# drprojects/superpoint_transformer

Hardware: AMD Instinct MI355X
Metric: Mpoints/s SPT fwd+bwd on S3DIS-scale NAG (higher is better)
Workload: dtype f32 (the reference's shipped matmul class - configs/train.yaml:60-61 `float32_matmul_precision: high` = TF32 / bf16x3 next to `precision: 32` - as bf16x3: matrix products on the bf16 pipe with split operands, attention and the backward of the fused layers and of the attention blocks' Linears hi*hi +

## Files before the change

include/spt_hip.h:

```cpp
#ifndef SPT_HIP_H
#define SPT_HIP_H

#include <stddef.h>
#include <stdint.h>

#ifdef __cplusplus
extern "C" {
#endif

typedef void* spt_stream_t;

enum spt_reduce_op {
  SPT_SUM = 0,
  SPT_MEAN = 1,
  SPT_MIN = 2,
  SPT_MAX = 3
};

typedef struct spt_gn_fwd_tables {
  const float* weight;
  const float* mean_scale;
  float eps;
  float* mean;
  float* rstd;
// ... 368 lines not shown
                                       const int64_t* edge_a, const int64_t* edge_b, int64_t e,
                                       float* gend, spt_stream_t stream);

int spt_skinny_linear_supported(int K, int N);
int spt_skinny_linear_f32(const float* x, int64_t rows, int K, const float* W, const float* bias,
                          int N, float* y, spt_stream_t stream);
int spt_skinny_linear_wt_f32(const float* x, int64_t rows, int K, const float* Wt, int N, float* y,
                             spt_stream_t stream);
int spt_skinny_pre_supported(int K, int N, int num_graphs);
int spt_skinny_linear_pre_f32(const float* x, int64_t rows, int K, const float* W, const float* bias,
                              int N, float* y, const float* pre_am, const float* pre_scale,
                              const float* pre_bias, const int64_t* batch, int num_graphs,
                              const float* residual, spt_stream_t stream);
int spt_skinny_dw_pre_f32(const float* gy, const float* x, int64_t rows, int N, int K, float* gw,
                          float* gb, const float* pre_am, const float* pre_scale,
                          const float* pre_bias, const int64_t* batch, int num_graphs, void* ws,
                          size_t ws_bytes, spt_stream_t stream);
int spt_skinny_use_split_bf16(int mode);
int spt_skinny_linear_pre_m_f32(const float* x, int64_t rows, int K, const float* W, const float* bias,
                                int N, float* y, const float* pre_am, const float* pre_scale,
                                const float* pre_bias, const int64_t* batch, int num_graphs,
                                const float* residual, int mode, spt_stream_t stream);
int spt_skinny_linear_wt_m_f32(const float* x, int64_t rows, int K, const float* Wt, int N, float* y,
                               int mode, spt_stream_t stream);
int spt_skinny_dw_pre_m_f32(const float* gy, const float* x, int64_t rows, int N, int K, float* gw,
                            float* gb, const float* pre_am, const float* pre_scale,
                            const float* pre_bias, const int64_t* batch, int num_graphs, int mode,
                            void* ws, size_t ws_bytes, spt_stream_t stream);
int spt_skinny_dw_supported(int K, int N);
size_t spt_skinny_dw_workspace_bytes(int K, int N);
int spt_skinny_dw_f32(const float* gy, const float* x, int64_t rows, int N, int K, float* gw,
                      float* gb, void* ws, size_t ws_bytes, spt_stream_t stream);
int spt_narrow_linear_bwd_supported(int K, int N);
size_t spt_narrow_linear_bwd_workspace_bytes(int K, int N);
int spt_narrow_linear_bwd_f32(const float* gy, const float* x, const float* W, int64_t rows, int N,
                              int K, float* gx, float* gw, float* gb, void* ws, size_t ws_bytes,
                              spt_stream_t stream);

int spt_graphnorm_tables_f32(const double* total, int num_graphs, int d, const float* weight,
                             const float* mean_scale, float eps, float* mean, float* rstd,
                             float* am, float* scale, spt_stream_t stream);
int spt_graphnorm_apply_f32(const float* x, const int64_t* batch, int64_t r, int d,
                            int num_graphs, const float* am, const float* scale,
                            const float* bias, float act_slope, float* y, spt_stream_t stream);
int spt_graphnorm_bwd_stats_f32(const float* x, const float* gy, const int64_t* batch, int64_t r,
                                int d, int num_graphs, const float* am, const float* scale,
                                const float* bias, float act_slope, double* total, void* ws,
                                size_t ws_bytes, spt_stream_t stream);
size_t spt_graphnorm_bwd_stats_sparse_workspace_bytes(int64_t num_seg, int d, int num_graphs);
int spt_graphnorm_bwd_stats_sparse_f32(const float* x, const float* gout, const int32_t* arg,
                                       const int64_t* seg_graph, const int64_t* graph_rows,
                                       int64_t num_seg, int64_t n, int d, int num_graphs,
                                       const float* am, const float* scale, const float* bias,
                                       float act_slope, double* total, void* ws,
                                       size_t ws_bytes, spt_stream_t stream);
int spt_graphnorm_bwd_stats_sparse_ex_f32(
    const void* x, int x_is_bf16, const float* gout, const int32_t* arg, const int64_t* seg_graph,
    const int64_t* graph_rows, int64_t num_seg, int64_t n, int d, int num_graphs,
    const float* am, const float* scale, const float* bias, float act_slope, double* total,
    void* ws, size_t ws_bytes, spt_stream_t stream);
int spt_graphnorm_bwd_stats_sparse_raw_f32(
    const float* raw, const float* gout, const int32_t* arg, const int64_t* seg_graph,
    const int64_t* graph_rows, int64_t num_seg, int64_t n, int d, int num_graphs,
    const float* am, const float* scale, const float* bias, float act_slope, double* total,
    void* ws, size_t ws_bytes, spt_stream_t stream);
int spt_graphnorm_bwd_tables_f32(const double* total, int num_graphs, int d, const float* weight,
                                 const float* mean_scale, const float* mean, const float* rstd,
                                 float* c1, float* c2, float* c3, float* gweight, float* gbias,
                                 float* gmean_scale, spt_stream_t stream);

int spt_fused_linear_supported(int K, int N);
int spt_fused_linear_use_split_bf16(int mode);
size_t spt_fused_linear_workspace_bytes(int K, int N);
int spt_fused_linear_fwd_f32(const float* x, int64_t r0, int64_t r1, int K, const float* W,
                             int N, const float* pre_am, const float* pre_scale,
                             const float* pre_bias, float pre_slope, float* h, double* total,
                             void* ws, size_t ws_bytes, spt_stream_t stream);
int spt_fused_linear_bwd_f32(const float* gy, const float* h, int64_t r0, int64_t r1, int N,
                             const float* am, const float* scale, const float* bias,
                             float slope, const float* c1, const float* c2, const float* c3,
                             const float* xprev, int K, const float* pre_am,
                             const float* pre_scale, const float* pre_bias, float pre_slope,
                             const float* W, float* gx, float* gW, int accumulate,
                             double* prev_total, void* ws, size_t ws_bytes, spt_stream_t stream);
int spt_fused_linear_pooled_supported(int K, int N);
int spt_fused_linear_pooled_supported_ex(int K, int N, int mode);
#define SPT_FMLP_BWD_REGISTER_STAGED 4
#define SPT_FMLP_H_BF16 8
#define SPT_FMLP_X_BF16 16
int spt_fused_linear_storage_supported(int K, int N);
int spt_fused_linear_bwd_use_dma(int on);
int spt_fused_linear_fwd_use_x3(int on);
int spt_fused_linear_fwd_ex_f32(const float* x, int64_t r0, int64_t r1, int K, const float* W,
                                int N, const float* pre_am, const float* pre_scale,
                                const float* pre_bias, float pre_slope, float* h, double* total,
                                int mode, void* ws, size_t ws_bytes, spt_stream_t stream);
int spt_fused_linear_bwd_ex_f32(const float* gy, const float* h, int64_t r0, int64_t r1, int N,
                                const float* am, const float* scale, const float* bias,
                                float slope, const float* c1, const float* c2, const float* c3,
                                const float* xprev, int K, const float* pre_am,
                                const float* pre_scale, const float* pre_bias, float pre_slope,
                                const float* W, float* gx, float* gW, int accumulate,
                                double* prev_total, int mode, void* ws, size_t ws_bytes,
                                spt_stream_t stream);
int spt_fused_linear_bwd_pooled_ex_f32(
    const float* gout, const int32_t* arg, const int32_t* perm, const int32_t* pos_seg,
    const float* h, int64_t p0, int64_t p1, int N, const float* am, const float* scale,
    const float* bias, float slope, const float* c1, const float* c2, const float* c3,
    const float* xprev, int K, const float* pre_am, const float* pre_scale, const float* pre_bias,
    float pre_slope, const float* W, float* gx, float* gW, int accumulate, double* prev_total,
    int mode, void* ws, size_t ws_bytes, spt_stream_t stream);
int spt_fused_linear_bwd_pooled_f32(
    const float* gout, const int32_t* arg, const int32_t* perm, const int32_t* pos_seg,
    const float* h, int64_t p0, int64_t p1, int N, const float* am, const float* scale,
    const float* bias, float slope, const float* c1, const float* c2, const float* c3,
    const float* xprev, int K, const float* pre_am, const float* pre_scale, const float* pre_bias,
    float pre_slope, const float* W, float* gx, float* gW, int accumulate, double* prev_total,
    void* ws, size_t ws_bytes, spt_stream_t stream);

int spt_fused_linear_fwd_runs_f32(const float* x, int nruns, const int64_t* run_r0,
                                  const int64_t* run_r1, const int32_t* run_graph, int num_graphs,
                                  int K, const float* W, int N, const float* pre_am,
                                  const float* pre_scale, const float* pre_bias, float pre_slope,
                                  float* h, double* total, int mode, void* ws, size_t ws_bytes,
                                  spt_stream_t stream);
int spt_fused_linear_bwd_runs_f32(
    const float* gy, const float* h, int nruns, const int64_t* run_r0, const int64_t* run_r1,
    const int32_t* run_graph, int num_graphs, int N, const float* am, const float* scale,
    const float* bias, float slope, const float* c1, const float* c2, const float* c3,
    const float* xprev, int K, const float* pre_am, const float* pre_scale, const float* pre_bias,
    float pre_slope, const float* W, float* gx, float* gW, double* prev_total, int mode, void* ws,
    size_t ws_bytes, spt_stream_t stream);
int spt_fused_linear_bwd_pooled_runs_f32(
    const float* gout, const int32_t* arg, const int32_t* perm, const int32_t* pos_seg,
    const float* h, int nruns, const int64_t* run_p0, const int64_t* run_p1,
    const int32_t* run_graph, int num_graphs, int N, const float* am, const float* scale,
    const float* bias, float slope, const float* c1, const float* c2, const float* c3,
    const float* xprev, int K, const float* pre_am, const float* pre_scale, const float* pre_bias,
    float pre_slope, const float* W, float* gx, float* gW, double* prev_total, int mode, void* ws,
    size_t ws_bytes, spt_stream_t stream);
int spt_fused_linear_fwd_runs_gn_f32(const float* x, int nruns, const int64_t* run_r0,
                                     const int64_t* run_r1, const int32_t* run_graph, int num_graphs,
                                     int K, const float* W, int N, const float* pre_am,
                                     const float* pre_scale, const float* pre_bias, float pre_slope,
                                     float* h, double* total, int mode, void* ws, size_t ws_bytes,
                                     const spt_gn_fwd_tables* norm, spt_stream_t stream);
int spt_fused_linear_bwd_runs_gn_f32(
    const float* gy, const float* h, int nruns, const int64_t* run_r0, const int64_t* run_r1,
    const int32_t* run_graph, int num_graphs, int N, const float* am, const float* scale,
    const float* bias, float slope, const float* c1, const float* c2, const float* c3,
    const float* xprev, int K, const float* pre_am, const float* pre_scale, const float* pre_bias,
    float pre_slope, const float* W, float* gx, float* gW, double* prev_total, int mode, void* ws,
    size_t ws_bytes, const spt_gn_bwd_tables* prev_norm, spt_stream_t stream);
int spt_fused_linear_bwd_pooled_runs_gn_f32(
    const float* gout, const int32_t* arg, const int32_t* perm, const int32_t* pos_seg,
    const float* h, int nruns, const int64_t* run_p0, const int64_t* run_p1,
    const int32_t* run_graph, int num_graphs, int N, const float* am, const float* scale,
    const float* bias, float slope, const float* c1, const float* c2, const float* c3,
    const float* xprev, int K, const float* pre_am, const float* pre_scale, const float* pre_bias,
    float pre_slope, const float* W, float* gx, float* gW, double* prev_total, int mode, void* ws,
    size_t ws_bytes, const spt_gn_bwd_tables* prev_norm, spt_stream_t stream);

int spt_csr_check_i64(const int64_t* idx, const int64_t* points, const int64_t* pointers, int64_t n,
                      int64_t num_seg, int check_ascending, int32_t* flag, spt_stream_t stream);
int spt_csr_adopt_i64(const int64_t* idx, const int64_t* points, const int64_t* pointers, int64_t n,
                      int64_t num_seg, int32_t* perm32, int32_t* rowptr32, int32_t* flag,
                      spt_stream_t stream);

int spt_fused_linear_pool_supported(int K, int N, int mode);
size_t spt_fused_linear_pool_gram_len(int K);
size_t spt_fused_linear_pool_workspace_bytes(int K, int N);
int spt_fused_linear_fwd_pool_runs_f32(
    const void* x, const int32_t* perm, const int32_t* pos_seg, const int32_t* rowptr,
    const int64_t* seg_graph, int64_t num_seg, int64_t n_rows, int nruns, const int64_t* run_p0,
    const int64_t* run_p1, const int32_t* run_graph, int num_graphs, int K, const float* W, int N,
    const float* gn_weight, const float* gn_bias, const float* gn_mean_scale, float eps, float slope,
    const float* pre_am, const float* pre_scale, const float* pre_bias, float pre_slope, float* out,
    int32_t* arg, int32_t* argpos, float* raw, double* gram, double* total, float* mean, float* rstd,
    float* am, float* scale, int mode, void* ws, size_t ws_bytes, spt_stream_t stream);
int spt_fused_linear_bwd_pool_runs_f32(
    const float* gout, const float* raw, const int32_t* argpos, const int32_t* perm,
    const int32_t* pos_seg, const int64_t* seg_graph, int64_t num_seg, int nruns,
    const int64_t* run_p0, const int64_t* run_p1, const int32_t* run_graph, int num_graphs, int N,
    const float* am, const float* scale, const float* bias, float slope, const float* c1,
    const float* c2, const float* c3, const void* xprev, int K, const float* pre_am,
    const float* pre_scale, const float* pre_bias, float pre_slope, const float* W,
    const double* gram, float* gm, float* gx, float* gW, double* prev_total, int mode, void* ws,
    size_t ws_bytes, spt_stream_t stream);
int spt_fused_linear_bwd_pool_runs_gn_f32(
    const float* gout, const float* raw, const int32_t* argpos, const int32_t* perm,
    const int32_t* pos_seg, const int64_t* seg_graph, int64_t num_seg, int nruns,
    const int64_t* run_p0, const int64_t* run_p1, const int32_t* run_graph, int num_graphs, int N,
    const float* am, const float* scale, const float* bias, float slope, const float* c1,
    const float* c2, const float* c3, const void* xprev, int K, const float* pre_am,
    const float* pre_scale, const float* pre_bias, float pre_slope, const float* W,
    const double* gram, float* gm, float* gx, float* gW, double* prev_total, int mode, void* ws,
    size_t ws_bytes, const spt_gn_bwd_tables* prev_norm, spt_stream_t stream);

size_t spt_cross_entropy_workspace_bytes(int64_t rows);
int spt_cross_entropy_fwd_f32(const float* logits, const int64_t* target, int64_t rows, int C,
                              int64_t ignore_index, float* lse, float* loss, float* count,
                              void* ws, size_t ws_bytes, spt_stream_t stream);
int spt_cross_entropy_bwd_f32(const float* logits, const int64_t* target, const float* lse,
                              int64_t rows, int C, int64_t ignore_index, const float* gout,
                              const float* count, float* glogits, spt_stream_t stream);

int spt_hist_loss_fwd_f32(const float* logits, const int64_t* target, int64_t rows, int C, int ncols,
                          int mode, int64_t ignore_index, const float* weight, float* loss,
                          double* den, int64_t* confmat, void* ws, size_t ws_bytes,
                          spt_stream_t stream);
int spt_hist_loss_bwd_f32(const float* logits, const int64_t* target, int64_t rows, int C, int ncols,
                          int mode, int64_t ignore_index, const float* weight, const float* gout,
                          const double* den, float* glogits, spt_stream_t stream);
int spt_confusion_matrix_i64(const int64_t* pred, const int64_t* target, int64_t rows, int C,
                             int ncols, int64_t* confmat, spt_stream_t stream);

#ifdef __cplusplus
}
#endif
#endif
```

superpoint_transformer_amd/_lib.py:

```python
import ctypes
import os

import torch

_HERE = os.path.dirname(os.path.abspath(__file__))
LIB_PATH = os.path.join(_HERE, "lib", "libspt_hip.so")

_c = ctypes
_i64 = _c.c_int64
_int = _c.c_int
_p = _c.c_void_p
_sz = _c.c_size_t
_f32 = _c.c_float
_f64 = _c.c_double

SIGNATURES = {
    "spt_version": (_int, []),
    "spt_last_error": (_c.c_char_p, []),
    "spt_csr_build_workspace_bytes": (_sz, [_i64, _i64]),
    "spt_csr_build": (_int, [_p, _i64, _i64, _p, _p, _p, _sz, _p]),
    "spt_csr_pos_seg": (_int, [_p, _i64, _i64, _p, _p]),
    "spt_csr_gather_i64_i32": (_int, [_p, _p, _i64, _p, _p]),
    "spt_segcsr_reduce_f32": (_int, [_int, _p, _p, _p, _i64, _i64, _int, _p, _p, _p]),
    "spt_segcsr_max_affine_f32": (_int, [_p, _p, _p, _i64, _i64, _int, _p, _p, _p, _f32, _p, _p, _p, _p]),
    "spt_segcsr_max_affine_bf16_supported": (_int, [_int, _i64]),
    "spt_segcsr_max_affine_bf16": (_int, [_p, _p, _p, _i64, _i64, _int, _p, _p, _p, _f32, _p, _p, _p, _p]),
    "spt_segcsr_max_affine_raw_supported": (_int, [_int, _i64]),
    "spt_segcsr_max_affine_raw_f32": (_int, [_p, _int, _p, _p, _i64, _i64, _int, _p, _p, _p, _f32, _p, _p, _p,
                                             _p, _p]),
    "spt_graphnorm_bwd_stats_sparse_raw_f32": (_int, [_p, _p, _p, _p, _p, _i64, _i64, _int, _int, _p, _p, _p,
                                                      _f32, _p, _p, _sz, _p]),
    "spt_fused_linear_storage_supported": (_int, [_int, _int]),
    "spt_graphnorm_bwd_stats_sparse_ex_f32": (_int, [_p, _int, _p, _p, _p, _p, _i64, _i64, _int, _int, _p, _p,
                                                     _p, _f32, _p, _p, _sz, _p]),
    "spt_segcsr_reduce_bwd_f32": (_int, [_int, _p, _p, _p, _p, _p, _i64, _i64, _int, _p, _p]),
    "spt_segcsr_sum_i64": (_int, [_p, _p, _p, _i64, _i64, _int, _p, _p]),
    "spt_gather_rows_f32": (_int, [_p, _p, _i64, _i64, _int, _p, _p]),
    "spt_graphnorm_workspace_bytes": (_sz, [_i64, _int, _int]),
    "spt_graphnorm_fwd_f32": (_int, [_p, _p, _i64, _int, _int, _p, _p, _p, _f32, _f32,
                                     _p, _p, _p, _p, _sz, _p]),
    "spt_graphnorm_bwd_f32": (_int, [_p, _p, _p, _i64, _int, _int, _p, _p, _p, _p, _p,
                                     _f32, _p, _p, _p, _p, _p, _sz, _p]),
    "spt_graphnorm_stats_f32": (_int, [_p, _p, _i64, _int, _int, _p, _p, _f32, _p, _p, _p, _p,
                                       _p, _sz, _p]),
    "spt_graphnorm_bwd_acc_f32": (_int, [_p, _p, _p, _i64, _int, _int, _p, _p, _p, _p, _p,
                                         _f32, _p, _p, _p, _p, _p, _p, _sz, _p]),
    "spt_edge_attn_fwd_f32": (_int, [_p, _i64, _int, _int, _int, _p, _p, _p, _i64, _p, _int,
                                     _p, _p, _p, _p, _p, _p, _int, _f32, _p, _p, _p, _p]),
    "spt_edge_attn_bwd_workspace_bytes": (_sz, [_int, _int, _int, _int]),
    "spt_attn_use_mfma": (_int, [_int]),
    "spt_attn_bwd_packed": (_int, [_int]),
    "spt_attn_bwd_el_full_line": (_int, [_int]),
    "spt_attn_bwd_el_target_order": (_int, [_int]),
    "spt_attn_tile_record_ints": (_int, []),
    "spt_attn_pack_tile_ids_ex": (_int, [_p, _p, _p, _p, _i64, _p, _p]),
    "spt_attn_tile_record_ints_m": (_int, [_int]),
    "spt_attn_pack_tile_ids_m": (_int, [_p, _p, _p, _p, _i64, _int, _p, _p]),
    "spt_attn_mirror_prepare": (_int, [_p, _p, _i64, _i64, _p, _p, _p]),
    "spt_attn_pack_tile_ids_mirror": (_int, [_p, _p, _p, _p, _i64, _i64, _p, _p]),
    "spt_attn_split_pack_f32": (_int, [_p, _i64, _int, _int, _p, _p]),
    "spt_attn_split_grad_f32": (_int, [_p, _i64, _int, _int, _p, _p]),
    "spt_edge_attn_bwd_f32": (_int, [_p, _i64, _int, _int, _int, _p, _p, _p, _i64, _p, _int,
                                     _p, _p, _p, _p, _p, _p, _int, _f32, _p, _p, _p, _p,
                                     _p, _p, _p, _p, _p, _p, _p, _p, _p, _sz, _p]),
    "spt_edge_attn_bwd_acc_f32": (_int, [_p, _i64, _int, _int, _int, _p, _p, _p, _i64, _p, _int,
                                         _p, _p, _p, _p, _p, _p, _int, _f32, _p, _p, _p, _p,
                                         _p, _p, _int, _p, _p, _p, _p, _p, _p, _p, _sz, _p]),
    "spt_edge_attn_fwd_ex_f32": (_int, [_p, _i64, _int, _int, _int, _p, _p, _p, _i64, _p, _int,
                                        _p, _p, _p, _p, _p, _p, _int, _f32, _p, _p, _p, _int, _p]),
    "spt_edge_attn_bwd_ex_workspace_bytes": (_sz, [_i64, _i64, _int, _int, _int, _int]),
    "spt_edge_attn_bwd_el_supported": (_int, [_int, _int, _int, _int, _int]),
    "spt_attn_pack_tile_ids": (_int, [_p, _p, _p, _i64, _p, _p]),
    "spt_edge_attn_bwd_ex_f32": (_int, [_p, _i64, _int, _int, _int, _p, _p, _p, _p, _p, _p, _p, _i64, _p, _int,
                                        _p, _p, _p, _p, _p, _p, _int, _f32, _p, _p, _p, _p,
                                        _p, _p, _int, _p, _p, _p, _p, _p, _p, _int, _p, _sz, _p]),
    "spt_grid_knn_workspace_bytes": (_sz, [_i64, _i64]),
    "spt_knn_use_cell_path": (_int, [_int]),
    "spt_segcsr_use_stream": (_int, [_int]),
    "spt_segcsr_reduce_ex_f32": (_int, [_int, _p, _p, _p, _i64, _i64, _int, _p, _p, _int, _p]),
    "spt_segcsr_max_affine_ex_f32": (_int, [_p, _p, _p, _i64, _i64, _int, _p, _p, _p, _f32, _p, _p, _p,
                                            _int, _p]),
    "spt_grid_knn_ex_f32": (_int, [_p, _i64, _p, _i64, _int, _f32, _f32, _p, _p, _int, _int, _int,
                                   _p, _p, _p, _int, _p, _sz, _p]),
    "spt_grid_knn_geof_f32": (_int, [_p, _i64, _int, _f32, _f32, _p, _p, _int, _int, _int, _int,
                                     _p, _p, _p, _p, _int, _p, _sz, _p]),
    "spt_grid_knn_after_f32": (_int, [_p, _i64, _p, _i64, _int, _f32, _f32, _p, _p, _int, _int, _p, _p,
                                      _p, _p, _p, _sz, _p]),
    "spt_grid_knn_f32": (_int, [_p, _i64, _p, _i64, _int, _f32, _f32, _p, _p, _int, _int, _int,
                                _p, _p, _p, _p, _sz, _p]),
    "spt_point_geof_dense_f32": (_int, [_p, _i64, _p, _int, _int, _int, _int, _p, _p, _p]),
    "spt_point_geof_dense_ld_f32": (_int, [_p, _i64, _p, _int, _i64, _int, _int, _int, _p, _p, _p]),
    "spt_bbox_f32": (_int, [_p, _i64, _p, _p]),
    "spt_knn_subsample_f32": (_int, [_p, _i64, _p, _f32, _int, _p, _p, _p]),
    "spt_grid_cell_ids_f32": (_int, [_p, _i64, _f32, _p, _p, _p, _p]),
    "spt_grid_count_cells_workspace_bytes": (_sz, [_i64]),
    "spt_grid_count_cells_f32": (_int, [_p, _i64, _f32, _p, _p, _p, _p, _sz, _p]),
    "spt_spatial_order_workspace_bytes": (_sz, [_i64, _i64]),
    "spt_spatial_order": (_int, [_p, _i64, _f32, _p, _p, _p, _p, _sz, _p]),
    "spt_point_geof_csr_f32": (_int, [_p, _i64, _p, _p, _int, _int, _int, _p, _p]),
    "spt_vertical_edge_features_f32": (_int, [_p, _i64] + [_p] * 13 + [_p]),
    "spt_edge_affinity_features_f32": (_int, [_p, _i64, _int, _p, _p, _i64, _p, _p]),
    "spt_edge_affinity_features_bwd_f32": (_int, [_p, _p, _i64, _int, _p, _p, _i64, _p, _p]),
    "spt_scatter_pca_f32": (_int, [_p, _p, _p, _i64, _p, _p, _p]),
    "spt_neighbors_dense_to_csr_workspace_bytes": (_sz, [_i64]),
    "spt_neighbors_dense_to_csr": (_int, [_p, _i64, _int, _p, _p, _p, _p, _sz, _p]),
    "spt_horizontal_edge_features_f32": (_int, [_p, _i64, _i64, _p, _p, _p, _p, _p, _p, _p, _int,
                                                _p, _p, _p]),
    "spt_graphnorm_tables_f32": (_int, [_p, _int, _int, _p, _p, _f32, _p, _p, _p, _p, _p]),
    "spt_graphnorm_apply_f32": (_int, [_p, _p, _i64, _int, _int, _p, _p, _p, _f32, _p, _p]),
    "spt_graphnorm_bwd_stats_f32": (_int, [_p, _p, _p, _i64, _int, _int, _p, _p, _p, _f32, _p,
                                           _p, _sz, _p]),
    "spt_graphnorm_bwd_stats_sparse_workspace_bytes": (_sz, [_i64, _int, _int]),
    "spt_graphnorm_bwd_stats_sparse_f32": (_int, [_p, _p, _p, _p, _p, _i64, _i64, _int, _int, _p, _p,
                                                   _p, _f32, _p, _p, _sz, _p]),
    "spt_graphnorm_bwd_tables_f32": (_int, [_p, _int, _int, _p, _p, _p, _p, _p, _p, _p, _p, _p,
                                            _p, _p]),
    "spt_fused_linear_supported": (_int, [_int, _int]),
    "spt_fused_linear_use_split_bf16": (_int, [_int]),
    "spt_fused_linear_bwd_use_dma": (_int, [_int]),
    "spt_fused_linear_fwd_use_x3": (_int, [_int]),
    "spt_fused_linear_pooled_supported": (_int, [_int, _int]),
    "spt_fused_linear_bwd_pooled_f32": (_int, [_p, _p, _p, _p, _p, _i64, _i64, _int, _p, _p, _p, _f32,
                                               _p, _p, _p, _p, _int, _p, _p, _p, _f32, _p, _p, _p,
                                               _int, _p, _p, _sz, _p]),
    "spt_fused_linear_pooled_supported_ex": (_int, [_int, _int, _int]),
    "spt_fused_linear_fwd_ex_f32": (_int, [_p, _i64, _i64, _int, _p, _int, _p, _p, _p, _f32, _p, _p,
                                           _int, _p, _sz, _p]),
    "spt_fused_linear_bwd_ex_f32": (_int, [_p, _p, _i64, _i64, _int, _p, _p, _p, _f32, _p, _p, _p,
                                           _p, _int, _p, _p, _p, _f32, _p, _p, _p, _int, _p, _int, _p,
                                           _sz, _p]),
    "spt_fused_linear_bwd_pooled_ex_f32": (_int, [_p, _p, _p, _p, _p, _i64, _i64, _int, _p, _p, _p, _f32,
                                                  _p, _p, _p, _p, _int, _p, _p, _p, _f32, _p, _p, _p,
                                                  _int, _p, _int, _p, _sz, _p]),
    "spt_fused_linear_workspace_bytes": (_sz, [_int, _int]),
    "spt_fused_linear_fwd_runs_f32": (_int, [_p, _int, _p, _p, _p, _int, _int, _p, _int, _p, _p, _p,
                                             _f32, _p, _p, _int, _p, _sz, _p]),
    "spt_fused_linear_bwd_runs_f32": (_int, [_p, _p, _int, _p, _p, _p, _int, _int, _p, _p, _p, _f32,
                                             _p, _p, _p, _p, _int, _p, _p, _p, _f32, _p, _p, _p, _p,
                                             _int, _p, _sz, _p]),
    "spt_fused_linear_bwd_pooled_runs_f32": (_int, [_p, _p, _p, _p, _p, _int, _p, _p, _p, _int, _int,
                                                    _p, _p, _p, _f32, _p, _p, _p, _p, _int, _p, _p,
                                                    _p, _f32, _p, _p, _p, _p, _int, _p, _sz, _p]),
    "spt_fused_linear_fwd_runs_gn_f32": (_int, [_p, _int, _p, _p, _p, _int, _int, _p, _int, _p, _p, _p,
                                                _f32, _p, _p, _int, _p, _sz, _p, _p]),
    "spt_fused_linear_bwd_runs_gn_f32": (_int, [_p, _p, _int, _p, _p, _p, _int, _int, _p, _p, _p, _f32,
                                                _p, _p, _p, _p, _int, _p, _p, _p, _f32, _p, _p, _p, _p,
                                                _int, _p, _sz, _p, _p]),
    "spt_fused_linear_bwd_pooled_runs_gn_f32": (_int, [_p, _p, _p, _p, _p, _int, _p, _p, _p, _int, _int,
                                                       _p, _p, _p, _f32, _p, _p, _p, _p, _int, _p, _p,
                                                       _p, _f32, _p, _p, _p, _p, _int, _p, _sz, _p, _p]),
    "spt_fused_linear_bwd_pool_runs_gn_f32": (_int, [_p, _p, _p, _p, _p, _p, _i64, _int, _p, _p, _p, _int,
                                                     _int, _p, _p, _p, _f32, _p, _p, _p, _p, _int, _p, _p,
                                                     _p, _f32, _p, _p, _p, _p, _p, _p, _int, _p, _sz, _p, _p]),
    "spt_csr_check_i64": (_int, [_p, _p, _p, _i64, _i64, _int, _p, _p]),
    "spt_csr_adopt_i64": (_int, [_p, _p, _p, _i64, _i64, _p, _p, _p, _p]),
    "spt_fused_linear_pool_supported": (_int, [_int, _int, _int]),
    "spt_fused_linear_pool_gram_len": (_sz, [_int]),
    "spt_fused_linear_pool_workspace_bytes": (_sz, [_int, _int]),
    "spt_fused_linear_fwd_pool_runs_f32": (_int, [_p, _p, _p, _p, _p, _i64, _i64, _int, _p, _p, _p, _int,
                                                  _int, _p, _int, _p, _p, _p, _f32, _f32, _p, _p, _p,
                                                  _f32, _p, _p, _p, _p, _p, _p, _p, _p, _p, _p, _int, _p,
                                                  _sz, _p]),
    "spt_fused_linear_bwd_pool_runs_f32": (_int, [_p, _p, _p, _p, _p, _p, _i64, _int, _p, _p, _p, _int,
                                                  _int, _p, _p, _p, _f32, _p, _p, _p, _p, _int, _p, _p,
                                                  _p, _f32, _p, _p, _p, _p, _p, _p, _int, _p, _sz, _p]),
    "spt_fused_linear_fwd_f32": (_int, [_p, _i64, _i64, _int, _p, _int, _p, _p, _p, _f32, _p, _p,
                                        _p, _sz, _p]),
    "spt_fused_linear_bwd_f32": (_int, [_p, _p, _i64, _i64, _int, _p, _p, _p, _f32, _p, _p, _p,
                                        _p, _int, _p, _p, _p, _f32, _p, _p, _p, _int, _p, _p,
                                        _sz, _p]),
    "spt_unit_sphere_norm_f32": (_int, [_p, _p, _p, _p, _p, _p, _i64, _i64, _p, _p, _p, _p]),
    "spt_unit_sphere_assemble_f32": (_int, [_p, _p, _p, _p, _p, _p, _i64, _i64, _p, _int, _p, _p, _p, _p]),
    "spt_unit_sphere_workspace_bytes": (_sz, [_i64, _i64]),
    "spt_unit_sphere_norm_ws_f32": (_int, [_p, _p, _p, _p, _p, _p, _i64, _i64, _p, _p, _p, _p, _sz, _p]),
    "spt_unit_sphere_assemble_ws_f32": (_int, [_p, _p, _p, _p, _p, _p, _i64, _i64, _p, _int, _p, _p, _p,
                                               _p, _sz, _p]),
    "spt_sparse_sample_workspace_bytes": (_sz, [_i64, _i64]),
    "spt_sparse_sample": (_int, [_p, _i64, _i64, _p, _int, _int, _c.c_uint64, _p, _p, _p, _sz, _p]),
    "spt_segment_std_f32": (_int, [_p, _p, _p, _i64, _int, _p, _p]),
    "spt_segment_mean_orientation_f32": (_int, [_p, _p, _p, _i64, _p, _p]),
    "spt_cluster_graph_edges_workspace_bytes": (_sz, [_i64, _int]),
    "spt_cluster_graph_edges": (_int, [_p, _p, _p, _i64, _int, _f32, _int, _p, _p, _p, _p, _sz, _p]),
    "spt_skinny_linear_supported": (_int, [_int, _int]),
    "spt_narrow_linear_bwd_supported": (_int, [_int, _int]),
    "spt_narrow_linear_bwd_workspace_bytes": (_sz, [_int, _int]),
    "spt_narrow_linear_bwd_f32": (_int, [_p, _p, _p, _i64, _int, _int, _p, _p, _p, _p, _sz, _p]),
    "spt_cross_entropy_workspace_bytes": (_sz, [_i64]),
    "spt_cross_entropy_fwd_f32": (_int, [_p, _p, _i64, _int, _i64, _p, _p, _p, _p, _sz, _p]),
    "spt_cross_entropy_bwd_f32": (_int, [_p, _p, _p, _i64, _int, _i64, _p, _p, _p, _p]),
    "spt_hist_loss_fwd_f32": (_int, [_p, _p, _i64, _int, _int, _int, _i64, _p, _p, _p, _p, _p, _sz, _p]),
    "spt_hist_loss_bwd_f32": (_int, [_p, _p, _i64, _int, _int, _int, _i64, _p, _p, _p, _p, _p]),
    "spt_confusion_matrix_i64": (_int, [_p, _p, _i64, _int, _int, _p, _p]),
    "spt_skinny_dw_supported": (_int, [_int, _int]),
    "spt_skinny_dw_workspace_bytes": (_sz, [_int, _int]),
    "spt_skinny_dw_f32": (_int, [_p, _p, _i64, _int, _int, _p, _p, _p, _sz, _p]),
    "spt_skinny_linear_f32": (_int, [_p, _i64, _int, _p, _p, _int, _p, _p]),
    "spt_skinny_linear_wt_f32": (_int, [_p, _i64, _int, _p, _int, _p, _p]),
    "spt_skinny_pre_supported": (_int, [_int, _int, _int]),
    "spt_skinny_linear_pre_f32": (_int, [_p, _i64, _int, _p, _p, _int, _p, _p, _p, _p, _p, _int, _p, _p]),
    "spt_skinny_dw_pre_f32": (_int, [_p, _p, _i64, _int, _int, _p, _p, _p, _p, _p, _p, _int, _p, _sz, _p]),
    "spt_skinny_use_split_bf16": (_int, [_int]),
    "spt_skinny_linear_pre_m_f32": (_int, [_p, _i64, _int, _p, _p, _int, _p, _p, _p, _p, _p, _int, _p, _int, _p]),
    "spt_skinny_linear_wt_m_f32": (_int, [_p, _i64, _int, _p, _int, _p, _int, _p]),
    "spt_skinny_dw_pre_m_f32": (_int, [_p, _p, _i64, _int, _int, _p, _p, _p, _p, _p, _p, _int, _int, _p, _sz, _p]),
    "spt_index_inverse": (_int, [_p, _i64, _i64, _p, _p]),
    "spt_select_edges_workspace_bytes": (_sz, [_i64]),
    "spt_select_edges": (_int, [_p, _i64, _i64, _p, _i64, _p, _i64, _p, _p, _p, _sz, _p]),
    "spt_cluster_select_workspace_bytes": (_sz, [_i64, _i64, _i64]),
    "spt_cluster_select": (_int, [_p, _p, _i64, _p, _i64, _i64, _p, _p, _p, _p, _p, _p, _sz, _p]),
    "spt_relabel_consecutive_workspace_bytes": (_sz, [_i64]),
    "spt_relabel_consecutive": (_int, [_p, _p, _i64, _i64, _p, _p, _p, _p, _sz, _p]),
    "spt_radius_ball_workspace_bytes": (_sz, [_i64]),
    "spt_radius_ball_f32": (_int, [_p, _i64, _p, _f32, _int, _p, _i64, _p, _p, _p, _sz, _p]),
    "spt_cluster_pair_anchors_f32": (_int, [_p, _p, _p, _p, _p, _i64, _i64, _int, _int, _p, _p, _p]),
    "spt_adjacency_stats_workspace_bytes": (_sz, [_i64]),
    "spt_adjacency_stats": (_int, [_p, _p, _i64, _i64, _int, _p, _p, _p, _sz, _p]),
    "spt_adjacency_regression": (_int, [_p, _p, _p, _i64, _i64, _int, _f32, _f32, _p, _p, _sz, _p]),
    "spt_adjacency_count_workspace_bytes": (_sz, [_i64]),
    "spt_adjacency_count": (_int, [_p, _i64, _i64, _int, _p, _p, _p, _i64, _int, _p, _p, _p, _sz, _p]),
    "spt_adjacency_fill_workspace_bytes": (_sz, [_i64, _i64]),
    "spt_adjacency_fill": (_int, [_p, _p, _i64, _i64, _int, _f32, _f32, _p, _p, _p, _p, _i64, _int, _int,
                                  _p, _p, _i64, _p, _p, _p, _p, _sz, _p]),
    "spt_ground_bounds_workspace_bytes": (_sz, [_i64]),
    "spt_ground_bounds_f32": (_int, [_p, _i64, _f32, _p, _p, _sz, _p]),
    "spt_ground_cell_min_f32": (_int, [_p, _i64, _f32, _i64, _i64, _i64, _i64, _p, _p]),
    "spt_ground_trim_workspace_bytes": (_sz, [_i64]),
    "spt_ground_trim_f32": (_int, [_p, _i64, _p, _int, _f32, _p, _f32, _p, _i64, _p, _i64, _p, _p, _sz, _p]),
    "spt_ground_ransac_workspace_bytes": (_sz, [_int]),
    "spt_ground_ransac_f32": (_int, [_p, _i64, _p, _p, _i64, _p, _p, _int, _f64, _p, _p, _p, _sz, _p]),
    "spt_ground_elevation_f32": (_int, [_p, _i64, _p, _f32, _p, _p]),
    "spt_point_color_workspace_bytes": (_sz, [_i64]),
    "spt_point_color_f32": (_int, [_p, _int, _i64, _int, _p, _i64, _p, _i64, _p, _i64, _p, _sz, _p]),
    "spt_point_density_f32": (_int, [_p, _i64, _p, _i64, _i64, _int, _p, _p]),
}


class GnFwdTables(ctypes.Structure):
    _fields_ = [("weight", _p), ("mean_scale", _p), ("eps", _f32), ("mean", _p), ("rstd", _p),
                ("am", _p), ("scale", _p)]


class GnBwdTables(ctypes.Structure):
    _fields_ = [("weight", _p), ("mean_scale", _p), ("mean", _p), ("rstd", _p), ("c1", _p), ("c2", _p),
                ("c3", _p), ("gweight", _p), ("gbias", _p), ("gmean_scale", _p)]


def _load():
    if not os.path.exists(LIB_PATH):
        raise ImportError(
            f"{LIB_PATH} is missing: run `python -c 'import __graft_entry__ as g; "
            f"g.build()'` (hipcc --offload-arch=gfx950). There is no fallback path.")
    lib = ctypes.CDLL(LIB_PATH)
    for name, (res, args) in SIGNATURES.items():
        fn = getattr(lib, name)
        fn.restype = res
        fn.argtypes = args
    return lib


lib = _load()


def last_error():
    return lib.spt_last_error().decode("utf-8", "replace")


def check(status, what):
    if status != 0:
        raise RuntimeError(f"{what} failed ({status}): {last_error()}")


def ptr(t):
    return None if t is None else t.data_ptr()


def stream_ptr(device=None):
    return torch.cuda.current_stream(device).cuda_stream


def require_cuda(*tensors):
    for t in tensors:
        if t is not None and not t.is_cuda:
            raise RuntimeError(
                "superpoint_transformer_amd ops run on the MI355X only: got a "
                f"{t.device} tensor (no CPU fallback is provided)")
```

superpoint_transformer_amd/csrc/fused_mlp.hip:

```cpp
#include <math.h>
#include <stdlib.h>

#include "common.hpp"

namespace spt {
namespace fmlp {

typedef float f32x4 __attribute__((ext_vector_type(4)));
constexpr int WAVES = 4;
constexpr int TR = 16;
constexpr int MAX_BLOCKS = 1024;
constexpr int MAX_BWD_WAVES = 4096;

__device__ __forceinline__ double xg_sum_d(double v) {
  v += __shfl_xor(v, 16, 64);
  v += __shfl_xor(v, 32, 64);
  return v;
}
__device__ __forceinline__ void wave_sync_lds() {
  __builtin_amdgcn_fence(__ATOMIC_RELEASE, "wavefront");
  __builtin_amdgcn_wave_barrier();
  __builtin_amdgcn_fence(__ATOMIC_ACQUIRE, "wavefront");
}

// ... 637 lines not shown
    const __bf16 a = (__bf16)x[i];
    const float r1 = x[i] - (float)a;
    const __bf16 b = (__bf16)r1;
    const float r2 = r1 - (float)b;
    h[i] = a;
    m[i] = b;
    l[i] = (__bf16)r2;
  }
}
template <int K4, int NBK>
__global__ __launch_bounds__(WAVES_X3 * 64, 2) void fwd_kernel_x3(
    const float* __restrict__ x, int64_t r0, int64_t r1, int K, const float* __restrict__ W,
    const float* __restrict__ am, const float* __restrict__ sc, const float* __restrict__ bs,
    float slope, float* __restrict__ h, double* __restrict__ partial, FmlpRuns rt) {
  constexpr int KP = K4 * 4, KS = (KP + 31) / 32, KP32 = KS * 32, LDA = KP32 + 4, N = NBK * 16;
  constexpr int LDW = KP32 + 8;
  SPT_FMLP_RUN_FWD(N)
  __shared__ __attribute__((aligned(16))) float a_lds[WAVES_X3][TR * LDA];
  __shared__ __attribute__((aligned(16))) float tab[3 * KP32];
  __shared__ __attribute__((aligned(16))) __bf16 wpl[3][N * LDW];
  __shared__ double red[WAVES_X3][2 * N];
  const int lane = threadIdx.x & 63;
  const int wid = __builtin_amdgcn_readfirstlane(threadIdx.x >> 6);
  const int g = lane >> 4, c = lane & 15;
  float* al = a_lds[wid];
  const bool pre = am != nullptr;
  load_table(tab, am, K, KP32);
  load_table(tab + KP32, sc, K, KP32);
  load_table(tab + 2 * KP32, bs, K, KP32);
  for (int i = lane; i < TR * LDA; i += 64) al[i] = 0.f;
  for (int i = threadIdx.x; i < N * KP32; i += WAVES_X3 * 64) {
    const int n = i / KP32, k = i - n * KP32;
    const float w1[1] = {(k < K) ? W[(size_t)n * K + k] : 0.f};
    __bf16 a[1], b[1], cc[1];
    split3_bf16<1>(w1, a, b, cc);
    wpl[0][n * LDW + k] = a[0];
    wpl[1][n * LDW + k] = b[0];
    wpl[2][n * LDW + k] = cc[0];
  }
  __syncthreads();

  double s1[NBK], s2[NBK];
#pragma unroll
  for (int nb = 0; nb < NBK; ++nb) s1[nb] = s2[nb] = 0.0;

  const int64_t ntiles = (r1 - r0 + TR - 1) / TR;
  const int64_t wave = (int64_t)blockIdx.x * WAVES_X3 + wid;
  const int64_t nwaves = (int64_t)gridDim.x * WAVES_X3;
  constexpr int CHP = KP / 4, NITP = (TR * CHP + 63) / 64;
  const bool pref = (K & 3) == 0 && K == KP;
  float4 pv[NITP];
  auto prefetch = [&](int64_t t) {
    const int64_t row0 = r0 + t * TR;
    const int cnt = (t < ntiles) ? (int)((r1 - row0) < TR ? (r1 - row0) : TR) : 0;
#pragma unroll
    for (int j = 0; j < NITP; ++j) {
      const int q = lane + 64 * j, rr = q / CHP, k = (q - rr * CHP) << 2;
      const bool ok = q < TR * CHP && rr < cnt;
      const float4 v = *reinterpret_cast<const float4*>(x + (ok ? (row0 + rr) * K + k : r0 * K));
      pv[j] = ok ? v : make_float4(0.f, 0.f, 0.f, 0.f);
    }
  };
  if (pref && wave < ntiles) prefetch(wave);
  for (int64_t t = wave; t < ntiles; t += nwaves) {
    const int64_t row0 = r0 + t * TR;
    const int cnt = (int)((r1 - row0) < TR ? (r1 - row0) : TR);
    wave_sync_lds();
    if (pref) {
#pragma unroll
      for (int j = 0; j < NITP; ++j) {
        const int q = lane + 64 * j, rr = q / CHP, k = (q - rr * CHP) << 2;
        if (q < TR * CHP) {
          float4 w = pv[j];
          if (pre && rr < cnt) {
            const float4 a = *reinterpret_cast<const float4*>(tab + k);
            const float4 s4 = *reinterpret_cast<const float4*>(tab + KP32 + k);
            const float4 b = *reinterpret_cast<const float4*>(tab + 2 * KP32 + k);
            w.x = fmaf(w.x - a.x, s4.x, b.x); w.y = fmaf(w.y - a.y, s4.y, b.y);
            w.z = fmaf(w.z - a.z, s4.z, b.z); w.w = fmaf(w.w - a.w, s4.w, b.w);
            w.x = w.x > 0.f ? w.x : w.x * slope; w.y = w.y > 0.f ? w.y : w.y * slope;
            w.z = w.z > 0.f ? w.z : w.z * slope; w.w = w.w > 0.f ? w.w : w.w * slope;
          }
          *reinterpret_cast<float4*>(al + rr * LDA + k) = w;
        }
      }
    } else {
      stage_tile<KP32, LDA, KP32>(x, row0, cnt, K, pre, tab, slope, al, nullptr, lane);
    }
    wave_sync_lds();
    if (pref) prefetch(t + nwaves);
    f32x4 C[NBK];
#pragma unroll
    for (int nb = 0; nb < NBK; ++nb) C[nb] = (f32x4){0.f, 0.f, 0.f, 0.f};
#pragma unroll
    for (int ks = 0; ks < KS; ++ks) {
      const float4 a0 = *reinterpret_cast<const float4*>(al + c * LDA + 32 * ks + 8 * g);
      const float4 a1 = *reinterpret_cast<const float4*>(al + c * LDA + 32 * ks + 8 * g + 4);
      const float av[8] = {a0.x, a0.y, a0.z, a0.w, a1.x, a1.y, a1.z, a1.w};
      bf16x8 x1, x2, x3;
      split3_bf16<8>(av, x1, x2, x3);
#pragma unroll
      for (int nb = 0; nb < NBK; ++nb) {
        const int wo = (16 * nb + c) * LDW + 32 * ks + 8 * g;
        const bf16x8 w1 = *reinterpret_cast<const bf16x8*>(&wpl[0][wo]);
        const bf16x8 w2 = *reinterpret_cast<const bf16x8*>(&wpl[1][wo]);
        const bf16x8 w3 = *reinterpret_cast<const bf16x8*>(&wpl[2][wo]);
        f32x4 acc = C[nb];
        acc = __builtin_amdgcn_mfma_f32_16x16x32_bf16(x3, w1, acc, 0, 0, 0);
        acc = __builtin_amdgcn_mfma_f32_16x16x32_bf16(x1, w3, acc, 0, 0, 0);
        acc = __builtin_amdgcn_mfma_f32_16x16x32_bf16(x2, w2, acc, 0, 0, 0);
        acc = __builtin_amdgcn_mfma_f32_16x16x32_bf16(x2, w1, acc, 0, 0, 0);
        acc = __builtin_amdgcn_mfma_f32_16x16x32_bf16(x1, w2, acc, 0, 0, 0);
        acc = __builtin_amdgcn_mfma_f32_16x16x32_bf16(x1, w1, acc, 0, 0, 0);
        C[nb] = acc;
      }
    }
#pragma unroll
    for (int r = 0; r < 4; ++r) {
      const int rr = 4 * g + r;
      if (rr < cnt) {
        float* hr = h + (row0 + rr) * N + c;
#pragma unroll
        for (int nb = 0; nb < NBK; ++nb) {
          const float v = C[nb][r];
          hr[16 * nb] = v;
          s1[nb] += (double)v;
          s2[nb] += (double)v * (double)v;
        }
      }
    }
  }
#pragma unroll
  for (int nb = 0; nb < NBK; ++nb) {
    const double a = xg_sum_d(s1[nb]), b = xg_sum_d(s2[nb]);
    if (g == 0) {
      red[wid][nb * 16 + c] = a;
      red[wid][N + nb * 16 + c] = b;
    }
  }
  __syncthreads();
  double* out = partial + (size_t)blockIdx.x * (2 * N + 1);
  for (int i = threadIdx.x; i < 2 * N; i += WAVES_X3 * 64) {
    double t2 = 0.0;
#pragma unroll
    for (int w = 0; w < WAVES_X3; ++w) t2 += red[w][i];
    out[i] = t2;
  }
  if (threadIdx.x == 0) out[2 * N] = (blockIdx.x == 0) ? (double)(r1 - r0) : 0.0;
}

__host__ __device__ constexpr bool fmlp_bf_wg_reduce(int K4, int NBK, int NW) {
  return NBK * 16 <= NW * TR && K4 > 0;
}
template <int K4, int NBK, bool NEED_GX, int NW, bool LO, bool POOLED = false, bool PIPE = false,
          bool H16 = false, bool X16 = false>
__global__ __launch_bounds__(NW * 64, NW / 4) void bwd_kernel_bf(
    const float* __restrict__ gy, const float* __restrict__ h, int64_t r0, int64_t r1,
    const float* __restrict__ am, const float* __restrict__ sc, const float* __restrict__ bs,
    float slope, const float* __restrict__ c1, const float* __restrict__ c2,
    const float* __restrict__ c3, const float* __restrict__ xprev, int K,
    const float* __restrict__ pam, const float* __restrict__ psc, const float* __restrict__ pbs,
    float pslope, const float* __restrict__ W, float* __restrict__ gx,
    float* __restrict__ gw_partial, double* __restrict__ pstat_partial, FmlpRuns rt,
    const int32_t* __restrict__ perm = nullptr, const int32_t* __restrict__ pos_seg = nullptr,
    const float* __restrict__ gout = nullptr, const int32_t* __restrict__ arg = nullptr) {
  constexpr int KP = K4 * 4, KB = (KP + 15) / 16, KPP = KB * 16, N = NBK * 16;
  constexpr int NS = (N + 31) / 32, NP32 = NS * 32;
  constexpr int LDG = NP32 + 4, LDX = KPP + 4, LDT = NP32 + 8;
  constexpr bool WGR = fmlp_bf_wg_reduce(K4, NBK, NW);
  SPT_FMLP_RUN_BWD_T(N, NW, (WGR ? 1 : NW))
  __shared__ __attribute__((aligned(16))) float g_lds[NW][TR * LDG];
  __shared__ __attribute__((aligned(16))) float x_lds[NW][TR * LDX];
  __shared__ __attribute__((aligned(16))) __bf16 wt_hi[NEED_GX ? KPP * LDT : 8];
  __shared__ __attribute__((aligned(16))) __bf16 wt_lo[NEED_GX ? KPP * LDT : 8];
  __shared__ __attribute__((aligned(16))) float gt[6 * N];
  __shared__ __attribute__((aligned(16))) float pt[3 * KPP];
  const int lane = threadIdx.x & 63;
  const int wid = __builtin_amdgcn_readfirstlane(threadIdx.x >> 6);
  const int g = lane >> 4, c = lane & 15;
  float* gl = g_lds[wid];
  float* xl = x_lds[wid];
  const bool pre = pam != nullptr;
  if constexpr (NEED_GX) {
    for (int i = threadIdx.x; i < KPP * NP32; i += NW * 64) {
      const int k = i / NP32, n = i - k * NP32;
      const float w = (k < K && n < N) ? W[(size_t)n * K + k] : 0.f;
      const __bf16 hh = (__bf16)w;
      wt_hi[k * LDT + n] = hh;
      wt_lo[k * LDT + n] = (__bf16)(w - (float)hh);
    }
  }
  load_table(gt, am, N, N);
  load_table(gt + N, sc, N, N);
  load_table(gt + 2 * N, bs, N, N);
  load_table(gt + 3 * N, c1, N, N);
  load_table(gt + 4 * N, c2, N, N);
  load_table(gt + 5 * N, c3, N, N);
  load_table(pt, pam, K, KPP);
  load_table(pt + KPP, psc, K, KPP);
  load_table(pt + 2 * KPP, pbs, K, KPP);
  for (int i = lane; i < TR * LDX; i += 64) xl[i] = 0.f;
  for (int i = lane; i < TR * LDG; i += 64) gl[i] = 0.f;
  __syncthreads();

  f32x4 C3[NBK][KB];
#pragma unroll
  for (int nb = 0; nb < NBK; ++nb)
#pragma unroll
    for (int kb = 0; kb < KB; ++kb) C3[nb][kb] = (f32x4){0.f, 0.f, 0.f, 0.f};
  double p1[KB], p2[KB];
#pragma unroll
  for (int kb = 0; kb < KB; ++kb) p1[kb] = p2[kb] = 0.0;

  const int64_t ntiles = (r1 - r0 + TR - 1) / TR;
  const int64_t wave = (int64_t)blockIdx.x * NW + wid;
  const int64_t nwaves = (int64_t)gridDim.x * NW;
  auto gh_of = [&](const float4& hv, const float4& gv, int n) {
    const float4 a = *reinterpret_cast<const float4*>(gt + n);
    const float4 sc4 = *reinterpret_cast<const float4*>(gt + N + n);
    const float4 b4 = *reinterpret_cast<const float4*>(gt + 2 * N + n);
    const float4 k1 = *reinterpret_cast<const float4*>(gt + 3 * N + n);
    const float4 k2 = *reinterpret_cast<const float4*>(gt + 4 * N + n);
    const float4 k3 = *reinterpret_cast<const float4*>(gt + 5 * N + n);
    const float hh[4] = {hv.x, hv.y, hv.z, hv.w}, gg4[4] = {gv.x, gv.y, gv.z, gv.w};
    const float aa[4] = {a.x, a.y, a.z, a.w}, ss[4] = {sc4.x, sc4.y, sc4.z, sc4.w};
    const float bb[4] = {b4.x, b4.y, b4.z, b4.w}, q1[4] = {k1.x, k1.y, k1.z, k1.w};
    const float q2[4] = {k2.x, k2.y, k2.z, k2.w}, q3[4] = {k3.x, k3.y, k3.z, k3.w};
    float o4[4];
#pragma unroll
    for (int e = 0; e < 4; ++e) {
      const float o = hh[e] - aa[e];
      float gg = gg4[e];
      if (slope != 1.f) {
        const float y = fmaf(o, ss[e], bb[e]);
        gg = (y > 0.f) ? gg : gg * slope;
      }
      o4[e] = fmaf(q1[e], gg, -fmaf(q2[e], o, q3[e]));
    }
    return make_float4(o4[0], o4[1], o4[2], o4[3]);
  };
  static_assert(!(PIPE && (H16 || X16)), "the register-prefetch variant reads f32 rows");
  constexpr int CH = N / 4, CHX = KPP / 4;
  constexpr int HN = PIPE ? TR * CH / 64 : 1, XN = PIPE ? TR * CHX / 64 : 1;
  float4 p_h[HN], p_g[HN], p_x[XN];
  int4 p_a[(PIPE && POOLED) ? HN : 1];
  int rid_n = 0, seg_n = 0;
  auto load_ids = [&](int64_t t) {
    rid_n = seg_n = 0;
    if constexpr (POOLED) {
      const int64_t rowf = r0 + t * TR;
      if (t < ntiles && rowf + lane < r1 && lane < TR) {
        rid_n = perm[rowf + lane];
        seg_n = pos_seg[rowf + lane];
      }
    }
  };
  auto load_raw = [&](int64_t t, int rid_l, int seg_l) {
    const int64_t row0 = r0 + t * TR;
    const int cnt = (t < ntiles) ? (int)((r1 - row0) < TR ? (r1 - row0) : TR) : 0;
#pragma unroll
    for (int i = 0; i < HN; ++i) {
      const int q = lane + 64 * i, rr = q / CH, n = (q - rr * CH) << 2;
      const int rid = POOLED ? __shfl(rid_l, rr, 64) : 0;
      const int64_t sg = POOLED ? (int64_t)__shfl(seg_l, rr, 64) : 0;
      p_h[i] = p_g[i] = make_float4(0.f, 0.f, 0.f, 0.f);
      if (rr < cnt) {
        const int64_t hr = POOLED ? (int64_t)rid : row0 + rr;
        p_h[i] = *reinterpret_cast<const float4*>(h + hr * N + n);
        if constexpr (POOLED) {
          p_a[i] = *reinterpret_cast<const int4*>(arg + sg * N + n);
          p_g[i] = *reinterpret_cast<const float4*>(gout + sg * N + n);
        } else {
          p_g[i] = *reinterpret_cast<const float4*>(gy + (row0 + rr) * N + n);
        }
      }
    }
#pragma unroll
    for (int i = 0; i < XN; ++i) {
      const int q = lane + 64 * i, rr = q / CHX, k = (q - rr * CHX) << 2;
      const int64_t xr = POOLED ? (int64_t)__shfl(rid_l, rr, 64) : row0 + rr;
      p_x[i] = make_float4(0.f, 0.f, 0.f, 0.f);
      if (rr < cnt && k < K) p_x[i] = *reinterpret_cast<const float4*>(xprev + xr * K + k);
    }
  };
  load_ids(wave);
  if constexpr (PIPE) {
    load_raw(wave, rid_n, seg_n);
  }
  int rid_l = rid_n, seg_l = seg_n;
  load_ids(wave + nwaves);
  FM_PROBE_INIT
  for (int64_t t = wave; t < ntiles; t += nwaves) {
    const int64_t row0 = r0 + t * TR;
    const int cnt = (int)((r1 - row0) < TR ? (r1 - row0) : TR);
    wave_sync_lds();
    FM_PROBE(5)
    if constexpr (PIPE) {
#pragma unroll
      for (int i = 0; i < HN; ++i) {
        const int q = lane + 64 * i, rr = q / CH, n = (q - rr * CH) << 2;
        float4 gv = p_g[i];
        if constexpr (POOLED) {
          const int rid = __shfl(rid_l, rr, 64);
          gv = make_float4(p_a[i].x == rid ? gv.x : 0.f, p_a[i].y == rid ? gv.y : 0.f,
                           p_a[i].z == rid ? gv.z : 0.f, p_a[i].w == rid ? gv.w : 0.f);
        }
        float4 v = make_float4(0.f, 0.f, 0.f, 0.f);
        if (rr < cnt) v = gh_of(p_h[i], gv, n);
        *reinterpret_cast<float4*>(gl + rr * LDG + n) = v;
      }
#pragma unroll
      for (int i = 0; i < XN; ++i) {
        const int q = lane + 64 * i, rr = q / CHX, k = (q - rr * CHX) << 2;
        *reinterpret_cast<float4*>(xl + rr * LDX + k) = p_x[i];
      }
    } else {
      constexpr int NITG = TR * CH / 64, GS = NITG < 2 ? 1 : 2;
      static_assert(TR * CH % 64 == 0, "whole waves of chunks");
#pragma unroll 1
      for (int i0 = 0; i0 < NITG; i0 += GS) {
        float4 hv[GS], gv[GS];
        int4 av[POOLED ? GS : 1];
        int ridv[GS];
#pragma unroll
        for (int j = 0; j < GS; ++j) {
          const int q = lane + 64 * (i0 + j), rr = q / CH, n = (q - rr * CH) << 2;
          ridv[j] = POOLED ? __shfl(rid_l, rr, 64) : 0;
          const int64_t sg = POOLED ? (int64_t)__shfl(seg_l, rr, 64) : 0;
          hv[j] = gv[j] = make_float4(0.f, 0.f, 0.f, 0.f);
          if constexpr (POOLED) av[j] = make_int4(-1, -1, -1, -1);
          if (rr < cnt) {
            const int64_t hr = POOLED ? (int64_t)ridv[j] : row0 + rr;
            hv[j] = ld4<H16>(h, hr * N + n);
            if constexpr (POOLED) {
              av[j] = *reinterpret_cast<const int4*>(arg + sg * N + n);
              gv[j] = *reinterpret_cast<const float4*>(gout + sg * N + n);
            } else {
              gv[j] = *reinterpret_cast<const float4*>(gy + (row0 + rr) * N + n);
            }
          }
        }
#pragma unroll
        for (int j = 0; j < GS; ++j) {
          const int q = lane + 64 * (i0 + j), rr = q / CH, n = (q - rr * CH) << 2;
          float4 v = make_float4(0.f, 0.f, 0.f, 0.f);
          if (rr < cnt) {
            float4 g4 = gv[j];
            if constexpr (POOLED) {
              const int rid = ridv[j];
              g4 = make_float4(av[j].x == rid ? g4.x : 0.f, av[j].y == rid ? g4.y : 0.f,
                               av[j].z == rid ? g4.z : 0.f, av[j].w == rid ? g4.w : 0.f);
            }
            v = gh_of(hv[j], g4, n);
          }
          *reinterpret_cast<float4*>(gl + rr * LDG + n) = v;
        }
      }
      FM_PROBE(0)
      stage_tile<KPP, LDX, KPP, POOLED, (POOLED && NBK >= 8) ? 2 : 4, X16>(xprev, row0, cnt, K, false, pt,
                                                                             pslope, xl, nullptr, lane, rid_l);
      FM_PROBE(1)
    }
    const int rid_cur = rid_l;
    if constexpr (PIPE) load_raw(t + nwaves, rid_n, seg_n);
    rid_l = rid_n;
    seg_l = seg_n;
    load_ids(t + 2 * nwaves);
    wave_sync_lds();
    FM_PROBE(2)
    {
      bf16x4 Xh[KB], Xl[KB];
#pragma unroll
      for (int kb = 0; kb < KB; ++kb) {
        const int k = 16 * kb + c;
        float xv[4];
#pragma unroll
        for (int r = 0; r < 4; ++r) {
          float v = xl[(4 * g + r) * LDX + k];
          if (pre) {
            v = fmaf(v - pt[k], pt[KPP + k], pt[2 * KPP + k]);
            v = (v > 0.f) ? v : v * pslope;
            v = (4 * g + r < cnt && k < K) ? v : 0.f;
          }
          xv[r] = v;
        }
        split_bf16<4>(xv, Xh[kb], Xl[kb]);
      }
#pragma unroll
      for (int nb = 0; nb < NBK; ++nb) {
        float gv[4];
#pragma unroll
        for (int r = 0; r < 4; ++r) gv[r] = gl[(4 * g + r) * LDG + 16 * nb + c];
        bf16x4 gh4, gl4;
        split_bf16<4>(gv, gh4, gl4);
#pragma unroll
        for (int kb = 0; kb < KB; ++kb) C3[nb][kb] = mfma3_16<LO>(gh4, gl4, Xh[kb], Xl[kb], C3[nb][kb]);
      }
    }
    FM_PROBE(3)
    if constexpr (NEED_GX) {
      f32x4 CX[KB];
#pragma unroll
      for (int kb = 0; kb < KB; ++kb) CX[kb] = (f32x4){0.f, 0.f, 0.f, 0.f};
      constexpr int LAB = (NW == 4 && K4 > 16) ? 2 : 0, NSTG = NS * KB;
      bf16x8 bfh[LAB + 1], bfl[LAB + 1];
      auto ldb = [&](int step, bf16x8& bh, bf16x8& bl) {
        const int sg = step / KB, kb = step - sg * KB;
        bh = *reinterpret_cast<const bf16x8*>(wt_hi + (16 * kb + c) * LDT + 32 * sg + 8 * g);
        if constexpr (LO) bl = *reinterpret_cast<const bf16x8*>(wt_lo + (16 * kb + c) * LDT + 32 * sg + 8 * g);
        else bl = bh;
      };
#pragma unroll
      for (int i = 0; i < LAB && i < NSTG; ++i) ldb(i, bfh[i], bfl[i]);
      bf16x8 ah, alo;
#pragma unroll
      for (int step = 0; step < NSTG; ++step) {
        const int sg = step / KB, kb = step - sg * KB;
        if (kb == 0) {
          const float4 a0 = *reinterpret_cast<const float4*>(gl + c * LDG + 32 * sg + 8 * g);
          const float4 a1 = *reinterpret_cast<const float4*>(gl + c * LDG + 32 * sg + 8 * g + 4);
          const float av[8] = {a0.x, a0.y, a0.z, a0.w, a1.x, a1.y, a1.z, a1.w};
          split_bf16<8>(av, ah, alo);
        }
        if (step + LAB < NSTG) ldb(step + LAB, bfh[(step + LAB) % (LAB + 1)], bfl[(step + LAB) % (LAB + 1)]);
        if constexpr (LAB > 0) __builtin_amdgcn_sched_barrier(0);
        CX[kb] = mfma3_32<LO>(ah, alo, bfh[step % (LAB + 1)], bfl[step % (LAB + 1)], CX[kb]);
        if constexpr (LAB > 0) __builtin_amdgcn_sched_barrier(0);
      }
#pragma unroll
      for (int r = 0; r < 4; ++r) {
        const int rr = 4 * g + r;
        const int64_t orow = POOLED ? (int64_t)__shfl(rid_cur, rr, 64) : row0 + rr;
        if (rr < cnt) {
#pragma unroll
          for (int kb = 0; kb < KB; ++kb) {
            const int k = 16 * kb + c;
            if (k < K) {
              const float v = CX[kb][r];
              gx[orow * K + k] = v;
              if (pre) {
                const float o = xl[rr * LDX + k] - pt[k];
                float gg = v;
                if (pslope != 1.f) {
                  const float y = fmaf(o, pt[KPP + k], pt[2 * KPP + k]);
                  gg = (y > 0.f) ? gg : gg * pslope;
                }
                p1[kb] += (double)gg;
                p2[kb] += (double)gg * (double)o;
              }
            }
          }
        }
      }
    }
    FM_PROBE(4)
  }
#ifdef SPT_FMLP_PROFILE
  if (K4 == 16 && NBK == 8 && lane == 0 && wave == 5)
    printf("fmlp bwd<16,8,pooled=%d> wave 5 cycles: stage_gh %lu stage_x %lu ids+sync %lu dW %lu "
           "dX+store+stats %lu looptop %lu\n", (int)POOLED, (unsigned long)prof[0],
           (unsigned long)prof[1], (unsigned long)prof[2], (unsigned long)prof[3],
           (unsigned long)prof[4], (unsigned long)prof[5]);
#endif
  if constexpr (WGR) {
    __syncthreads();
    float* red = &x_lds[0][0];
    for (int w = 1; w < NW; ++w) {
      if (wid == w) {
#pragma unroll
        for (int nb = 0; nb < NBK; ++nb)
#pragma unroll
          for (int kb = 0; kb < KB; ++kb)
#pragma unroll
            for (int r = 0; r < 4; ++r) red[(16 * nb + 4 * g + r) * LDX + 16 * kb + c] = C3[nb][kb][r];
      }
      __syncthreads();
      if (wid == 0) {
#pragma unroll
        for (int nb = 0; nb < NBK; ++nb)
#pragma unroll
          for (int kb = 0; kb < KB; ++kb)
#pragma unroll
            for (int r = 0; r < 4; ++r) C3[nb][kb][r] += red[(16 * nb + 4 * g + r) * LDX + 16 * kb + c];
      }
      __syncthreads();
    }
  }
  if (!WGR || wid == 0) {
    float* gwp = gw_partial + (size_t)(WGR ? (int64_t)blockIdx.x : wave) * N * K;
#pragma unroll
    for (int nb = 0; nb < NBK; ++nb)
#pragma unroll
      for (int kb = 0; kb < KB; ++kb)
#pragma unroll
        for (int r = 0; r < 4; ++r) {
          const int k = 16 * kb + c;
          if (k < K) gwp[(size_t)(16 * nb + 4 * g + r) * K + k] = C3[nb][kb][r];
        }
  }
  if (pstat_partial) {
    double* pp = pstat_partial + (size_t)wave * (2 * K + 1);
#pragma unroll
    for (int kb = 0; kb < KB; ++kb) {
      const double a = xg_sum_d(p1[kb]), b = xg_sum_d(p2[kb]);
      const int k = 16 * kb + c;
      if (g == 0 && k < K) {
        pp[k] = a;
        pp[K + k] = b;
      }
    }
    if (lane == 0) pp[2 * K] = (wave == 0) ? (double)(r1 - r0) : 0.0;
  }
}

template <typename T>
__device__ __forceinline__ void reduce_tables_body(const T* __restrict__ partial, int ntab, int len,
                                                   T* __restrict__ total, int accumulate,
                                                   int bx = -1) {
  __shared__ T sl[64][17];
  const int cl = threadIdx.x & 15;
  const int col = (bx < 0 ? (int)blockIdx.x : bx) * 16 + cl;
  const int slice = threadIdx.x >> 4;
  T acc = 0;
  if (col < len) {
    const int per = (ntab + 63) / 64;
    const int lo = slice * per, hi = (lo + per < ntab) ? lo + per : ntab;
    int k = lo;
    constexpr int UNR = sizeof(T) == 4 ? 8 : 4;
    for (; k + UNR <= hi; k += UNR) {
      T a[UNR];
#pragma unroll
      for (int j = 0; j < UNR; ++j) a[j] = partial[(size_t)(k + j) * len + col];
#pragma unroll
      for (int j = 0; j < UNR; ++j) acc += a[j];
    }
    for (; k + 4 <= hi; k += 4) {
      const T a0 = partial[(size_t)k * len + col], a1 = partial[(size_t)(k + 1) * len + col];
      const T a2 = partial[(size_t)(k + 2) * len + col], a3 = partial[(size_t)(k + 3) * len + col];
      acc += a0; acc += a1; acc += a2; acc += a3;
    }
    for (; k < hi; ++k) acc += partial[(size_t)k * len + col];
  }
  sl[slice][cl] = acc;
  __syncthreads();
  if (slice == 0 && col < len) {
    T t = 0;
#pragma unroll
    for (int k = 0; k < 64; ++k) t += sl[k][cl];
    total[col] = accumulate ? total[col] + t : t;
  }
}
template <typename T>
__global__ __launch_bounds__(1024) void reduce_tables_kernel(const T* __restrict__ partial,
                                                             int ntab, int len,
                                                             T* __restrict__ total, int accumulate) {
  reduce_tables_body<T>(partial, ntab, len, total, accumulate);
}
template <typename T>
__global__ __launch_bounds__(1024) void reduce_tables_groups_kernel(const T* __restrict__ partial,
                                                                    FmlpGroups grp, int len,
                                                                    T* __restrict__ total) {
  const int b = blockIdx.y;
  reduce_tables_body<T>(partial + (size_t)grp.start[b] * len, grp.count[b], len,
                        total + (size_t)b * len, 0);
}

template <int NV>
__device__ __forceinline__ void sliced_col_sums(const double* const (&base)[NV], const int (&ntab)[NV],
                                                int len, const int (&col)[NV], double (*sl)[17],
                                                double (&out)[NV]) {
  const int cl = threadIdx.x & 15, slice = threadIdx.x >> 4;
  double acc[NV];
  int lo[NV], hi[NV], kmax = 0;
#pragma unroll
  for (int v = 0; v < NV; ++v) {
    acc[v] = 0;
    const int per = (ntab[v] + 63) / 64;
    lo[v] = slice * per;
    hi[v] = (lo[v] + per < ntab[v]) ? lo[v] + per : ntab[v];
    if (col[v] < 0) hi[v] = lo[v];
    const int n = hi[v] - lo[v];
    kmax = n > kmax ? n : kmax;
  }
  constexpr int UNR = NV <= 3 ? 4 : 1;
  int k = 0;
  if constexpr (UNR > 1)
  for (; k + UNR <= kmax; k += UNR) {
    double t[NV][UNR];
#pragma unroll
    for (int j = 0; j < UNR; ++j)
#pragma unroll
      for (int v = 0; v < NV; ++v)
        t[v][j] = (lo[v] + k + j < hi[v]) ? base[v][(size_t)(lo[v] + k + j) * len + col[v]] : 0.0;
#pragma unroll
    for (int j = 0; j < UNR; ++j)
#pragma unroll
      for (int v = 0; v < NV; ++v)
        if (lo[v] + k + j < hi[v]) acc[v] += t[v][j];
  }
  for (; k < kmax; ++k) {
    double t[NV];
#pragma unroll
    for (int v = 0; v < NV; ++v)
      t[v] = (lo[v] + k < hi[v]) ? base[v][(size_t)(lo[v] + k) * len + col[v]] : 0.0;
#pragma unroll
    for (int v = 0; v < NV; ++v)
      if (lo[v] + k < hi[v]) acc[v] += t[v];
  }
#pragma unroll
  for (int v = 0; v < NV; ++v) {
    sl[slice][cl] = acc[v];
    __syncthreads();
    double t = 0;
    if (slice == 0) {
#pragma unroll 8
      for (int k = 0; k < 64; ++k) t += sl[k][cl];
    }
    out[v] = t;
    __syncthreads();
  }
}

__global__ __launch_bounds__(1024) void fwd_post_kernel(const double* __restrict__ partial,
                                                        FmlpGroups grp, int N,
                                                        double* __restrict__ total,
                                                        spt_gn_fwd_tables t) {
  __shared__ double sl[64][17];
  const int b = blockIdx.y, cl = threadIdx.x & 15, slice = threadIdx.x >> 4;
  const int c = blockIdx.x * 16 + cl, len = 2 * N + 1;
  const bool cv = c < N;
  const double* pb = partial + (size_t)grp.start[b] * len;
  const double* const base[3] = {pb, pb, pb};
  const int ntab[3] = {grp.count[b], grp.count[b], grp.count[b]};
  const int col[3] = {cv ? c : -1, cv ? N + c : -1, 2 * N};
  double s3[3];
  sliced_col_sums<3>(base, ntab, len, col, sl, s3);
  const double s1 = s3[0], s2 = s3[1], cnt = s3[2];
  if (slice != 0) return;
  if (total) {
    double* tr = total + (size_t)b * len;
    if (cv) {
      tr[c] = s1;
      tr[N + c] = s2;
    }
    if (blockIdx.x == 0 && cl == 0) tr[2 * N] = cnt;
  }
  if (!cv) return;
  double n = cnt;
  if (n < 1.0) n = 1.0;
  const double mu = s1 / n;
  const double a = (double)t.mean_scale[c];
  double var = s2 / n - (2.0 * a - a * a) * mu * mu;
  if (var < 0.0) var = 0.0;
  const double rs = 1.0 / sqrt(var + (double)t.eps);
  const float mu32 = (float)mu, rs32 = (float)rs;
  const int o = b * N + c;
  t.mean[o] = mu32;
  t.rstd[o] = rs32;
  t.am[o] = (float)(a * (double)mu32);
  t.scale[o] = (float)((double)t.weight[c] * (double)rs32);
}

constexpr int POST_GB = 2;
__global__ __launch_bounds__(1024, 8) void bwd_post_kernel(const float* __restrict__ gwp, int ntab_w,
                                                        int NK, float* __restrict__ gW, int accumulate,
                                                        int nA, const double* __restrict__ pst,
                                                        FmlpGroups grp, int K, int B,
                                                        double* __restrict__ prev_total,
                                                        spt_gn_bwd_tables pn) {
  if ((int)blockIdx.x < nA) {
    reduce_tables_body<float>(gwp, ntab_w, NK, gW, accumulate, (int)blockIdx.x);
    return;
  }
  const int bx = (int)blockIdx.x - nA, len = 2 * K + 1;
  if (!pn.c1) {
    const int per_graph = (len + 15) / 16;
    const int b = bx / per_graph;
    reduce_tables_body<double>(pst + (size_t)grp.start[b] * len, grp.count[b], len,
                               prev_total + (size_t)b * len, 0, bx - b * per_graph);
    return;
  }
  __shared__ double sl[64][17];
  const int cl = threadIdx.x & 15, slice = threadIdx.x >> 4;
  const int c = bx * 16 + cl;
  const bool cv = c < K;
  const double w = cv ? (double)pn.weight[c] : 0.0, a = cv ? (double)pn.mean_scale[c] : 0.0;
  double gw = 0.0, gb = 0.0, ga = 0.0;
  for (int b0 = 0; b0 < B; b0 += POST_GB) {
    const int nb = (B - b0 < POST_GB) ? B - b0 : POST_GB;
    const double* base[3 * POST_GB];
    int ntab[3 * POST_GB], col[3 * POST_GB];
#pragma unroll
    for (int j = 0; j < POST_GB; ++j) {
      const int b = b0 + (j < nb ? j : 0);
      const double* pb = pst + (size_t)grp.start[b] * len;
      base[3 * j] = base[3 * j + 1] = base[3 * j + 2] = pb;
      ntab[3 * j] = ntab[3 * j + 1] = ntab[3 * j + 2] = grp.count[b];
      col[3 * j] = (j < nb && cv) ? c : -1;
      col[3 * j + 1] = (j < nb && cv) ? K + c : -1;
      col[3 * j + 2] = j < nb ? 2 * K : -1;
    }
    double s[3 * POST_GB];
    sliced_col_sums<3 * POST_GB>(base, ntab, len, col, sl, s);
    if (slice != 0) continue;
#pragma unroll
    for (int j = 0; j < POST_GB; ++j) {
      if (j >= nb) break;
      const int b = b0 + j;
      const double A = s[3 * j], GO = s[3 * j + 1], cnt = s[3 * j + 2];
      if (prev_total) {
        double* tr = prev_total + (size_t)b * len;
        if (cv) {
          tr[c] = A;
          tr[K + c] = GO;
        }
        if (bx == 0 && cl == 0) tr[2 * K] = cnt;
      }
      if (!cv) continue;
      double n = cnt;
      if (n < 1.0) n = 1.0;
      const double sd = (double)pn.rstd[b * K + c], mu = (double)pn.mean[b * K + c];
      const double k2 = w * sd * sd * sd * GO / n;
      const double sumdo = w * sd * A - k2 * n * mu * (1.0 - a);
      pn.c1[b * K + c] = (float)(w * sd);
      pn.c2[b * K + c] = (float)k2;
      pn.c3[b * K + c] = (float)(a * sumdo / n);
      gw += sd * GO;
      gb += A;
      ga += -mu * sumdo;
    }
  }
  if (slice == 0 && cv) {
    pn.gweight[c] = (float)gw;
    pn.gbias[c] = (float)gb;
    pn.gmean_scale[c] = (float)ga;
  }
}

static void bwd_post_launch(const float* gwp, int ntab_w, int NK, float* gW, int accumulate,
                            const double* pst, const FmlpGroups& grp, int K, int B,
                            double* prev_total, const spt_gn_bwd_tables* pn, hipStream_t stream) {
  const int nA = (NK + 15) / 16;
  spt_gn_bwd_tables none = {};
  int nB = 0;
  if (pn && pn->c1) nB = (K + 15) / 16;
  else if (prev_total) nB = ((2 * K + 1 + 15) / 16) * B;
  bwd_post_kernel<<<nA + nB, 1024, 0, stream>>>(gwp, ntab_w, NK, gW, accumulate, nA, pst, grp, K, B,
                                                prev_total, (pn && pn->c1) ? *pn : none);
}

static int grid_for_nw(int64_t rows, int per_cu, int nwv) {
  const int64_t tiles = (rows + TR - 1) / TR;
  int64_t blocks = (tiles + nwv - 1) / nwv;
  const int64_t cap = 256 * per_cu;
  if (blocks > cap) blocks = cap;
  if (blocks < 1) blocks = 1;
  return (int)blocks;
}

static int grid_for(int64_t rows, int per_cu) {
  const int64_t tiles = (rows + TR - 1) / TR;
  int64_t blocks = (tiles + WAVES - 1) / WAVES;
  const int64_t cap = 256 * per_cu;
  if (blocks > cap) blocks = cap;
  if (blocks < 1) blocks = 1;
  return (int)blocks;
}

}

bool fmlp_dma_supported(int K, int N);
int fmlp_dma_bwd_launch(bool pooled, bool lo, const float* gy, const float* h, FmlpRuns rt,
                        int64_t max_rows, int N, const float* am, const float* sc, const float* bs,
                        float slope, const float* c1, const float* c2, const float* c3,
                        const float* xprev, int K, const float* pam, const float* psc,
                        const float* pbs, float pslope, const float* W, float* gx,
                        float* gw_partial, double* pstat_partial, const int32_t* perm,
                        const int32_t* pos_seg, const float* gout, const int32_t* arg,
                        hipStream_t stream, bool s16 = false, int* gw_tabs = nullptr);
}

using namespace spt;
using namespace spt::fmlp;

#define SPT_FMLP_SHAPES(X) X(3, 2) X(5, 2) X(8, 2) X(8, 4) X(16, 4) X(16, 8) X(17, 4) X(33, 4)

static std::atomic<int> g_fmlp_mode{1};
static inline int fmlp_mode_of(int mode) { return mode < 0 ? (int)g_fmlp_mode : (mode & 3); }
static std::atomic<int> g_fmlp_x3{[] { const char* e = getenv("SPT_FMLP_X3"); return e ? (atoi(e) != 0) : 1; }()};
extern "C" int spt_fused_linear_fwd_use_x3(int on) {
  const int prev = g_fmlp_x3;
  if (on >= 0) g_fmlp_x3 = on != 0;
  return prev;
}
static std::atomic<int> g_fmlp_dma{1};
static inline bool fmlp_dma_of(int mode) { return g_fmlp_dma != 0 && !(mode >= 0 && (mode & 4)); }
extern "C" int spt_fused_linear_bwd_use_dma(int on) {
  const int prev = g_fmlp_dma;
  if (on >= 0) g_fmlp_dma = on != 0;
  return prev;
}
extern "C" int spt_fused_linear_use_split_bf16(int mode) {
  const int prev = g_fmlp_mode;
  g_fmlp_mode = mode < 0 ? 0 : (mode > 3 ? 3 : mode);
  return prev;
}

#define SPT_FMLP_POOLED_SHAPES(X) X(16, 8) X(16, 4) X(8, 4)
extern "C" int spt_fused_linear_pooled_supported(int K, int N) {
  return spt_fused_linear_pooled_supported_ex(K, N, -1);
}
extern "C" int spt_fused_linear_pooled_supported_ex(int K, int N, int mode) {
  const int k4 = (K + 3) / 4, nbk = N / 16;
  if (N % 16 || fmlp_mode_of(mode) < 1) return 0;
#define X(a, b) if (k4 == a && nbk == b) return 1;
  SPT_FMLP_POOLED_SHAPES(X)
#undef X
  return 0;
}

#define SPT_FMLP_ST_SHAPES(X) X(3, 2) X(8, 4) X(16, 8) X(16, 4)
#define SPT_FMLP_ST_POOLED_SHAPES(X) X(16, 8) X(16, 4) X(8, 4)
extern "C" int spt_fused_linear_storage_supported(int K, int N) {
  const int k4 = (K + 3) / 4, nbk = N / 16;
  if (N % 16) return 0;
#define X(a, b) if (k4 == a && nbk == b) return 1;
  SPT_FMLP_ST_SHAPES(X)
#undef X
  return 0;
}

extern "C" int spt_fused_linear_supported(int K, int N) {
  const int k4 = (K + 3) / 4, nbk = N / 16;
  if (N % 16) return 0;
#define X(a, b) if (k4 == a && nbk == b) return 1;
  SPT_FMLP_SHAPES(X)
#undef X
  return 0;
}

extern "C" size_t spt_fused_linear_workspace_bytes(int K, int N) {
  const size_t fwd = (size_t)MAX_BLOCKS * (2 * N + 1) * 8;
  const size_t bwd = (size_t)MAX_BWD_WAVES * ((size_t)N * K * 4 + (2 * K + 1) * 8);
  return align_up(fwd > bwd ? fwd : bwd, 256) + 4096;
}

static const char* fmlp_make_runs(int nruns, const int64_t* r0, const int64_t* r1, const int32_t* g,
                                  int num_graphs, FmlpRuns* rt, int64_t* max_rows) {
  if (nruns < 1 || nruns > FMLP_MAX_RUNS) return "1 <= nruns <= 16";
  if (num_graphs < 1 || num_graphs > FMLP_MAX_RUNS) return "1 <= num_graphs <= 16";
  if (!r0 || !r1 || !g) return "null run table";
  rt->n = nruns;
  *max_rows = 0;
  for (int r = 0; r < nruns; ++r) {
    if (r1[r] < r0[r] || g[r] < 0 || g[r] >= num_graphs) return "bad run";
    if (r && g[r] < g[r - 1]) return "runs must be sorted by graph";
    rt->r0[r] = r0[r];
    rt->r1[r] = r1[r];
    rt->g[r] = g[r];
    if (r1[r] - r0[r] > *max_rows) *max_rows = r1[r] - r0[r];
  }
  return nullptr;
}
static FmlpGroups fmlp_groups(const FmlpRuns& rt, int num_graphs, int per_run) {
  FmlpGroups grp;
  for (int b = 0; b < FMLP_MAX_RUNS; ++b) grp.start[b] = grp.count[b] = 0;
  for (int r = 0; r < rt.n; ++r) {
    const int b = rt.g[r];
    if (grp.count[b] == 0) grp.start[b] = r * per_run;
    grp.count[b] += per_run;
  }
  (void)num_graphs;
  return grp;
}

static int fmlp_fwd_impl(const char* fn, const float* x, const FmlpRuns& rt, int64_t max_rows,
                         int num_graphs, int K, const float* W, int N, const float* pre_am,
                         const float* pre_scale, const float* pre_bias, float pre_slope, float* h,
                         double* total, int mode, void* ws, size_t ws_bytes, hipStream_t stream,
                         const spt_gn_fwd_tables* norm = nullptr) {
  const int g_fmlp_mode = fmlp_mode_of(mode);
  (void)fn;
  SPT_CHECK_ARG(K >= 1 && N >= 16, "bad shape");
  SPT_CHECK_ARG(spt_fused_linear_supported(K, N), "(K, N) not built");
  SPT_CHECK_ARG(x && W && h && (total || norm) && ws, "null pointer");
  SPT_CHECK_ARG(!norm || (norm->weight && norm->mean_scale && norm->mean && norm->rstd && norm->am &&
                          norm->scale), "incomplete norm tables");
  auto post = [&](const double* partial_, int gx__) {
    if (norm)
      fwd_post_kernel<<<dim3((N + 15) / 16, num_graphs), 1024, 0, stream>>>(
          partial_, fmlp_groups(rt, num_graphs, gx__), N, total, *norm);
    else
      reduce_tables_groups_kernel<double><<<dim3((2 * N + 1 + 15) / 16, num_graphs), 1024, 0, stream>>>(
          partial_, fmlp_groups(rt, num_graphs, gx__), 2 * N + 1, total);
  };
  SPT_CHECK_ARG(ws_bytes >= spt_fused_linear_workspace_bytes(K, N), "workspace too small");
  SPT_CHECK_ARG(!pre_am || (pre_scale && pre_bias), "incomplete pre-normalisation tables");
  const int k4 = (K + 3) / 4, nbk = N / 16;
  const int per_cu = (k4 * nbk <= 32) ? 4 : 2;
  int gx_ = grid_for(max_rows, per_cu);
  const int cap = MAX_BLOCKS / rt.n;
  if (gx_ > cap) gx_ = cap;
  const bool x3 = g_fmlp_mode == 1 && g_fmlp_x3 && !(mode >= 0 && (mode & (SPT_FMLP_H_BF16 | SPT_FMLP_X_BF16)));
  if (x3) {
    const int64_t tiles = (max_rows + TR - 1) / TR;
    int64_t blocks = (tiles + WAVES_X3 - 1) / WAVES_X3;
    const int64_t cap8 = 256 * ((k4 * nbk <= 32) ? 2 : 1);
    if (blocks > cap8) blocks = cap8;
    if (blocks > cap) blocks = cap;
    gx_ = (int)(blocks < 1 ? 1 : blocks);
  }
  const dim3 grid((unsigned)gx_, (unsigned)rt.n);
  const dim3 grid8 = grid;
  double* partial = (double*)ws;
  const bool h16 = mode >= 0 && (mode & SPT_FMLP_H_BF16), x16 = mode >= 0 && (mode & SPT_FMLP_X_BF16);
  if (h16 || x16) {
    SPT_CHECK_ARG(g_fmlp_mode == 3 && h16 && spt_fused_linear_storage_supported(K, N) &&
                  (!x16 || K % 32 == 0),
                  "bf16 activation storage: bf16 matrix mode, a built shape, h stored as bf16");
#define XS(a, b)                                                                                   \
  if (k4 == a && nbk == b) {                                                                       \
    if (x16)                                                                                       \
      fwd_kernel_bf<a, b, false, true, true><<<grid, WAVES * 64, 0, stream>>>(                     \
          x, 0, 0, K, W, pre_am, pre_scale, pre_bias, pre_slope, h, partial, rt);                  \
    else                                                                                           \
      fwd_kernel_bf<a, b, false, false, true><<<grid, WAVES * 64, 0, stream>>>(                    \
          x, 0, 0, K, W, pre_am, pre_scale, pre_bias, pre_slope, h, partial, rt);                  \
  }
    SPT_FMLP_ST_SHAPES(XS)
#undef XS
    post(partial, gx_);
    SPT_CHECK_LAUNCH();
    return 0;
  }
#define X(a, b)                                                                        \
  if (k4 == a && nbk == b) {                                                           \
    if (g_fmlp_mode == 3)                                                              \
      fwd_kernel_bf<a, b, false><<<grid, WAVES * 64, 0, stream>>>(x, 0, 0, K, W, pre_am, pre_scale, \
                                                                  pre_bias, pre_slope, h, partial, rt); \
    else if (g_fmlp_mode == 2)                                                         \
      fwd_kernel_bf<a, b, true><<<grid, WAVES * 64, 0, stream>>>(x, 0, 0, K, W, pre_am, pre_scale, \
                                                                 pre_bias, pre_slope, h, partial, rt);  \
    else if (g_fmlp_mode == 1 && g_fmlp_x3)                                            \
      fwd_kernel_x3<a, b><<<grid8, WAVES_X3 * 64, 0, stream>>>(x, 0, 0, K, W, pre_am, pre_scale, \
                                                               pre_bias, pre_slope, h, partial, rt); \
    else                                                                               \
      fwd_kernel<a, b><<<grid, WAVES * 64, 0, stream>>>(x, 0, 0, K, W, pre_am, pre_scale, \
                                                        pre_bias, pre_slope, h, partial, rt);  \
  }
  SPT_FMLP_SHAPES(X)
#undef X
  post(partial, gx_);
  SPT_CHECK_LAUNCH();
  return 0;
}

extern "C" int spt_fused_linear_fwd_f32(const float* x, int64_t r0, int64_t r1, int K,
                                        const float* W, int N, const float* pre_am,
                                        const float* pre_scale, const float* pre_bias,
                                        float pre_slope, float* h, double* total, void* ws,
                                        size_t ws_bytes, spt_stream_t stream_) {
  return spt_fused_linear_fwd_ex_f32(x, r0, r1, K, W, N, pre_am, pre_scale, pre_bias, pre_slope, h,
                                     total, -1, ws, ws_bytes, stream_);
}
extern "C" int spt_fused_linear_fwd_ex_f32(const float* x, int64_t r0, int64_t r1, int K,
                                           const float* W, int N, const float* pre_am,
                                           const float* pre_scale, const float* pre_bias,
                                           float pre_slope, float* h, double* total, int mode,
                                           void* ws, size_t ws_bytes, spt_stream_t stream_) {
  SPT_CHECK_ARG(r1 >= r0, "bad shape");
  FmlpRuns rt;
  rt.n = 1; rt.g[0] = 0; rt.r0[0] = r0; rt.r1[0] = r1;
  return fmlp_fwd_impl(__func__, x, rt, r1 - r0, 1, K, W, N, pre_am, pre_scale, pre_bias, pre_slope,
                       h, total, mode, ws, ws_bytes, (hipStream_t)stream_);
}
extern "C" int spt_fused_linear_fwd_runs_f32(const float* x, int nruns, const int64_t* run_r0,
                                             const int64_t* run_r1, const int32_t* run_graph,
                                             int num_graphs, int K, const float* W, int N,
                                             const float* pre_am, const float* pre_scale,
                                             const float* pre_bias, float pre_slope, float* h,
                                             double* total, int mode, void* ws, size_t ws_bytes,
                                             spt_stream_t stream_) {
  FmlpRuns rt;
  int64_t max_rows;
  const char* err = fmlp_make_runs(nruns, run_r0, run_r1, run_graph, num_graphs, &rt, &max_rows);
  SPT_CHECK_ARG(!err, err ? err : "");
  return fmlp_fwd_impl(__func__, x, rt, max_rows, num_graphs, K, W, N, pre_am, pre_scale, pre_bias,
                       pre_slope, h, total, mode, ws, ws_bytes, (hipStream_t)stream_);
}
extern "C" int spt_fused_linear_fwd_runs_gn_f32(const float* x, int nruns, const int64_t* run_r0,
                                                const int64_t* run_r1, const int32_t* run_graph,
                                                int num_graphs, int K, const float* W, int N,
                                                const float* pre_am, const float* pre_scale,
                                                const float* pre_bias, float pre_slope, float* h,
                                                double* total, int mode, void* ws, size_t ws_bytes,
                                                const spt_gn_fwd_tables* norm, spt_stream_t stream_) {
  FmlpRuns rt;
  int64_t max_rows;
  const char* err = fmlp_make_runs(nruns, run_r0, run_r1, run_graph, num_graphs, &rt, &max_rows);
  SPT_CHECK_ARG(!err, err ? err : "");
  SPT_CHECK_ARG(norm, "null norm descriptor");
  return fmlp_fwd_impl(__func__, x, rt, max_rows, num_graphs, K, W, N, pre_am, pre_scale, pre_bias,
                       pre_slope, h, total, mode, ws, ws_bytes, (hipStream_t)stream_, norm);
}

static int fmlp_bwd_impl(bool pooled, const float* gy, const float* gout, const int32_t* arg,
                         const int32_t* perm, const int32_t* pos_seg, const float* h,
                         const FmlpRuns& rt, int64_t max_rows, int num_graphs, int N,
                         const float* am, const float* scale, const float* bias, float slope,
                         const float* c1, const float* c2, const float* c3, const float* xprev,
                         int K, const float* pre_am, const float* pre_scale, const float* pre_bias,
                         float pre_slope, const float* W, float* gx, float* gW, int accumulate,
                         double* prev_total, int mode, void* ws, size_t ws_bytes,
                         hipStream_t stream, const spt_gn_bwd_tables* prev_norm = nullptr) {
  const int g_fmlp_mode = fmlp_mode_of(mode);
  const bool g_fmlp_split_bf16 = g_fmlp_mode >= 1;
  const bool want_prev = prev_total || prev_norm;
  SPT_CHECK_ARG(!prev_norm || (prev_norm->weight && prev_norm->mean_scale && prev_norm->mean &&
                               prev_norm->rstd && prev_norm->c1 && prev_norm->c2 && prev_norm->c3 &&
                               prev_norm->gweight && prev_norm->gbias && prev_norm->gmean_scale),
                "incomplete norm tables");
  SPT_CHECK_ARG(K >= 1 && N >= 16, "bad shape");
  SPT_CHECK_ARG(h && am && scale && bias && c1 && c2 && c3 && xprev && W && gW && ws, "null pointer");
  SPT_CHECK_ARG(ws_bytes >= spt_fused_linear_workspace_bytes(K, N), "workspace too small");
  if (pooled) {
    SPT_CHECK_ARG(spt_fused_linear_pooled_supported_ex(K, N, g_fmlp_mode),
                  "(K, N) has no pooled kernel in this matrix mode");
    SPT_CHECK_ARG(gout && arg && perm && pos_seg && gx, "null pointer");
    SPT_CHECK_ARG(!want_prev || pre_am, "previous-layer statistics need its tables");
  } else {
    SPT_CHECK_ARG(spt_fused_linear_supported(K, N), "(K, N) not built");
    SPT_CHECK_ARG(gy, "null pointer");
    SPT_CHECK_ARG(!want_prev || (gx && pre_am), "previous-layer statistics need gx and its tables");
  }
  const int k4 = (K + 3) / 4, nbk = N / 16;
  int gx_ = 1, nwv = 1;
  float* gwp = (float*)ws;
  double* pst = (double*)((char*)ws + align_up((size_t)MAX_BWD_WAVES * N * K * 4, 256));
  double* pstp = want_prev ? pst : nullptr;
  const int nr = rt.n;
  auto cap_grid = [&](int g_, int nw_) {
    const int cap = MAX_BWD_WAVES / (nw_ * nr);
    return g_ > cap ? (cap < 1 ? 1 : cap) : g_;
  };
#define XP(a, b)                                                                                 \
  if (k4 == a && nbk == b) {                                                                     \
     \
     \
    constexpr bool big = (a * b >= 32);                                                          \
    constexpr int NWB = (a * b > 128) ? 4 : (big ? 8 : 4);                                       \
    gx_ = cap_grid(grid_for_nw(max_rows, (a * b > 128) ? 1 : (big ? ((a * b <= 32) ? 2 : 1) : 4), NWB), NWB); \
    nwv = NWB;                                                                                   \
    gw_tabs = gx_ * (fmlp_bf_wg_reduce(a, b, NWB) ? 1 : NWB);                                    \
    const dim3 grid((unsigned)gx_, (unsigned)nr);                                                \
    if (g_fmlp_mode == 3)                                                                        \
      bwd_kernel_bf<a, b, true, NWB, false, true><<<grid, NWB * 64, 0, stream>>>(                \
          nullptr, h, 0, 0, am, scale, bias, slope, c1, c2, c3, xprev, K, pre_am, pre_scale,     \
          pre_bias, pre_slope, W, gx, gwp, pstp, rt, perm, pos_seg, gout, arg);                  \
    else                                                                                         \
      bwd_kernel_bf<a, b, true, NWB, true, true><<<grid, NWB * 64, 0, stream>>>(                 \
          nullptr, h, 0, 0, am, scale, bias, slope, c1, c2, c3, xprev, K, pre_am, pre_scale,     \
          pre_bias, pre_slope, W, gx, gwp, pstp, rt, perm, pos_seg, gout, arg);                  \
  }
#define X(a, b)                                                                                  \
  if (k4 == a && nbk == b) {                                                                     \
    constexpr bool big = (a * b >= 32);                 \
    constexpr int NWV = big ? 8 : 4;                                                             \
             \
                                \
     \
     \
    constexpr int NWB = (a * b > 128) ? 4 : NWV;                                                 \
    if (g_fmlp_split_bf16) {                                                                     \
      gx_ = cap_grid(grid_for_nw(max_rows, (a * b > 128) ? 1 : (big ? ((a * b <= 32) ? 2 : 1) : 4), NWB), NWB); \
      nwv = NWB;                                                                                 \
      gw_tabs = gx_ * (fmlp_bf_wg_reduce(a, b, NWB) ? 1 : NWB);                                  \
    } else {                                                                                     \
      gx_ = cap_grid(grid_for_nw(max_rows, big ? ((a * b <= 32) ? 2 : 1) : 4, NWV), NWV);        \
      nwv = NWV;                                                                                 \
      gw_tabs = gx_ * NWV;                                                                       \
    }                                                                                            \
    const dim3 grid((unsigned)gx_, (unsigned)nr);                                                \
     \
     \
    constexpr bool PIPE_ = (a * b > 128);             \
    if (PIPE_ && K % 4 == 0 && g_fmlp_mode == 3 && gx)                                           \
      bwd_kernel_bf<a, b, true, NWB, false, false, PIPE_><<<grid, NWB * 64, 0, stream>>>(        \
          gy, h, 0, 0, am, scale, bias, slope, c1, c2, c3, xprev, K, pre_am, pre_scale,          \
          pre_bias, pre_slope, W, gx, gwp, pstp, rt);                                            \
    else if (PIPE_ && K % 4 == 0 && g_fmlp_split_bf16 && gx)                                     \
      bwd_kernel_bf<a, b, true, NWB, true, false, PIPE_><<<grid, NWB * 64, 0, stream>>>(         \
          gy, h, 0, 0, am, scale, bias, slope, c1, c2, c3, xprev, K, pre_am, pre_scale,          \
          pre_bias, pre_slope, W, gx, gwp, pstp, rt);                                            \
    else if (g_fmlp_mode == 3 && gx)                                                             \
      bwd_kernel_bf<a, b, true, NWB, false><<<grid, NWB * 64, 0, stream>>>(                      \
          gy, h, 0, 0, am, scale, bias, slope, c1, c2, c3, xprev, K, pre_am, pre_scale,          \
          pre_bias, pre_slope, W, gx, gwp, pstp, rt);                                            \
    else if (g_fmlp_mode == 3)                                                                   \
      bwd_kernel_bf<a, b, false, NWB, false><<<grid, NWB * 64, 0, stream>>>(                     \
          gy, h, 0, 0, am, scale, bias, slope, c1, c2, c3, xprev, K, pre_am, pre_scale,          \
          pre_bias, pre_slope, W, nullptr, gwp, nullptr, rt);                                    \
    else if (g_fmlp_split_bf16 && gx)                                                            \
      bwd_kernel_bf<a, b, true, NWB, true><<<grid, NWB * 64, 0, stream>>>(                       \
          gy, h, 0, 0, am, scale, bias, slope, c1, c2, c3, xprev, K, pre_am, pre_scale,          \
          pre_bias, pre_slope, W, gx, gwp, pstp, rt);                                            \
    else if (g_fmlp_split_bf16)                                                                  \
      bwd_kernel_bf<a, b, false, NWB, true><<<grid, NWB * 64, 0, stream>>>(                      \
          gy, h, 0, 0, am, scale, bias, slope, c1, c2, c3, xprev, K, pre_am, pre_scale,          \
          pre_bias, pre_slope, W, nullptr, gwp, nullptr, rt);                                    \
    else if (gx)                                                                                 \
      bwd_kernel<a, b, true, NWV, big><<<grid, NWV * 64, 0, stream>>>(                           \
          gy, h, 0, 0, am, scale, bias, slope, c1, c2, c3, xprev, K, pre_am, pre_scale,          \
          pre_bias, pre_slope, W, gx, gwp, pstp, rt);                                            \
    else                                                                                         \
      bwd_kernel<a, b, false, NWV, big><<<grid, NWV * 64, 0, stream>>>(                          \
          gy, h, 0, 0, am, scale, bias, slope, c1, c2, c3, xprev, K, pre_am, pre_scale,          \
          pre_bias, pre_slope, W, nullptr, gwp, nullptr, rt);                                    \
  }
  int per_run = 0;
  int gw_tabs = 0;
  const bool h16 = mode >= 0 && (mode & SPT_FMLP_H_BF16), x16 = mode >= 0 && (mode & SPT_FMLP_X_BF16);
  if (h16 || x16) {
    SPT_CHECK_ARG(g_fmlp_mode == 3 && h16 && spt_fused_linear_storage_supported(K, N) &&
                  (!x16 || K % 16 == 0),
                  "bf16 activation storage: bf16 matrix mode, a built shape, h stored as bf16");
#define XSP(a, b)                                                                                \
  if (pooled && k4 == a && nbk == b) {                                                           \
    constexpr bool big = (a * b >= 32);                                                          \
    constexpr int NWB = (a * b > 128) ? 4 : (big ? 8 : 4);                                       \
    gx_ = cap_grid(grid_for_nw(max_rows, (a * b > 128) ? 1 : (big ? ((a * b <= 32) ? 2 : 1) : 4), NWB), NWB); \
    nwv = NWB;                                                                                   \
    gw_tabs = gx_ * (fmlp_bf_wg_reduce(a, b, NWB) ? 1 : NWB);                                    \
    const dim3 grid((unsigned)gx_, (unsigned)nr);                                                \
    if (x16)                                                                                     \
      bwd_kernel_bf<a, b, true, NWB, false, true, false, true, true><<<grid, NWB * 64, 0, stream>>>( \
          nullptr, h, 0, 0, am, scale, bias, slope, c1, c2, c3, xprev, K, pre_am, pre_scale,     \
          pre_bias, pre_slope, W, gx, gwp, pstp, rt, perm, pos_seg, gout, arg);                  \
    else                                                                                         \
      bwd_kernel_bf<a, b, true, NWB, false, true, false, true, false><<<grid, NWB * 64, 0, stream>>>( \
          nullptr, h, 0, 0, am, scale, bias, slope, c1, c2, c3, xprev, K, pre_am, pre_scale,     \
          pre_bias, pre_slope, W, gx, gwp, pstp, rt, perm, pos_seg, gout, arg);                  \
  }
#define XSD(a, b)                                                                                \
  if (!pooled && k4 == a && nbk == b) {                                                          \
    constexpr bool big = (a * b >= 32);                                                          \
    constexpr int NWV = big ? 8 : 4;                                                             \
    constexpr int NWB = (a * b > 128) ? 4 : NWV;                                                 \
    gx_ = cap_grid(grid_for_nw(max_rows, (a * b > 128) ? 1 : (big ? ((a * b <= 32) ? 2 : 1) : 4), NWB), NWB); \
    nwv = NWB;                                                                                   \
    gw_tabs = gx_ * (fmlp_bf_wg_reduce(a, b, NWB) ? 1 : NWB);                                    \
    const dim3 grid((unsigned)gx_, (unsigned)nr);                                                \
    if (gx && x16)                                                                               \
      bwd_kernel_bf<a, b, true, NWB, false, false, false, true, true><<<grid, NWB * 64, 0, stream>>>( \
          gy, h, 0, 0, am, scale, bias, slope, c1, c2, c3, xprev, K, pre_am, pre_scale,          \
          pre_bias, pre_slope, W, gx, gwp, pstp, rt);                                            \
    else if (gx)                                                                                 \
      bwd_kernel_bf<a, b, true, NWB, false, false, false, true, false><<<grid, NWB * 64, 0, stream>>>( \
          gy, h, 0, 0, am, scale, bias, slope, c1, c2, c3, xprev, K, pre_am, pre_scale,          \
          pre_bias, pre_slope, W, gx, gwp, pstp, rt);                                            \
    else if (x16)                                                                                \
      bwd_kernel_bf<a, b, false, NWB, false, false, false, true, true><<<grid, NWB * 64, 0, stream>>>( \
          gy, h, 0, 0, am, scale, bias, slope, c1, c2, c3, xprev, K, pre_am, pre_scale,          \
          pre_bias, pre_slope, W, nullptr, gwp, nullptr, rt);                                    \
    else                                                                                         \
      bwd_kernel_bf<a, b, false, NWB, false, false, false, true, false><<<grid, NWB * 64, 0, stream>>>( \
          gy, h, 0, 0, am, scale, bias, slope, c1, c2, c3, xprev, K, pre_am, pre_scale,          \
          pre_bias, pre_slope, W, nullptr, gwp, nullptr, rt);                                    \
  }
    if (x16 && gx && fmlp_dma_of(mode) && fmlp_dma_supported(K, N)) {
      per_run = fmlp_dma_bwd_launch(pooled, false, gy, h, rt, max_rows, N, am, scale, bias, slope, c1,
                                    c2, c3, xprev, K, pre_am, pre_scale, pre_bias, pre_slope, W, gx,
                                    gwp, pstp, perm, pos_seg, gout, arg, stream, true, &gw_tabs);
    } else {
      SPT_FMLP_ST_POOLED_SHAPES(XSP)
      SPT_FMLP_ST_SHAPES(XSD)
      per_run = gx_ * nwv;
    }
#undef XSP
#undef XSD
  } else if (g_fmlp_split_bf16 && gx && fmlp_dma_of(mode) && fmlp_dma_supported(K, N)) {
    per_run = fmlp_dma_bwd_launch(pooled, g_fmlp_mode != 3, gy, h, rt, max_rows, N, am, scale, bias,
                                  slope, c1, c2, c3, xprev, K, pre_am, pre_scale, pre_bias, pre_slope,
                                  W, gx, gwp, pstp, perm, pos_seg, gout, arg, stream, false, &gw_tabs);
  } else if (pooled) {
    SPT_FMLP_POOLED_SHAPES(XP)
    per_run = gx_ * nwv;
  } else {
    SPT_FMLP_SHAPES(X)
    per_run = gx_ * nwv;
  }
#undef X
#undef XP
  SPT_CHECK_ARG(per_run > 0, "no kernel for this shape");
  bwd_post_launch(gwp, gw_tabs * nr, N * K, gW, accumulate, pst, fmlp_groups(rt, num_graphs, per_run), K,
                  num_graphs, prev_total, prev_norm, stream);
  SPT_CHECK_LAUNCH();
  return 0;
}

extern "C" int spt_fused_linear_bwd_pooled_f32(
    const float* gout, const int32_t* arg, const int32_t* perm, const int32_t* pos_seg,
    const float* h, int64_t p0, int64_t p1, int N, const float* am, const float* scale,
    const float* bias, float slope, const float* c1, const float* c2, const float* c3,
    const float* xprev, int K, const float* pre_am, const float* pre_scale, const float* pre_bias,
    float pre_slope, const float* W, float* gx, float* gW, int accumulate, double* prev_total,
    void* ws, size_t ws_bytes, spt_stream_t stream_) {
  return spt_fused_linear_bwd_pooled_ex_f32(gout, arg, perm, pos_seg, h, p0, p1, N, am, scale, bias,
                                            slope, c1, c2, c3, xprev, K, pre_am, pre_scale, pre_bias,
                                            pre_slope, W, gx, gW, accumulate, prev_total, -1, ws,
                                            ws_bytes, stream_);
}
extern "C" int spt_fused_linear_bwd_pooled_ex_f32(
    const float* gout, const int32_t* arg, const int32_t* perm, const int32_t* pos_seg,
    const float* h, int64_t p0, int64_t p1, int N, const float* am, const float* scale,
    const float* bias, float slope, const float* c1, const float* c2, const float* c3,
    const float* xprev, int K, const float* pre_am, const float* pre_scale, const float* pre_bias,
    float pre_slope, const float* W, float* gx, float* gW, int accumulate, double* prev_total,
    int mode, void* ws, size_t ws_bytes, spt_stream_t stream_) {
  SPT_CHECK_ARG(p1 >= p0, "bad shape");
  FmlpRuns rt;
  rt.n = 1; rt.g[0] = 0; rt.r0[0] = p0; rt.r1[0] = p1;
  return fmlp_bwd_impl(true, nullptr, gout, arg, perm, pos_seg, h, rt, p1 - p0, 1, N, am, scale, bias,
                       slope, c1, c2, c3, xprev, K, pre_am, pre_scale, pre_bias, pre_slope, W, gx, gW,
                       accumulate, prev_total, mode, ws, ws_bytes, (hipStream_t)stream_);
}
extern "C" int spt_fused_linear_bwd_pooled_runs_f32(
    const float* gout, const int32_t* arg, const int32_t* perm, const int32_t* pos_seg,
    const float* h, int nruns, const int64_t* run_p0, const int64_t* run_p1,
    const int32_t* run_graph, int num_graphs, int N, const float* am, const float* scale,
    const float* bias, float slope, const float* c1, const float* c2, const float* c3,
    const float* xprev, int K, const float* pre_am, const float* pre_scale, const float* pre_bias,
    float pre_slope, const float* W, float* gx, float* gW, double* prev_total, int mode, void* ws,
    size_t ws_bytes, spt_stream_t stream_) {
  FmlpRuns rt;
  int64_t max_rows;
  const char* err = fmlp_make_runs(nruns, run_p0, run_p1, run_graph, num_graphs, &rt, &max_rows);
  SPT_CHECK_ARG(!err, err ? err : "");
  return fmlp_bwd_impl(true, nullptr, gout, arg, perm, pos_seg, h, rt, max_rows, num_graphs, N, am,
                       scale, bias, slope, c1, c2, c3, xprev, K, pre_am, pre_scale, pre_bias,
                       pre_slope, W, gx, gW, 0, prev_total, mode, ws, ws_bytes, (hipStream_t)stream_);
}
extern "C" int spt_fused_linear_bwd_pooled_runs_gn_f32(
    const float* gout, const int32_t* arg, const int32_t* perm, const int32_t* pos_seg,
    const float* h, int nruns, const int64_t* run_p0, const int64_t* run_p1,
    const int32_t* run_graph, int num_graphs, int N, const float* am, const float* scale,
    const float* bias, float slope, const float* c1, const float* c2, const float* c3,
    const float* xprev, int K, const float* pre_am, const float* pre_scale, const float* pre_bias,
    float pre_slope, const float* W, float* gx, float* gW, double* prev_total, int mode, void* ws,
    size_t ws_bytes, const spt_gn_bwd_tables* prev_norm, spt_stream_t stream_) {
  FmlpRuns rt;
  int64_t max_rows;
  const char* err = fmlp_make_runs(nruns, run_p0, run_p1, run_graph, num_graphs, &rt, &max_rows);
  SPT_CHECK_ARG(!err, err ? err : "");
  SPT_CHECK_ARG(prev_norm, "null norm descriptor");
  return fmlp_bwd_impl(true, nullptr, gout, arg, perm, pos_seg, h, rt, max_rows, num_graphs, N, am,
                       scale, bias, slope, c1, c2, c3, xprev, K, pre_am, pre_scale, pre_bias,
                       pre_slope, W, gx, gW, 0, prev_total, mode, ws, ws_bytes, (hipStream_t)stream_,
                       prev_norm);
}

extern "C" int spt_fused_linear_bwd_f32(const float* gy, const float* h, int64_t r0, int64_t r1,
                                        int N, const float* am, const float* scale,
                                        const float* bias, float slope, const float* c1,
                                        const float* c2, const float* c3, const float* xprev,
                                        int K, const float* pre_am, const float* pre_scale,
                                        const float* pre_bias, float pre_slope, const float* W,
                                        float* gx, float* gW, int accumulate,
                                        double* prev_total, void* ws, size_t ws_bytes,
                                        spt_stream_t stream_) {
  return spt_fused_linear_bwd_ex_f32(gy, h, r0, r1, N, am, scale, bias, slope, c1, c2, c3, xprev, K,
                                     pre_am, pre_scale, pre_bias, pre_slope, W, gx, gW, accumulate,
                                     prev_total, -1, ws, ws_bytes, stream_);
}
extern "C" int spt_fused_linear_bwd_ex_f32(const float* gy, const float* h, int64_t r0, int64_t r1,
                                           int N, const float* am, const float* scale,
                                           const float* bias, float slope, const float* c1,
                                           const float* c2, const float* c3, const float* xprev,
                                           int K, const float* pre_am, const float* pre_scale,
                                           const float* pre_bias, float pre_slope, const float* W,
                                           float* gx, float* gW, int accumulate,
                                           double* prev_total, int mode, void* ws, size_t ws_bytes,
                                           spt_stream_t stream_) {
  SPT_CHECK_ARG(r1 >= r0, "bad shape");
  FmlpRuns rt;
  rt.n = 1; rt.g[0] = 0; rt.r0[0] = r0; rt.r1[0] = r1;
  return fmlp_bwd_impl(false, gy, nullptr, nullptr, nullptr, nullptr, h, rt, r1 - r0, 1, N, am, scale,
                       bias, slope, c1, c2, c3, xprev, K, pre_am, pre_scale, pre_bias, pre_slope, W,
                       gx, gW, accumulate, prev_total, mode, ws, ws_bytes, (hipStream_t)stream_);
}
extern "C" int spt_fused_linear_bwd_runs_f32(
    const float* gy, const float* h, int nruns, const int64_t* run_r0, const int64_t* run_r1,
    const int32_t* run_graph, int num_graphs, int N, const float* am, const float* scale,
    const float* bias, float slope, const float* c1, const float* c2, const float* c3,
    const float* xprev, int K, const float* pre_am, const float* pre_scale, const float* pre_bias,
    float pre_slope, const float* W, float* gx, float* gW, double* prev_total, int mode, void* ws,
    size_t ws_bytes, spt_stream_t stream_) {
  FmlpRuns rt;
  int64_t max_rows;
  const char* err = fmlp_make_runs(nruns, run_r0, run_r1, run_graph, num_graphs, &rt, &max_rows);
  SPT_CHECK_ARG(!err, err ? err : "");
  return fmlp_bwd_impl(false, gy, nullptr, nullptr, nullptr, nullptr, h, rt, max_rows, num_graphs, N,
                       am, scale, bias, slope, c1, c2, c3, xprev, K, pre_am, pre_scale, pre_bias,
                       pre_slope, W, gx, gW, 0, prev_total, mode, ws, ws_bytes, (hipStream_t)stream_);
}
extern "C" int spt_fused_linear_bwd_runs_gn_f32(
    const float* gy, const float* h, int nruns, const int64_t* run_r0, const int64_t* run_r1,
    const int32_t* run_graph, int num_graphs, int N, const float* am, const float* scale,
    const float* bias, float slope, const float* c1, const float* c2, const float* c3,
    const float* xprev, int K, const float* pre_am, const float* pre_scale, const float* pre_bias,
    float pre_slope, const float* W, float* gx, float* gW, double* prev_total, int mode, void* ws,
    size_t ws_bytes, const spt_gn_bwd_tables* prev_norm, spt_stream_t stream_) {
  FmlpRuns rt;
  int64_t max_rows;
  const char* err = fmlp_make_runs(nruns, run_r0, run_r1, run_graph, num_graphs, &rt, &max_rows);
  SPT_CHECK_ARG(!err, err ? err : "");
  SPT_CHECK_ARG(prev_norm, "null norm descriptor");
  return fmlp_bwd_impl(false, gy, nullptr, nullptr, nullptr, nullptr, h, rt, max_rows, num_graphs, N,
                       am, scale, bias, slope, c1, c2, c3, xprev, K, pre_am, pre_scale, pre_bias,
                       pre_slope, W, gx, gW, 0, prev_total, mode, ws, ws_bytes, (hipStream_t)stream_,
                       prev_norm);
}

namespace spt {
bool fpool_supported(int K, int N);
int fpool_gram_len(int K);
int fpool_fwd_launch(int prec, bool in16, const float* x, const int32_t* perm, const int32_t* pos_seg,
                     const int32_t* rowptr, const FmlpRuns& rt, int64_t max_rows, int K, int N,
                     const float* W, const float* gnw, const float* pam, const float* psc,
                     const float* pbs, float pslope, float* raw, int32_t* argpos, double* partial,
                     hipStream_t stream);
void fpool_tables_launch(int K, const double* gram, int B, const float* W, int N, int bfw,
                         const float* weight, const float* mean_scale, float eps, double* total,
                         float* mean, float* rstd, float* am, float* scale, hipStream_t stream);
void fpool_apply_launch(int K, bool in16, const int32_t* rowptr, const int32_t* perm,
                        const int64_t* seg_graph, int64_t num_seg, int N, int64_t n_rows,
                        const float* am, const float* sc, const float* bs, float slope,
                        const float* gnw, const float* x, const float* W, const float* pam,
                        const float* psc, const float* pbs, float pslope, int bfw, float* raw,
                        int32_t* argpos, int32_t* arg, float* out, hipStream_t stream);
int fpool_bwd_launch(bool lo, bool x16, const float* gout, const float* raw, const int32_t* argpos,
                     const int32_t* perm, const int32_t* pos_seg, const int64_t* seg_graph,
                     int64_t num_seg, const FmlpRuns& rt, int64_t max_rows, int num_graphs, int K,
                     int N, const float* am, const float* sc, const float* bs, float slope,
                     const float* c1, const float* c2, const float* c3, const float* xprev,
                     const float* pam, const float* psc, const float* pbs, float pslope,
                     const float* W, float* gm, float* Mbuf, float* c0buf, float* gx,
                     float* gw_partial, double* pstat_partial, int max_waves, hipStream_t stream,
                     int* gw_tabs);
void fpool_gw_dense_launch(int K, const double* gram, int B, const float* W, int N, int bfw,
                           const float* am, const float* c2, const float* c3, float* gW,
                           hipStream_t stream);
}

static int fpool_prec_of(int mode) {
  const int m = fmlp_mode_of(mode);
  if (m == 1) return g_fmlp_x3 ? 3 : 0;
  return m == 2 ? 2 : (m == 3 ? 1 : 0);
}
extern "C" int spt_fused_linear_pool_supported(int K, int N, int mode) {
  return fpool_supported(K, N) && fpool_prec_of(mode) != 0;
}
extern "C" size_t spt_fused_linear_pool_gram_len(int K) { return (size_t)fpool_gram_len(K); }
extern "C" size_t spt_fused_linear_pool_workspace_bytes(int K, int N) {
  return align_up(spt_fused_linear_workspace_bytes(K, N), 256) +
         align_up((size_t)FMLP_MAX_RUNS * (K * K + K) * 4, 256) + 256;
}

extern "C" int spt_fused_linear_fwd_pool_runs_f32(
    const void* x, const int32_t* perm, const int32_t* pos_seg, const int32_t* rowptr,
    const int64_t* seg_graph, int64_t num_seg, int64_t n_rows, int nruns, const int64_t* run_p0,
    const int64_t* run_p1, const int32_t* run_graph, int num_graphs, int K, const float* W, int N,
    const float* gn_weight, const float* gn_bias, const float* gn_mean_scale, float eps, float slope,
    const float* pre_am, const float* pre_scale, const float* pre_bias, float pre_slope, float* out,
    int32_t* arg, int32_t* argpos, float* raw, double* gram, double* total, float* mean, float* rstd,
    float* am, float* scale, int mode, void* ws, size_t ws_bytes, spt_stream_t stream_) {
  hipStream_t stream = (hipStream_t)stream_;
  FmlpRuns rt;
  int64_t max_rows;
  const char* err = fmlp_make_runs(nruns, run_p0, run_p1, run_graph, num_graphs, &rt, &max_rows);
  SPT_CHECK_ARG(!err, err ? err : "");
  const int prec = fpool_prec_of(mode);
  const bool in16 = mode >= 0 && (mode & SPT_FMLP_X_BF16);
  SPT_CHECK_ARG(fpool_supported(K, N) && prec != 0 && (!in16 || prec == 1),
                "(K, N) has no pool-fused kernel in this matrix mode");
  SPT_CHECK_ARG(x && pos_seg && rowptr && W && gn_weight && gn_bias && gn_mean_scale && pre_am &&
                pre_scale && pre_bias && out && argpos && raw && gram && mean && rstd && am && scale && ws,
                "null pointer");
  SPT_CHECK_ARG(num_seg >= 0 && n_rows >= 0 && (num_graphs == 1 || seg_graph), "bad shape");
  SPT_CHECK_ARG(ws_bytes >= spt_fused_linear_pool_workspace_bytes(K, N), "workspace too small");
  for (int r = 0; r < rt.n; ++r)
    SPT_CHECK_ARG(rt.r0[r] == (r ? rt.r1[r - 1] : 0), "runs must tile the CSR positions");
  SPT_CHECK_ARG(rt.r1[rt.n - 1] == n_rows, "runs must tile the CSR positions");
  double* partial = (double*)ws;
  const int glen = fpool_gram_len(K);
  const int gx_ = fpool_fwd_launch(prec, in16, (const float*)x, perm, pos_seg, rowptr, rt, max_rows, K, N,
                                   W, gn_weight, pre_am, pre_scale, pre_bias, pre_slope, raw, argpos,
                                   partial, stream);
  SPT_CHECK_ARG(gx_ > 0, "no kernel for this variant");
  reduce_tables_groups_kernel<double><<<dim3((glen + 15) / 16, num_graphs), 1024, 0, stream>>>(
      partial, fmlp_groups(rt, num_graphs, gx_), glen, gram);
  fpool_tables_launch(K, gram, num_graphs, W, N, prec == 1, gn_weight, gn_mean_scale, eps, total, mean,
                      rstd, am, scale, stream);
  fpool_apply_launch(K, in16, rowptr, perm, seg_graph, num_seg, N, n_rows, am, scale, gn_bias, slope,
                     gn_weight, (const float*)x, W, pre_am, pre_scale, pre_bias, pre_slope, prec == 1,
                     raw, argpos, arg, out, stream);
  SPT_CHECK_LAUNCH();
  return 0;
}

static int fpool_bwd_entry(
    const float* gout, const float* raw, const int32_t* argpos, const int32_t* perm,
    const int32_t* pos_seg, const int64_t* seg_graph, int64_t num_seg, int nruns,
    const int64_t* run_p0, const int64_t* run_p1, const int32_t* run_graph, int num_graphs, int N,
    const float* am, const float* scale, const float* bias, float slope, const float* c1,
    const float* c2, const float* c3, const void* xprev, int K, const float* pre_am,
    const float* pre_scale, const float* pre_bias, float pre_slope, const float* W,
    const double* gram, float* gm, float* gx, float* gW, double* prev_total, int mode, void* ws,
    size_t ws_bytes, spt_stream_t stream_, const spt_gn_bwd_tables* prev_norm) {
  hipStream_t stream = (hipStream_t)stream_;
  FmlpRuns rt;
  int64_t max_rows;
  const char* err = fmlp_make_runs(nruns, run_p0, run_p1, run_graph, num_graphs, &rt, &max_rows);
  SPT_CHECK_ARG(!err, err ? err : "");
  const int prec = fpool_prec_of(mode);
  const bool x16 = mode >= 0 && (mode & SPT_FMLP_X_BF16);
  SPT_CHECK_ARG(fpool_supported(K, N) && prec != 0 && (!x16 || prec == 1),
                "(K, N) has no pool-fused kernel in this matrix mode");
  SPT_CHECK_ARG(gout && raw && argpos && pos_seg && am && scale && bias && c1 && c2 && c3 && xprev &&
                pre_am && pre_scale && pre_bias && W && gram && gm && gx && gW && (prev_total || prev_norm) && ws,
                "null pointer");
  SPT_CHECK_ARG(num_seg >= 0 && (num_graphs == 1 || seg_graph), "bad shape");
  SPT_CHECK_ARG(ws_bytes >= spt_fused_linear_pool_workspace_bytes(K, N), "workspace too small");
  float* gwp = (float*)ws;
  double* pst = (double*)((char*)ws + align_up((size_t)MAX_BWD_WAVES * N * K * 4, 256));
  float* Mbuf = (float*)((char*)ws + align_up(spt_fused_linear_workspace_bytes(K, N), 256));
  float* c0buf = Mbuf + (size_t)FMLP_MAX_RUNS * K * K;
  int gw_tabs = 0;
  const int per_run = fpool_bwd_launch(prec != 1, x16, gout, raw, argpos, perm, pos_seg, seg_graph, num_seg,
                                       rt, max_rows, num_graphs, K, N, am, scale, bias, slope, c1, c2, c3,
                                       (const float*)xprev, pre_am, pre_scale, pre_bias, pre_slope, W, gm,
                                       Mbuf, c0buf, gx, gwp, pst, MAX_BWD_WAVES, stream, &gw_tabs);
  SPT_CHECK_ARG(per_run > 0, "no kernel for this variant");
  bwd_post_launch(gwp, gw_tabs * rt.n, N * K, gW, 0, pst, fmlp_groups(rt, num_graphs, per_run), K,
                  num_graphs, prev_total, prev_norm, stream);
  fpool_gw_dense_launch(K, gram, num_graphs, W, N, prec == 1, am, c2, c3, gW, stream);
  SPT_CHECK_LAUNCH();
  return 0;
}
extern "C" int spt_fused_linear_bwd_pool_runs_f32(
    const float* gout, const float* raw, const int32_t* argpos, const int32_t* perm,
    const int32_t* pos_seg, const int64_t* seg_graph, int64_t num_seg, int nruns,
    const int64_t* run_p0, const int64_t* run_p1, const int32_t* run_graph, int num_graphs, int N,
    const float* am, const float* scale, const float* bias, float slope, const float* c1,
    const float* c2, const float* c3, const void* xprev, int K, const float* pre_am,
    const float* pre_scale, const float* pre_bias, float pre_slope, const float* W,
    const double* gram, float* gm, float* gx, float* gW, double* prev_total, int mode, void* ws,
    size_t ws_bytes, spt_stream_t stream_) {
  return fpool_bwd_entry(gout, raw, argpos, perm, pos_seg, seg_graph, num_seg, nruns, run_p0, run_p1, run_graph,
                         num_graphs, N, am, scale, bias, slope, c1, c2, c3, xprev, K, pre_am, pre_scale,
                         pre_bias, pre_slope, W, gram, gm, gx, gW, prev_total, mode, ws, ws_bytes, stream_, nullptr);
}
extern "C" int spt_fused_linear_bwd_pool_runs_gn_f32(
    const float* gout, const float* raw, const int32_t* argpos, const int32_t* perm,
    const int32_t* pos_seg, const int64_t* seg_graph, int64_t num_seg, int nruns,
    const int64_t* run_p0, const int64_t* run_p1, const int32_t* run_graph, int num_graphs, int N,
    const float* am, const float* scale, const float* bias, float slope, const float* c1,
    const float* c2, const float* c3, const void* xprev, int K, const float* pre_am,
    const float* pre_scale, const float* pre_bias, float pre_slope, const float* W,
    const double* gram, float* gm, float* gx, float* gW, double* prev_total, int mode, void* ws,
    size_t ws_bytes, const spt_gn_bwd_tables* prev_norm, spt_stream_t stream_) {
  SPT_CHECK_ARG(prev_norm, "null norm descriptor");
  return fpool_bwd_entry(gout, raw, argpos, perm, pos_seg, seg_graph, num_seg, nruns, run_p0, run_p1, run_graph,
                         num_graphs, N, am, scale, bias, slope, c1, c2, c3, xprev, K, pre_am, pre_scale,
// ... 3 lines not shown
```

superpoint_transformer_amd/csrc/fused_mlp_dma.hip:

```cpp
#include <math.h>

#include "common.hpp"

#ifndef SPT_FDMA_SKIP
#define SPT_FDMA_SKIP 0
#endif

namespace spt {
namespace fdma {

typedef float f32x4 __attribute__((ext_vector_type(4)));
typedef __bf16 bf16x8 __attribute__((ext_vector_type(8)));
typedef __bf16 bf16x4 __attribute__((ext_vector_type(4)));
typedef short s16x4 __attribute__((ext_vector_type(4)));
constexpr int TR = 16;

__device__ __forceinline__ double xg_sum_d(double v) {
  v += __shfl_xor(v, 16, 64);
  v += __shfl_xor(v, 32, 64);
  return v;
}
__device__ __forceinline__ void lds_order() {
  __builtin_amdgcn_fence(__ATOMIC_RELEASE, "wavefront");
  __builtin_amdgcn_wave_barrier();
  __builtin_amdgcn_fence(__ATOMIC_ACQUIRE, "wavefront");
}
__device__ __forceinline__ void lds_dma16(const void* g, float* lds) {
#if SPT_FDMA_SKIP & 32
  return;
#endif
  const unsigned a = __builtin_amdgcn_readfirstlane(
      (unsigned)(size_t)((__attribute__((address_space(3))) void*)lds));
  asm volatile("s_mov_b32 m0, %0\n\ts_nop 0\n\tglobal_load_lds_dwordx4 %1, off"
               :: "s"(a), "v"(g) : "memory");
}
__device__ __forceinline__ void wait_vm0() {
  asm volatile("s_waitcnt vmcnt(0)" ::: "memory");
  __builtin_amdgcn_fence(__ATOMIC_ACQUIRE, "wavefront");
}
__device__ __forceinline__ void wait_lds() {
  asm volatile("s_waitcnt lgkmcnt(0)" ::: "memory");
}
__device__ __forceinline__ int opaque(int v) {
  asm volatile("" : "+v"(v));
  return v;
}
template <int NV, typename V>
__device__ __forceinline__ void split_bf16(const float (&x)[NV], V& hi, V& lo) {
#pragma unroll
  for (int i = 0; i < NV; ++i) {
    const __bf16 h = (__bf16)x[i];
    hi[i] = h;
    lo[i] = (__bf16)(x[i] - (float)h);
  }
}
template <bool LO>
__device__ __forceinline__ f32x4 mfma3_32(const bf16x8& ah, const bf16x8& al, const bf16x8& bh,
                                          const bf16x8& bl, f32x4 c) {
  if constexpr (LO) {
    c = __builtin_amdgcn_mfma_f32_16x16x32_bf16(al, bh, c, 0, 0, 0);
    c = __builtin_amdgcn_mfma_f32_16x16x32_bf16(ah, bl, c, 0, 0, 0);
  }
  return __builtin_amdgcn_mfma_f32_16x16x32_bf16(ah, bh, c, 0, 0, 0);
}
template <bool LO>
__device__ __forceinline__ f32x4 mfma3_16(const bf16x4& ah, const bf16x4& al, const bf16x4& bh,
                                          const bf16x4& bl, f32x4 c) {
  const s16x4 AH = __builtin_bit_cast(s16x4, ah), AL = __builtin_bit_cast(s16x4, al);
  const s16x4 BH = __builtin_bit_cast(s16x4, bh), BL = __builtin_bit_cast(s16x4, bl);
  if constexpr (LO) {
    c = __builtin_amdgcn_mfma_f32_16x16x16bf16_1k(AL, BH, c, 0, 0, 0);
    c = __builtin_amdgcn_mfma_f32_16x16x16bf16_1k(AH, BL, c, 0, 0, 0);
  }
  return __builtin_amdgcn_mfma_f32_16x16x16bf16_1k(AH, BH, c, 0, 0, 0);
}

template <int R>
__device__ __forceinline__ int pick_lane(int v, int base, int sel) {
  int r = __builtin_amdgcn_readlane(v, base);
#pragma unroll
  for (int j = 1; j < R; ++j) r = (sel == j) ? __builtin_amdgcn_readlane(v, base + j) : r;
  return r;
}

template <int K, int N, int NW, int OCC, bool LO, bool POOLED, bool S16 = false>
__global__ __launch_bounds__(NW * 64, OCC) void bwd_dma_kernel(
    const float* __restrict__ gy, const float* __restrict__ h, int64_t r0, int64_t r1,
    const float* __restrict__ am, const float* __restrict__ sc, const float* __restrict__ bs,
    float slope, const float* __restrict__ c1, const float* __restrict__ c2,
    const float* __restrict__ c3, const float* __restrict__ xprev,
    const float* __restrict__ pam, const float* __restrict__ psc, const float* __restrict__ pbs,
    float pslope, const float* __restrict__ W, float* __restrict__ gx,
    float* __restrict__ gw_partial, double* __restrict__ pstat_partial,
    const int32_t* __restrict__ perm, const int32_t* __restrict__ pos_seg,
    const float* __restrict__ gout, const int32_t* __restrict__ arg, FmlpRuns rt) {
  constexpr int NC = N / 4, KC = K / 4, NBK = N / 16, KB = K / 16, NS = N / 32;
  if (rt.n > 0) {
    const int run_ = blockIdx.y, gph_ = rt.g[run_];
    r0 = rt.r0[run_];
    r1 = rt.r1[run_];
    am += (size_t)gph_ * N; sc += (size_t)gph_ * N;
    c1 += (size_t)gph_ * N; c2 += (size_t)gph_ * N; c3 += (size_t)gph_ * N;
    if (pam) { pam += (size_t)gph_ * K; psc += (size_t)gph_ * K; }
    gw_partial += (size_t)run_ * gridDim.x * N * K;
    if (pstat_partial) pstat_partial += (size_t)run_ * gridDim.x * NW * (2 * K + 1);
  }
  constexpr int HI = TR * NC / 64, XI = TR * KC / 64;
  constexpr int RH = 64 / NC;
  constexpr int NSEG = RH;
  constexpr int LDT = N + 8;
  constexpr int W_H = TR * N, W_X = TR * K, W_G = POOLED ? NSEG * N : 0;
  static_assert(K % 16 == 0 && N % 32 == 0 && (TR * NC) % 64 == 0 && (TR * KC) % 64 == 0, "shape");
  __shared__ __attribute__((aligned(16))) float lw[NW][W_H + W_X + 2 * W_G];
  __shared__ __attribute__((aligned(16))) __bf16 wt_hi[K * LDT];
  __shared__ __attribute__((aligned(16))) __bf16 wt_lo[LO ? K * LDT : 8];
  __shared__ __attribute__((aligned(16))) float pt[3 * K];
  const int lane = threadIdx.x & 63;
  const int wid = __builtin_amdgcn_readfirstlane(threadIdx.x >> 6);
  const int g = lane >> 4, c = lane & 15;
  float* HB = lw[wid];
  float* XB = HB + W_H;
  float* GO = XB + W_X;
  int* AR = reinterpret_cast<int*>(GO + W_G);
  const bool pre = pam != nullptr;
  for (int i = threadIdx.x; i < K * N; i += NW * 64) {
    const int k = i / N, n = i - k * N;
    const float w = W[(size_t)n * K + k];
    const __bf16 hh = (__bf16)w;
    wt_hi[k * LDT + n] = hh;
    if constexpr (LO) wt_lo[k * LDT + n] = (__bf16)(w - (float)hh);
  }
  for (int i = threadIdx.x; i < K; i += NW * 64) {
    pt[i] = pre ? pam[i] : 0.f;
    pt[K + i] = pre ? psc[i] : 1.f;
    pt[2 * K + i] = pre ? pbs[i] : 0.f;
  }
  __syncthreads();

  f32x4 C3[NBK][KB];
#pragma unroll
  for (int nb = 0; nb < NBK; ++nb)
#pragma unroll
    for (int kb = 0; kb < KB; ++kb) C3[nb][kb] = (f32x4){0.f, 0.f, 0.f, 0.f};
  double p1[KB], p2[KB];
#pragma unroll
  for (int kb = 0; kb < KB; ++kb) p1[kb] = p2[kb] = 0.0;

  const int64_t ntiles = (r1 - r0 + TR - 1) / TR;
  const int64_t wave = (int64_t)blockIdx.x * NW + wid;
  const int64_t nwaves = (int64_t)gridDim.x * NW;

  const float4 t_am = *reinterpret_cast<const float4*>(am + 4 * (lane % NC));
  const float4 t_sc = *reinterpret_cast<const float4*>(sc + 4 * (lane % NC));
  const float4 t_bs = *reinterpret_cast<const float4*>(bs + 4 * (lane % NC));
  const float4 t_c1 = *reinterpret_cast<const float4*>(c1 + 4 * (lane % NC));
  const float4 t_c2 = *reinterpret_cast<const float4*>(c2 + 4 * (lane % NC));
  const float4 t_c3 = *reinterpret_cast<const float4*>(c3 + 4 * (lane % NC));
  int ln = opaque(lane);
  auto gh1 = [&](float hh, float gg, float aa, float ss, float bb, float q1, float q2, float q3) {
    const float o = hh - aa;
    if (slope != 1.f) {
      const float y = fmaf(o, ss, bb);
      gg = (y > 0.f) ? gg : gg * slope;
    }
    return fmaf(q1, gg, -fmaf(q2, o, q3));
  };
  auto gh_of = [&](const float4& hv, const float4& gv) {
    return make_float4(gh1(hv.x, gv.x, t_am.x, t_sc.x, t_bs.x, t_c1.x, t_c2.x, t_c3.x),
                       gh1(hv.y, gv.y, t_am.y, t_sc.y, t_bs.y, t_c1.y, t_c2.y, t_c3.y),
                       gh1(hv.z, gv.z, t_am.z, t_sc.z, t_bs.z, t_c1.z, t_c2.z, t_c3.z),
                       gh1(hv.w, gv.w, t_am.w, t_sc.w, t_bs.w, t_c1.w, t_c2.w, t_c3.w));
  };
  auto pick = [&](int v, int base) {
    const int hi = ln / NC;
    int r = __builtin_amdgcn_readlane(v, base);
#pragma unroll
    for (int j = 1; j < RH; ++j) r = (hi == j) ? __builtin_amdgcn_readlane(v, base + j) : r;
    return r;
  };
  constexpr int RX = 64 / KC;
  auto pickx = [&](int v, int base) {
    const int hx = ln / KC;
    int r = __builtin_amdgcn_readlane(v, base);
#pragma unroll
    for (int j = 1; j < RX; ++j) r = (hx == j) ? __builtin_amdgcn_readlane(v, base + j) : r;
    return r;
  };

  int rid_n = 0, seg_n = 0;
  auto load_ids = [&](int64_t t) {
    rid_n = seg_n = 0;
    const int64_t rowf = r0 + t * TR;
    if constexpr (POOLED) {
      if (t < ntiles && rowf + lane < r1 && lane < TR) {
        rid_n = perm[rowf + lane];
        seg_n = pos_seg[rowf + lane];
      }
    } else {
      if (t < ntiles && lane < TR) rid_n = (rowf + lane < r1) ? lane : 0;
    }
  };
  constexpr int NC16 = N / 8, RH16 = 64 / NC16, HI16 = TR / RH16;
  constexpr int KC16 = K / 8, RX16 = 64 / KC16, XI16 = (TR + RX16 - 1) / RX16;
  static_assert(!S16 || (TR % RH16 == 0 && RX16 <= TR), "bf16 rows: whole DMA instructions per tile");
  auto issue_h = [&](int64_t t, int rid_l, int seg_l) {
    if (t >= ntiles) return;
    const int64_t row0 = r0 + t * TR;
    const int hi = ln / NC, n4 = ln % NC;
    if constexpr (S16) {
      const uint16_t* hb = reinterpret_cast<const uint16_t*>(h) + (POOLED ? 0 : row0 * N);
      const int h16 = ln / NC16, p16 = ln % NC16;
#pragma unroll
      for (int i = 0; i < HI16; ++i)
        lds_dma16(hb + (int64_t)pick_lane<RH16>(rid_l, RH16 * i, h16) * N + 8 * p16,
                  HB + W_H / 2 + 256 * i);
    } else {
      const float* hb = POOLED ? h : h + row0 * N;
#pragma unroll
      for (int i = 0; i < HI; ++i) {
        const int rr7 = (hi + RH * i) & 7;
        lds_dma16(hb + (int64_t)pick(rid_l, RH * i) * N + 4 * (n4 ^ rr7), HB + 256 * i);
      }
    }
    if constexpr (POOLED) {
      const int cnt = (int)((r1 - row0) < TR ? (r1 - row0) : TR);
      const int s0 = __builtin_amdgcn_readlane(seg_l, 0);
      const int s1 = __builtin_amdgcn_readfirstlane(__shfl(seg_l, cnt - 1, 64));
      const int64_t sgm = (s0 + hi < s1) ? s0 + hi : s1;
      lds_dma16(gout + sgm * N + 4 * n4, GO);
      lds_dma16(arg + sgm * N + 4 * n4, reinterpret_cast<float*>(AR));
    }
  };
  auto issue_x = [&](int64_t t, int rid_l) {
    if (t >= ntiles) return;
    const int64_t row0 = r0 + t * TR;
    if constexpr (S16) {
      const uint16_t* xb = reinterpret_cast<const uint16_t*>(xprev) + (POOLED ? 0 : row0 * K);
      const int x16 = ln / KC16, q16 = ln % KC16;
#pragma unroll
      for (int i = 0; i < XI16; ++i)
        lds_dma16(xb + (int64_t)pick_lane<RX16>(rid_l, RX16 * i, x16) * K + 8 * q16,
                  XB + W_X / 2 + 256 * i);
    } else {
      const float* xb = POOLED ? xprev : xprev + row0 * K;
      const int hx = ln / KC, px = ln % KC;
#pragma unroll
      for (int i = 0; i < XI; ++i) {
        const int rr = hx + RX * i;
        lds_dma16(xb + (int64_t)pickx(rid_l, RX * i) * K + 4 * (px ^ (4 * ((rr >> 2) & 1))), XB + 256 * i);
      }
    }
  };

  load_ids(wave);
  int rid_l = rid_n, seg_l = seg_n;
  issue_h(wave, rid_l, seg_l);
  issue_x(wave, rid_l);
  load_ids(wave + nwaves);
  for (int64_t t = wave; t < ntiles; t += nwaves) {
    const int64_t row0 = r0 + t * TR;
    const int cnt = (int)((r1 - row0) < TR ? (r1 - row0) : TR);
    ln = opaque(ln);
    const int hi = ln / NC, n4 = ln % NC, hx = ln / KC, px = ln % KC, g = ln >> 4, c = ln & 15;
    float4 gyv[POOLED ? 1 : HI];
    if constexpr (!POOLED) {
#pragma unroll
      for (int i = 0; i < HI; ++i) {
        const int rr = hi + RH * i;
        gyv[i] = (rr < cnt) ? *reinterpret_cast<const float4*>(gy + (row0 + rr) * N + 4 * n4)
                            : make_float4(0.f, 0.f, 0.f, 0.f);
      }
    }
    wait_vm0();
    lds_order();
    if constexpr (S16) {
#pragma unroll
      for (int i = 0; i < XI; ++i) {
        const int rr = hx + RX * i;
        const int cx = px ^ (4 * ((rr >> 2) & 1));
        const uint2 u = *reinterpret_cast<const uint2*>(
            reinterpret_cast<const uint16_t*>(XB + W_X / 2) + rr * K + 4 * cx);
        *reinterpret_cast<float4*>(XB + rr * K + 4 * px) =
            make_float4(__uint_as_float(u.x << 16), __uint_as_float(u.x & 0xffff0000u),
                        __uint_as_float(u.y << 16), __uint_as_float(u.y & 0xffff0000u));
      }
    }
    if constexpr (!(SPT_FDMA_SKIP & 1)) {
      const int s0 = POOLED ? __builtin_amdgcn_readlane(seg_l, 0) : 0;
      const int s1 = POOLED ? __builtin_amdgcn_readfirstlane(__shfl(seg_l, cnt - 1, 64)) : 0;
      const bool in_lds = s1 - s0 < NSEG;
#pragma unroll
      for (int i = 0; i < HI; ++i) {
        const int rr = hi + RH * i;
        float* slot = HB + rr * N + 4 * (n4 ^ (rr & 7));
        float4 hv;
        if constexpr (S16) {
          const uint2 u = *reinterpret_cast<const uint2*>(
              reinterpret_cast<const uint16_t*>(HB + W_H / 2) + rr * N + 4 * n4);
          hv = make_float4(__uint_as_float(u.x << 16), __uint_as_float(u.x & 0xffff0000u),
                           __uint_as_float(u.y << 16), __uint_as_float(u.y & 0xffff0000u));
        } else {
          hv = *reinterpret_cast<const float4*>(slot);
        }
        float4 gv;
        if constexpr (POOLED) {
          const int rid = pick(rid_l, RH * i);
          const int sg = pick(seg_l, RH * i);
          int4 av;
          if (in_lds) {
            gv = *reinterpret_cast<const float4*>(GO + (sg - s0) * N + 4 * n4);
            av = *reinterpret_cast<const int4*>(AR + (sg - s0) * N + 4 * n4);
          } else {
            gv = *reinterpret_cast<const float4*>(gout + (int64_t)sg * N + 4 * n4);
            av = *reinterpret_cast<const int4*>(arg + (int64_t)sg * N + 4 * n4);
          }
          gv = make_float4(av.x == rid ? gv.x : 0.f, av.y == rid ? gv.y : 0.f,
                           av.z == rid ? gv.z : 0.f, av.w == rid ? gv.w : 0.f);
        } else {
          gv = gyv[i];
        }
        *reinterpret_cast<float4*>(slot) = gh_of(hv, gv);
      }
      if (cnt < TR) {
#pragma unroll
        for (int i = 0; i < HI; ++i) {
          const int rr = hi + RH * i;
          if (rr >= cnt)
            *reinterpret_cast<float4*>(HB + rr * N + 4 * (n4 ^ (rr & 7))) = make_float4(0.f, 0.f, 0.f, 0.f);
        }
      }
    }
    lds_order();
    if constexpr (!(SPT_FDMA_SKIP & 2)) {
      bf16x4 Xh[KB], Xl[KB];
#pragma unroll
      for (int kb = 0; kb < KB; ++kb) {
        const int k = 16 * kb + c;
        float xv[4];
#pragma unroll
        for (int r = 0; r < 4; ++r) {
          float v = XB[(4 * g + r) * K + 4 * ((4 * kb + (c >> 2)) ^ (4 * (g & 1))) + (c & 3)];
          if (pre) {
            v = fmaf(v - pt[k], pt[K + k], pt[2 * K + k]);
            v = (v > 0.f) ? v : v * pslope;
          }
          xv[r] = v;
        }
        split_bf16<4>(xv, Xh[kb], Xl[kb]);
      }
#pragma unroll
      for (int nb = 0; nb < NBK; ++nb) {
        float gv[4];
#pragma unroll
        for (int r = 0; r < 4; ++r)
          gv[r] = HB[(4 * g + r) * N + 4 * ((4 * nb + (c >> 2)) ^ (4 * (g & 1) + r)) + (c & 3)];
        bf16x4 gh4, gl4;
        split_bf16<4>(gv, gh4, gl4);
#pragma unroll
        for (int kb = 0; kb < KB; ++kb) C3[nb][kb] = mfma3_16<LO>(gh4, gl4, Xh[kb], Xl[kb], C3[nb][kb]);
      }
    }
    f32x4 CX[KB];
#pragma unroll
    for (int kb = 0; kb < KB; ++kb) CX[kb] = (f32x4){0.f, 0.f, 0.f, 0.f};
    if constexpr (!(SPT_FDMA_SKIP & 4)) {
#pragma unroll
      for (int sg = 0; sg < NS; ++sg) {
        const float4 a0 = *reinterpret_cast<const float4*>(HB + c * N + 4 * ((8 * sg + 2 * g) ^ (c & 7)));
        const float4 a1 = *reinterpret_cast<const float4*>(HB + c * N + 4 * ((8 * sg + 2 * g + 1) ^ (c & 7)));
        const float av[8] = {a0.x, a0.y, a0.z, a0.w, a1.x, a1.y, a1.z, a1.w};
        bf16x8 ah, alo;
        split_bf16<8>(av, ah, alo);
#pragma unroll
        for (int kb = 0; kb < KB; ++kb) {
          const bf16x8 bh = *reinterpret_cast<const bf16x8*>(wt_hi + (16 * kb + c) * LDT + 32 * sg + 8 * g);
          bf16x8 bl = bh;
          if constexpr (LO) bl = *reinterpret_cast<const bf16x8*>(wt_lo + (16 * kb + c) * LDT + 32 * sg + 8 * g);
          CX[kb] = mfma3_32<LO>(ah, alo, bh, bl, CX[kb]);
        }
      }
    }
    const int rid_cur = rid_l;
    wait_lds();
    issue_h(t + nwaves, rid_n, seg_n);
#pragma unroll
    for (int kb = 0; kb < KB; ++kb) {
      const int k = 16 * kb + c;
#pragma unroll
      for (int r = 0; r < 4; ++r) {
        float* xs = XB + (4 * g + r) * K + 4 * ((4 * kb + (c >> 2)) ^ (4 * (g & 1))) + (c & 3);
        const float v = CX[kb][r];
        if (!(SPT_FDMA_SKIP & 8) && pre) {
          const float o = *xs - pt[k];
          float gg = v;
          if (pslope != 1.f) {
            const float y = fmaf(o, pt[K + k], pt[2 * K + k]);
            gg = (y > 0.f) ? gg : gg * pslope;
          }
          p1[kb] += (double)gg;
          p2[kb] += (double)gg * (double)o;
        }
        *xs = v;
      }
    }
    lds_order();
#pragma unroll
    for (int i = 0; i < XI; ++i) {
      const int rr = hx + RX * i;
      const float4 v = *reinterpret_cast<const float4*>(XB + rr * K + 4 * px);
      const int64_t orow = POOLED ? (int64_t)pickx(rid_cur, RX * i) : row0 + rr;
      if (!(SPT_FDMA_SKIP & 16) && rr < cnt)
        *reinterpret_cast<float4*>(gx + orow * K + 4 * (px ^ (4 * ((rr >> 2) & 1)))) = v;
    }
    wait_lds();
    issue_x(t + nwaves, rid_n);
    rid_l = rid_n;
    seg_l = seg_n;
    load_ids(t + 2 * nwaves);
  }
  wait_vm0();
  {
    constexpr int LDR = K + 4;
    static_assert(N * LDR <= NW * (W_H + W_X + 2 * W_G), "the table fits the tile buffers");
    __syncthreads();
    float* red = &lw[0][0];
    for (int w = 1; w < NW; ++w) {
      if (wid == w) {
#pragma unroll
        for (int nb = 0; nb < NBK; ++nb)
#pragma unroll
          for (int kb = 0; kb < KB; ++kb)
#pragma unroll
            for (int r = 0; r < 4; ++r) red[(16 * nb + 4 * g + r) * LDR + 16 * kb + c] = C3[nb][kb][r];
      }
      __syncthreads();
      if (wid == 0) {
#pragma unroll
        for (int nb = 0; nb < NBK; ++nb)
#pragma unroll
          for (int kb = 0; kb < KB; ++kb)
#pragma unroll
            for (int r = 0; r < 4; ++r) C3[nb][kb][r] += red[(16 * nb + 4 * g + r) * LDR + 16 * kb + c];
      }
      __syncthreads();
    }
  }
  if (wid == 0) {
    float* gwp = gw_partial + (size_t)blockIdx.x * N * K;
#pragma unroll
    for (int nb = 0; nb < NBK; ++nb)
#pragma unroll
      for (int kb = 0; kb < KB; ++kb)
#pragma unroll
        for (int r = 0; r < 4; ++r)
          gwp[(size_t)(16 * nb + 4 * g + r) * K + 16 * kb + c] = C3[nb][kb][r];
  }
  if (pstat_partial) {
    double* pp = pstat_partial + (size_t)wave * (2 * K + 1);
#pragma unroll
    for (int kb = 0; kb < KB; ++kb) {
      const double a = xg_sum_d(p1[kb]), b = xg_sum_d(p2[kb]);
      if (g == 0) {
        pp[16 * kb + c] = a;
        pp[K + 16 * kb + c] = b;
      }
    }
    if (lane == 0) pp[2 * K] = (wave == 0) ? (double)(r1 - r0) : 0.0;
  }
}

}

bool fmlp_dma_supported(int K, int N) {
  return (K == 64 && N == 128) || (K == 32 && N == 64) || (K == 64 && N == 64);
}

int fmlp_dma_bwd_launch(bool pooled, bool lo, const float* gy, const float* h, FmlpRuns rt,
                        int64_t max_rows, int N, const float* am, const float* sc, const float* bs,
                        float slope, const float* c1, const float* c2, const float* c3,
                        const float* xprev, int K, const float* pam, const float* psc,
                        const float* pbs, float pslope, const float* W, float* gx,
                        float* gw_partial, double* pstat_partial, const int32_t* perm,
                        const int32_t* pos_seg, const float* gout, const int32_t* arg,
                        hipStream_t stream, bool s16, int* gw_tabs) {
  using namespace fdma;
  const int64_t tiles = (max_rows + TR - 1) / TR;
  const int nr = rt.n < 1 ? 1 : rt.n;
#define SPT_DMA_CASE(KK, NN, NWV, PER_CU, OCC)                                                        \
  if (K == KK && N == NN) {                                                                        \
    int64_t blocks = (tiles + NWV - 1) / NWV;                                                      \
                                      \
    const int64_t cap = (256 * PER_CU) / nr > 1 ? (256 * PER_CU) / nr : 1;                         \
    if (blocks > cap) blocks = cap;                                                                \
    if (blocks < 1) blocks = 1;                                                                    \
    const dim3 grid((unsigned)blocks, (unsigned)nr);                                               \
    if (s16 && pooled)                                                                             \
      bwd_dma_kernel<KK, NN, NWV, OCC, false, true, true><<<grid, NWV * 64, 0, stream>>>(          \
          gy, h, 0, 0, am, sc, bs, slope, c1, c2, c3, xprev, pam, psc, pbs, pslope, W, gx,         \
          gw_partial, pstat_partial, perm, pos_seg, gout, arg, rt);                                \
    else if (s16)                                                                                  \
      bwd_dma_kernel<KK, NN, NWV, OCC, false, false, true><<<grid, NWV * 64, 0, stream>>>(         \
          gy, h, 0, 0, am, sc, bs, slope, c1, c2, c3, xprev, pam, psc, pbs, pslope, W, gx,         \
          gw_partial, pstat_partial, perm, pos_seg, gout, arg, rt);                                \
    else if (pooled && lo)                                                                              \
      bwd_dma_kernel<KK, NN, NWV, OCC, true, true><<<grid, NWV * 64, 0, stream>>>(                      \
          gy, h, 0, 0, am, sc, bs, slope, c1, c2, c3, xprev, pam, psc, pbs, pslope, W, gx,         \
          gw_partial, pstat_partial, perm, pos_seg, gout, arg, rt);                                \
    else if (pooled)                                                                               \
      bwd_dma_kernel<KK, NN, NWV, OCC, false, true><<<grid, NWV * 64, 0, stream>>>(                     \
          gy, h, 0, 0, am, sc, bs, slope, c1, c2, c3, xprev, pam, psc, pbs, pslope, W, gx,         \
          gw_partial, pstat_partial, perm, pos_seg, gout, arg, rt);                                \
    else if (lo)                                                                                   \
      bwd_dma_kernel<KK, NN, NWV, OCC, true, false><<<grid, NWV * 64, 0, stream>>>(                     \
          gy, h, 0, 0, am, sc, bs, slope, c1, c2, c3, xprev, pam, psc, pbs, pslope, W, gx,         \
          gw_partial, pstat_partial, perm, pos_seg, gout, arg, rt);                                \
    else                                                                                           \
      bwd_dma_kernel<KK, NN, NWV, OCC, false, false><<<grid, NWV * 64, 0, stream>>>(                    \
          gy, h, 0, 0, am, sc, bs, slope, c1, c2, c3, xprev, pam, psc, pbs, pslope, W, gx,         \
          gw_partial, pstat_partial, perm, pos_seg, gout, arg, rt);                                \
    if (gw_tabs) *gw_tabs = (int)blocks;                                                           \
    return (int)blocks * NWV;                                                                      \
  }
  SPT_DMA_CASE(64, 128, 8, 1, 2)
  SPT_DMA_CASE(64, 64, 8, 1, 2)
  SPT_DMA_CASE(32, 64, 8, 2, 4)
#undef SPT_DMA_CASE
  return 0;
}

}
```

superpoint_transformer_amd/ops.py:

```python
import contextlib
import ctypes
import os

import torch

from . import _lib
from . import precision as _precision
from .csr import EdgeCSR, SegmentCSR, csr_of, edge_csr_of

_OPS = {"sum": 0, "add": 0, "mean": 1, "min": 2, "max": 3}

_TIMERS = {}
_TIMER_PREFIXES = []
_TIMER_CAP = 8192


def enable_timer(name, prefix=False):
    _TIMERS[name] = []
    if prefix and name not in _TIMER_PREFIXES:
        _TIMER_PREFIXES.append(name)


def timer_count(name):
    return len(_TIMERS.get(name) or [])
# ... 1326 lines not shown
    def rows_per_graph(self):
        out = [0] * self.B
        for a, b, g in zip(self.r0, self.r1, self.g):
            out[g] += b - a
        return out


def graph_runs(batch, num_graphs, rows):
    if batch is None or (num_graphs is not None and int(num_graphs) == 1):
        return GraphRuns([(0, rows, 0)], 1, rows)
    B = int(num_graphs)
    if B > MAX_FUSED_RUNS:
        return None
    memo = getattr(batch, _GRUN_ATTR, None)
    key = (batch._version, B, batch.data_ptr(), batch.numel())
    if memo is not None and memo[0] == key:
        return memo[1]
    runs = None
    hp = _host_ptr(batch, B)
    if batch.numel() == 0:
        runs = GraphRuns([], B, 0)
    elif hp is not None:
        runs = GraphRuns([(hp[g], hp[g + 1], g) for g in range(B) if hp[g + 1] > hp[g]], B,
                         batch.numel())
    else:
        change = (batch[1:] != batch[:-1])
        n_change = int(change.sum())
        if n_change + 1 <= MAX_FUSED_RUNS:
            starts = [0] + (torch.nonzero(change).flatten() + 1).tolist()
            ends = starts[1:] + [int(batch.numel())]
            ids = batch[torch.tensor(starts, device=batch.device)].tolist()
            if all(0 <= g < B for g in ids):
                runs = GraphRuns(list(zip(starts, ends, ids)), B, batch.numel())
    try:
        setattr(batch, _GRUN_ATTR, (key, runs))
    except Exception:
        pass
    return runs


_GRUN_ATTR = "_spt_graph_runs"


def graph_runs_via(batch, num_graphs, holder, *deps):
    key = tuple((d._version, d.data_ptr(), d.numel()) for d in deps) + (int(num_graphs),)
    memo = getattr(holder, _GRUN_ATTR + "_via", None)
    host = getattr(holder, "_spt_host_runs", None)
    if memo is not None and memo[0] == key:
        runs = memo[1]
    elif (host is not None and holder._version == 0 and host[0] == (int(num_graphs), batch.numel())
          and len(host[1]) <= MAX_FUSED_RUNS):
        runs = GraphRuns(list(host[1]), int(num_graphs), batch.numel())
    else:
        runs = graph_runs(batch, num_graphs, batch.numel())
        try:
            setattr(holder, _GRUN_ATTR + "_via", (key, runs))
        except Exception:
            pass
    try:
        setattr(batch, _GRUN_ATTR, ((batch._version, int(num_graphs), batch.data_ptr(), batch.numel()), runs))
    except Exception:
        pass
    return runs


def fused_mlp_supported(dims):
    return all(_lib.lib.spt_fused_linear_supported(int(k), int(n))
               for k, n in zip(dims[:-1], dims[1:]))


_ST_H, _ST_X = 8, 16


def _fmlp_forward(x, batch, runs, eps_list, slope_list, params, apply_last=True, fmode=-1,
                  store16=False):
    L = len(eps_list)
    Ws = [params[4 * i].detach().float().contiguous() for i in range(L)]
    gnw = [params[4 * i + 1].detach().float().contiguous() for i in range(L)]
    gnb = [params[4 * i + 2].detach().float().contiguous() for i in range(L)]
    gms = [params[4 * i + 3].detach().float().contiguous() for i in range(L)]
    x2 = x.detach().contiguous()
    if x2.dtype != torch.float32:
        x2 = x2.float()
    R = x2.shape[0]
    dev = x2.device
    B = runs.B
    nr, c_r0, c_r1, c_g = runs.c_arrays()
    sp = _lib.stream_ptr(dev)
    hs, tabs = [], []
    cur, pre = x2, None
    y = None
    with torch.cuda.device(dev):
        for l in range(L):
            N, K = Ws[l].shape
            h = torch.empty((R, N), dtype=torch.bfloat16 if store16 else torch.float32, device=dev)
            lmode = (3 | _ST_H | (_ST_X if l else 0)) if store16 else fmode
            total = torch.empty((B, 2 * N + 1), dtype=torch.float64, device=dev)
            nb = _lib.lib.spt_fused_linear_workspace_bytes(K, N)
            ws = _workspace(nb, dev)
            pa = ps = pb = None
            if pre is not None:
                pa, ps, pb = pre
            mean = torch.empty((B, N), dtype=torch.float32, device=dev)
            rstd, am, sc = (torch.empty_like(mean) for _ in range(3))
            if FUSE_POST:
                norm = _lib.GnFwdTables(_lib.ptr(gnw[l]), _lib.ptr(gms[l]), float(eps_list[l]),
                                        _lib.ptr(mean), _lib.ptr(rstd), _lib.ptr(am), _lib.ptr(sc))
                with _timed(f"fused_linear_fwd:{K}x{N}:{R}"):
                    st = _lib.lib.spt_fused_linear_fwd_runs_gn_f32(
                        _lib.ptr(cur), nr, c_r0, c_r1, c_g, B, K, _lib.ptr(Ws[l]), N,
                        _lib.ptr(pa), _lib.ptr(ps), _lib.ptr(pb),
                        float(slope_list[l - 1]) if l else 1.0, _lib.ptr(h),
                        _lib.ptr(total), lmode, _lib.ptr(ws), ws.numel(), ctypes.addressof(norm), sp)
                _lib.check(st, "spt_fused_linear_fwd_runs_gn_f32")
            else:
                with _timed(f"fused_linear_fwd:{K}x{N}:{R}"):
                    st = _lib.lib.spt_fused_linear_fwd_runs_f32(
                        _lib.ptr(cur), nr, c_r0, c_r1, c_g, B, K, _lib.ptr(Ws[l]), N,
                        _lib.ptr(pa), _lib.ptr(ps), _lib.ptr(pb),
                        float(slope_list[l - 1]) if l else 1.0, _lib.ptr(h),
                        _lib.ptr(total), lmode, _lib.ptr(ws), ws.numel(), sp)
                _lib.check(st, "spt_fused_linear_fwd_runs_f32")
                st = _lib.lib.spt_graphnorm_tables_f32(
                    _lib.ptr(total), B, N, _lib.ptr(gnw[l]), _lib.ptr(gms[l]), float(eps_list[l]),
                    _lib.ptr(mean), _lib.ptr(rstd), _lib.ptr(am), _lib.ptr(sc), sp)
                _lib.check(st, "spt_graphnorm_tables_f32")
            hs.append(h)
            tabs.append((mean, rstd, am, sc))
            cur, pre = h, (am, sc, gnb[l])
        if apply_last:
            assert not store16, "bf16 storage: the last norm is applied by the consumer (the pool)"
            N = Ws[-1].shape[0]
            y = torch.empty((R, N), dtype=torch.float32, device=dev)
            st = _lib.lib.spt_graphnorm_apply_f32(
                _lib.ptr(hs[-1]), _lib.ptr(batch) if B > 1 else None, R, N, B,
                _lib.ptr(tabs[-1][2]), _lib.ptr(tabs[-1][3]), _lib.ptr(gnb[-1]),
                float(slope_list[-1]), _lib.ptr(y), sp)
            _lib.check(st, "spt_graphnorm_apply_f32")
    saved = (x2, batch, *hs, *[t for tab in tabs for t in tab], *Ws, *gnw, *gnb, *gms)
    return y, saved, hs[-1], (tabs[-1][2], tabs[-1][3], gnb[-1])


FUSE_POST = os.environ.get("SPT_FUSE_POST", "1") != "0"


def fuse_post(on=None):
    global FUSE_POST
    old = FUSE_POST
    if on is not None:
        FUSE_POST = bool(on)
    return old


def _fmlp_backward(saved, meta, gy, top_total=None, pooled=None, top_tabs=None):
    L, runs, slopes, in_dtype, need_gx0 = meta[:5]
    fmode = meta[5] if len(meta) > 5 else -1
    store16 = bool(meta[6]) if len(meta) > 6 else False
    sv = list(saved)
    x2, batch = sv[0], sv[1]
    hs = sv[2:2 + L]
    tabs = [tuple(sv[2 + L + 4 * i: 2 + L + 4 * i + 4]) for i in range(L)]
    o = 2 + 5 * L
    Ws, gnw, gnb, gms = sv[o:o + L], sv[o + L:o + 2 * L], sv[o + 2 * L:o + 3 * L], sv[o + 3 * L:o + 4 * L]
    R = x2.shape[0]
    dev = x2.device
    B = runs.B
    nr, c_r0, c_r1, c_g = runs.c_arrays()
    sp = _lib.stream_ptr(dev)
    g_cur = gy.contiguous().float() if gy is not None else None
    grads = [None] * (4 * L)
    gx0 = None
    with torch.cuda.device(dev):
        N = Ws[-1].shape[0]
        mean, rstd, am, sc = tabs[-1]
        if top_tabs is not None:
            total = None
        elif top_total is not None:
            total = top_total
        else:
            assert not store16, "bf16 storage: the top statistics come from the sparse route"
            total = torch.empty((B, 2 * N + 1), dtype=torch.float64, device=dev)
            ws = _workspace(_lib.lib.spt_graphnorm_workspace_bytes(R, N, B), dev)
            st = _lib.lib.spt_graphnorm_bwd_stats_f32(
                _lib.ptr(hs[-1]), _lib.ptr(g_cur), _lib.ptr(batch) if B > 1 else None, R, N, B,
                _lib.ptr(am), _lib.ptr(sc), _lib.ptr(gnb[-1]), float(slopes[-1]), _lib.ptr(total),
                _lib.ptr(ws), ws.numel(), sp)
            _lib.check(st, "spt_graphnorm_bwd_stats_f32")
        cur_tabs = top_tabs
        for l in range(L - 1, -1, -1):
            N, K = Ws[l].shape
            mean, rstd, am, sc = tabs[l]
            if cur_tabs is not None:
                c1, c2, c3, gw_n, gb_n, ga_n = cur_tabs
            else:
                c1, c2, c3 = (torch.empty((B, N), dtype=torch.float32, device=dev) for _ in range(3))
                gw_n, gb_n, ga_n = (torch.empty(N, dtype=torch.float32, device=dev) for _ in range(3))
                st = _lib.lib.spt_graphnorm_bwd_tables_f32(
                    _lib.ptr(total), B, N, _lib.ptr(gnw[l]), _lib.ptr(gms[l]), _lib.ptr(mean),
                    _lib.ptr(rstd), _lib.ptr(c1), _lib.ptr(c2), _lib.ptr(c3), _lib.ptr(gw_n),
                    _lib.ptr(gb_n), _lib.ptr(ga_n), sp)
                _lib.check(st, "spt_graphnorm_bwd_tables_f32")
            xprev = hs[l - 1] if l else x2
            pre = tabs[l - 1] if l else None
            want_gx = l > 0 or need_gx0
            gx = torch.empty((R, K), dtype=torch.float32, device=dev) if want_gx else None
            gW = torch.empty((N, K), dtype=torch.float32, device=dev)
            nxt_tabs, pn = None, None
            if l and FUSE_POST:
                nxt_tabs = (*(torch.empty((B, K), dtype=torch.float32, device=dev) for _ in range(3)),
                            *(torch.empty(K, dtype=torch.float32, device=dev) for _ in range(3)))
                pn = _lib.GnBwdTables(_lib.ptr(gnw[l - 1]), _lib.ptr(gms[l - 1]), _lib.ptr(tabs[l - 1][0]),
                                      _lib.ptr(tabs[l - 1][1]), *[_lib.ptr(t) for t in nxt_tabs])
            ptot = (torch.empty((B, 2 * K + 1), dtype=torch.float64, device=dev)
                    if (l and pn is None) else None)
            ws = _workspace(_lib.lib.spt_fused_linear_workspace_bytes(K, N), dev)
            pa = ps = pb = None
            if pre is not None:
                pa, ps, pb = pre[2], pre[3], gnb[l - 1]
            lmode = (3 | _ST_H | (_ST_X if l else 0)) if store16 else fmode
            if pooled is not None and l == L - 1:
                p_gout, p_arg, p_csr = pooled
                args = (_lib.ptr(p_gout), _lib.ptr(p_arg), _lib.ptr(p_csr.perm),
                        _lib.ptr(p_csr.pos_seg()), _lib.ptr(hs[l]), nr, c_r0, c_r1, c_g, B, N,
                        _lib.ptr(am), _lib.ptr(sc), _lib.ptr(gnb[l]), float(slopes[l]),
                        _lib.ptr(c1), _lib.ptr(c2), _lib.ptr(c3), _lib.ptr(xprev), K,
                        _lib.ptr(pa), _lib.ptr(ps), _lib.ptr(pb),
                        float(slopes[l - 1]) if l else 1.0, _lib.ptr(Ws[l]), _lib.ptr(gx),
                        _lib.ptr(gW), _lib.ptr(ptot), lmode, _lib.ptr(ws), ws.numel())
                with _timed(f"fused_linear_bwd_pooled:{K}x{N}:{R}"):
                    if pn is not None:
                        st = _lib.lib.spt_fused_linear_bwd_pooled_runs_gn_f32(*args, ctypes.addressof(pn), sp)
                    else:
                        st = _lib.lib.spt_fused_linear_bwd_pooled_runs_f32(*args, sp)
                _lib.check(st, "spt_fused_linear_bwd_pooled_runs_f32")
            else:
                args = (_lib.ptr(g_cur), _lib.ptr(hs[l]), nr, c_r0, c_r1, c_g, B, N,
                        _lib.ptr(am), _lib.ptr(sc), _lib.ptr(gnb[l]), float(slopes[l]),
                        _lib.ptr(c1), _lib.ptr(c2), _lib.ptr(c3), _lib.ptr(xprev), K,
                        _lib.ptr(pa), _lib.ptr(ps), _lib.ptr(pb),
                        float(slopes[l - 1]) if l else 1.0, _lib.ptr(Ws[l]), _lib.ptr(gx),
                        _lib.ptr(gW), _lib.ptr(ptot), lmode, _lib.ptr(ws), ws.numel())
                if pn is not None:
                    st = _lib.lib.spt_fused_linear_bwd_runs_gn_f32(*args, ctypes.addressof(pn), sp)
                else:
                    st = _lib.lib.spt_fused_linear_bwd_runs_f32(*args, sp)
                _lib.check(st, "spt_fused_linear_bwd_runs_f32")
            grads[4 * l], grads[4 * l + 1], grads[4 * l + 2], grads[4 * l + 3] = gW, gw_n, gb_n, ga_n
            if l:
                g_cur, total, cur_tabs = gx, ptot, nxt_tabs
            else:
                gx0 = gx
    return (None if gx0 is None else gx0.to(in_dtype)), grads


class _FusedMLP(torch.autograd.Function):

    @staticmethod
    def forward(ctx, x, batch, runs, eps_list, slope_list, *params):
        fmode = _precision.fused_mode()
        y, saved, _, _ = _fmlp_forward(x, batch, runs, eps_list, slope_list, params, fmode=fmode)
        ctx.save_for_backward(*saved)
        ctx.meta = (len(eps_list), runs, list(slope_list), x.dtype, x.requires_grad, fmode)
        return y.to(x.dtype)

    @staticmethod
    def backward(ctx, gy):
        gx0, grads = _fmlp_backward(ctx.saved_tensors, ctx.meta, gy)
        return (gx0, None, None, None, None, *grads)


POOL_RAW_OUTPUT = True

POOL_IN_FORWARD = os.environ.get("SPT_POOL_IN_FORWARD", "1") != "0"


def pool_in_forward(on=None):
    global POOL_IN_FORWARD
    prev = POOL_IN_FORWARD
    if on is not None:
        POOL_IN_FORWARD = bool(on)
    return prev


class _FusedMLPMaxPool(torch.autograd.Function):

    @staticmethod
    def forward(ctx, x, batch, runs, eps_list, slope_list, csr, seg_graph, *params):
        fmode = _precision.fused_mode()
        L = len(eps_list)
        dims = [params[0].shape[1]] + [params[4 * i].shape[0] for i in range(L)]
        store16 = bool(
            _precision.bf16_activation_storage()
            and all(_lib.lib.spt_fused_linear_storage_supported(int(k), int(n))
                    for k, n in zip(dims[:-1], dims[1:]))
            and all(int(k) % 32 == 0 for k in dims[1:-1])
            and 256 % int(dims[-1]) == 0
            and _lib.lib.spt_segcsr_max_affine_bf16_supported(int(dims[-1]), x.shape[0]))
        ctx.pool_fused = False
        mode_top = (3 | _ST_X) if store16 else fmode
        if (POOL_IN_FORWARD and L > 1 and runs.sorted_batch
                and _lib.lib.spt_fused_linear_pool_supported(int(dims[-2]), int(dims[-1]), mode_top)
                and (runs.B == 1 or graph_ranges(seg_graph, runs.B, csr.num_seg) is not None)):
            return _FusedMLPMaxPool._forward_pooled(ctx, x, batch, runs, eps_list, slope_list, csr,
                                                    seg_graph, params, fmode, store16, mode_top)
        _, saved, h_last, (am, sc, bs) = _fmlp_forward(x, batch, runs, eps_list, slope_list,
                                                        params, apply_last=False, fmode=fmode,
                                                        store16=store16)
        R, N = h_last.shape
        dev = h_last.device
        out = torch.empty((csr.num_seg, N), dtype=torch.float32, device=dev)
        arg = torch.empty((csr.num_seg, N), dtype=torch.int32, device=dev)
        raw = None
        if (POOL_RAW_OUTPUT and any(ctx.needs_input_grad) and N <= 256 and 256 % N == 0
                and _lib.lib.spt_segcsr_max_affine_raw_supported(int(N), R)):
            raw = torch.empty((csr.num_seg, N), dtype=torch.float32, device=dev)
        with torch.cuda.device(dev), _timed(f"segcsr_reduce_fwd:3:{R}x{N}"):
            if raw is not None:
                st = _lib.lib.spt_segcsr_max_affine_raw_f32(
                    _lib.ptr(h_last), 1 if store16 else 0, _lib.ptr(csr.perm), _lib.ptr(csr.rowptr),
                    R, csr.num_seg, N, _lib.ptr(am), _lib.ptr(sc), _lib.ptr(bs),
                    float(slope_list[-1]), _lib.ptr(seg_graph), _lib.ptr(out), _lib.ptr(arg),
                    _lib.ptr(raw), _lib.stream_ptr(dev))
            else:
                seg_max = (_lib.lib.spt_segcsr_max_affine_bf16 if store16
                           else _lib.lib.spt_segcsr_max_affine_f32)
                st = seg_max(
                    _lib.ptr(h_last), _lib.ptr(csr.perm), _lib.ptr(csr.rowptr), R, csr.num_seg, N,
                    _lib.ptr(am), _lib.ptr(sc), _lib.ptr(bs), float(slope_list[-1]),
                    _lib.ptr(seg_graph), _lib.ptr(out), _lib.ptr(arg), _lib.stream_ptr(dev))
        _lib.check(st, "spt_segcsr_max_affine")
        ctx.has_raw = raw is not None
        if raw is not None:
            ctx.save_for_backward(arg, *saved, raw)
        else:
            ctx.save_for_backward(arg, *saved)
        ctx.csr = csr
        ctx.seg_graph = seg_graph
        ctx.meta = (len(eps_list), runs, list(slope_list), x.dtype, x.requires_grad,
                    3 if store16 else fmode, store16)
        return out.to(x.dtype)

    @staticmethod
    def _forward_pooled(ctx, x, batch, runs, eps_list, slope_list, csr, seg_graph, params, fmode,
                        store16, mode_top):
        L = len(eps_list)
        _, saved_sub, h_prev, (pam, psc, pbs) = _fmlp_forward(
            x, batch, runs, eps_list[:L - 1], slope_list[:L - 1], params[:4 * (L - 1)],
            apply_last=False, fmode=fmode, store16=store16)
        W = params[4 * (L - 1)].detach().float().contiguous()
        gnw, gnb, gms = (params[4 * (L - 1) + i].detach().float().contiguous() for i in (1, 2, 3))
        N, K = W.shape
        R = h_prev.shape[0]
        dev = h_prev.device
        B = runs.B
        S = csr.num_seg
        nr, c_r0, c_r1, c_g = runs.c_arrays()
        out = torch.empty((S, N), dtype=torch.float32, device=dev)
        arg = None
        argpos = torch.empty((S, N), dtype=torch.int32, device=dev)
        raw = torch.empty((S, N), dtype=torch.float32, device=dev)
        glen = int(_lib.lib.spt_fused_linear_pool_gram_len(K))
        gram = torch.empty((B, glen), dtype=torch.float64, device=dev)
        mean, rstd, am, sc = (torch.empty((B, N), dtype=torch.float32, device=dev) for _ in range(4))
        nb = _lib.lib.spt_fused_linear_pool_workspace_bytes(K, N)
        ws = _workspace(nb, dev)
        with torch.cuda.device(dev), _timed(f"fused_linear_fwd_pool:{K}x{N}:{R}"):
            st = _lib.lib.spt_fused_linear_fwd_pool_runs_f32(
                _lib.ptr(h_prev), _lib.ptr(csr.perm), _lib.ptr(csr.pos_seg()), _lib.ptr(csr.rowptr),
                _lib.ptr(seg_graph), S, R, nr, c_r0, c_r1, c_g, B, K, _lib.ptr(W), N,
                _lib.ptr(gnw), _lib.ptr(gnb), _lib.ptr(gms), float(eps_list[-1]),
                float(slope_list[-1]), _lib.ptr(pam), _lib.ptr(psc), _lib.ptr(pbs),
                float(slope_list[-2]), _lib.ptr(out), _lib.ptr(arg), _lib.ptr(argpos), _lib.ptr(raw),
# ... 159 lines not shown
```

Measured before the change: 348.2.

## Fold bottom MLP layer's weight gradient into layer-1 backward via per-graph moment tables

When backpropagating through layer 1 of a fused MLP whose input x0 is narrow (K0=12), the change skips writing gx for layer 1 and the separate layer-0 backward pass. Instead the kernel accumulates per-workgroup moment tables (gg·[x0-shift,1] and the Gram of [x0-shift,1]) with split-bf16 MFMAs. A post kernel then reconstructs gW0 and the GroupNorm parameter grads algebraically from those tables, using a per-graph shift computed from up to 4096 rows to limit cancellation. This removes a full R×K gradient write/read and one bwd kernel, at the cost of extra MFMA work per tile, more LDS, and numerical risk from the algebraic reconstruction.

```diff
diff --git a/include/spt_hip.h b/include/spt_hip.h
--- a/include/spt_hip.h
+++ b/include/spt_hip.h
@@ -544,6 +544,15 @@
     const float* xprev, int K, const float* pre_am, const float* pre_scale, const float* pre_bias,
     float pre_slope, const float* W, float* gx, float* gW, double* prev_total, int mode, void* ws,
     size_t ws_bytes, const spt_gn_bwd_tables* prev_norm, spt_stream_t stream);
+int spt_fused_linear_bwd_fold_supported(int K0, int K, int N, int mode);
+int spt_fused_linear_bwd_runs_gn_fold_f32(
+    const float* gy, const float* h, int nruns, const int64_t* run_r0, const int64_t* run_r1,
+    const int32_t* run_graph, int num_graphs, int N, const float* am, const float* scale,
+    const float* bias, float slope, const float* c1, const float* c2, const float* c3,
+    const float* xprev, int K, const float* pre_am, const float* pre_scale, const float* pre_bias,
+    float pre_slope, const float* W, float* gW, int mode, void* ws, size_t ws_bytes,
+    const spt_gn_bwd_tables* prev_norm, const float* x0, int K0, const float* W0, float* gW0,
+    spt_stream_t stream);
 int spt_fused_linear_bwd_pooled_runs_gn_f32(
     const float* gout, const int32_t* arg, const int32_t* perm, const int32_t* pos_seg,
     const float* h, int nruns, const int64_t* run_p0, const int64_t* run_p1,
diff --git a/superpoint_transformer_amd/_lib.py b/superpoint_transformer_amd/_lib.py
--- a/superpoint_transformer_amd/_lib.py
+++ b/superpoint_transformer_amd/_lib.py
@@ -146,6 +146,10 @@
     "spt_fused_linear_bwd_runs_gn_f32": (_int, [_p, _p, _int, _p, _p, _p, _int, _int, _p, _p, _p, _f32,
                                                 _p, _p, _p, _p, _int, _p, _p, _p, _f32, _p, _p, _p, _p,
                                                 _int, _p, _sz, _p, _p]),
+    "spt_fused_linear_bwd_fold_supported": (_int, [_int, _int, _int, _int]),
+    "spt_fused_linear_bwd_runs_gn_fold_f32": (_int, [_p, _p, _int, _p, _p, _p, _int, _int, _p, _p, _p, _f32,
+                                                     _p, _p, _p, _p, _int, _p, _p, _p, _f32, _p, _p,
+                                                     _int, _p, _sz, _p, _p, _int, _p, _p, _p]),
     "spt_fused_linear_bwd_pooled_runs_gn_f32": (_int, [_p, _p, _p, _p, _p, _int, _p, _p, _p, _int, _int,
                                                        _p, _p, _p, _f32, _p, _p, _p, _p, _int, _p, _p,
                                                        _p, _f32, _p, _p, _p, _p, _int, _p, _sz, _p, _p]),
diff --git a/superpoint_transformer_amd/csrc/fused_mlp.hip b/superpoint_transformer_amd/csrc/fused_mlp.hip
--- a/superpoint_transformer_amd/csrc/fused_mlp.hip
+++ b/superpoint_transformer_amd/csrc/fused_mlp.hip
@@ -813,8 +813,10 @@
 __host__ __device__ constexpr bool fmlp_bf_wg_reduce(int K4, int NBK, int NW) {
   return NBK * 16 <= NW * TR && K4 > 0;
 }
+constexpr int fold_zp(int K0) { return (K0 + 16) / 16 * 16; }
+constexpr int FOLD_SHIFT_LD = 32;
 template <int K4, int NBK, bool NEED_GX, int NW, bool LO, bool POOLED = false, bool PIPE = false,
-          bool H16 = false, bool X16 = false>
+          bool H16 = false, bool X16 = false, int FK0 = 0>
 __global__ __launch_bounds__(NW * 64, NW / 4) void bwd_kernel_bf(
     const float* __restrict__ gy, const float* __restrict__ h, int64_t r0, int64_t r1,
     const float* __restrict__ am, const float* __restrict__ sc, const float* __restrict__ bs,
@@ -824,12 +826,27 @@
     float pslope, const float* __restrict__ W, float* __restrict__ gx,
     float* __restrict__ gw_partial, double* __restrict__ pstat_partial, FmlpRuns rt,
     const int32_t* __restrict__ perm = nullptr, const int32_t* __restrict__ pos_seg = nullptr,
-    const float* __restrict__ gout = nullptr, const int32_t* __restrict__ arg = nullptr) {
+    const float* __restrict__ gout = nullptr, const int32_t* __restrict__ arg = nullptr,
+    const float* __restrict__ x0 = nullptr, const float* __restrict__ fshift = nullptr,
+    float* __restrict__ fold_partial = nullptr) {
   constexpr int KP = K4 * 4, KB = (KP + 15) / 16, KPP = KB * 16, N = NBK * 16;
   constexpr int NS = (N + 31) / 32, NP32 = NS * 32;
   constexpr int LDG = NP32 + 4, LDX = KPP + 4, LDT = NP32 + 8;
   constexpr bool WGR = fmlp_bf_wg_reduce(K4, NBK, NW);
+  constexpr bool FOLD = FK0 > 0;
+  constexpr int ZP = fold_zp(FOLD ? FK0 : 1), ZB = ZP / 16, LDZ = ZP + 4, FLN = (KPP + ZP) * ZP;
+  static_assert(!FOLD || (WGR && NEED_GX && !POOLED && !PIPE && !H16 && !X16 && KP == KPP && ZP <= 32),
+                "the fold: dense f32 rows, one table per workgroup");
+  static_assert(!FOLD || FLN <= NW * TR * LDX, "the fold table fits the x tile buffers");
   SPT_FMLP_RUN_BWD_T(N, NW, (WGR ? 1 : NW))
+  if constexpr (FOLD) {
+    if (rt.n > 0) {
+      fshift += (size_t)rt.g[blockIdx.y] * FOLD_SHIFT_LD;
+      fold_partial += (size_t)blockIdx.y * gridDim.x * FLN;
+    }
+  }
+  __shared__ __attribute__((aligned(16))) float z_lds[FOLD ? NW : 1][FOLD ? TR * LDZ : 4];
+  __shared__ float fsh[32];
   __shared__ __attribute__((aligned(16))) float g_lds[NW][TR * LDG];
   __shared__ __attribute__((aligned(16))) float x_lds[NW][TR * LDX];
   __shared__ __attribute__((aligned(16))) __bf16 wt_hi[NEED_GX ? KPP * LDT : 8];
@@ -862,8 +879,20 @@
   load_table(pt + 2 * KPP, pbs, K, KPP);
   for (int i = lane; i < TR * LDX; i += 64) xl[i] = 0.f;
   for (int i = lane; i < TR * LDG; i += 64) gl[i] = 0.f;
+  if constexpr (FOLD) {
+    if (threadIdx.x < 32) fsh[threadIdx.x] = (int)threadIdx.x < FK0 ? fshift[threadIdx.x] : 0.f;
+  }
+  float* zl = z_lds[FOLD ? wid : 0];
   __syncthreads();
 
+  f32x4 FA[FOLD ? KB : 1][ZB], FG[FOLD ? ZB : 1][ZB];
+#pragma unroll
+  for (int zb = 0; zb < ZB; ++zb) {
+#pragma unroll
+    for (int kb = 0; kb < (FOLD ? KB : 1); ++kb) FA[kb][zb] = (f32x4){0.f, 0.f, 0.f, 0.f};
+#pragma unroll
+    for (int za = 0; za < (FOLD ? ZB : 1); ++za) FG[za][zb] = (f32x4){0.f, 0.f, 0.f, 0.f};
+  }
   f32x4 C3[NBK][KB];
 #pragma unroll
   for (int nb = 0; nb < NBK; ++nb)
@@ -1020,6 +1049,8 @@
       FM_PROBE(0)
       stage_tile<KPP, LDX, KPP, POOLED, (POOLED && NBK >= 8) ? 2 : 4, X16>(xprev, row0, cnt, K, false, pt,
                                                                              pslope, xl, nullptr, lane, rid_l);
+      if constexpr (FOLD)
+        stage_tile<ZP, LDZ, ZP>(x0, row0, cnt, FK0, false, pt, pslope, zl, nullptr, lane);
       FM_PROBE(1)
     }
     const int rid_cur = rid_l;
@@ -1088,6 +1119,13 @@
         CX[kb] = mfma3_32<LO>(ah, alo, bfh[step % (LAB + 1)], bfl[step % (LAB + 1)], CX[kb]);
         if constexpr (LAB > 0) __builtin_amdgcn_sched_barrier(0);
       }
+      float ggv[FOLD ? KB : 1][4];
+      if constexpr (FOLD) {
+#pragma unroll
+        for (int kb = 0; kb < KB; ++kb)
+#pragma unroll
+          for (int r = 0; r < 4; ++r) ggv[kb][r] = 0.f;
+      }
 #pragma unroll
       for (int r = 0; r < 4; ++r) {
         const int rr = 4 * g + r;
@@ -1098,7 +1136,7 @@
             const int k = 16 * kb + c;
             if (k < K) {
               const float v = CX[kb][r];
-              gx[orow * K + k] = v;
+              if constexpr (!FOLD) gx[orow * K + k] = v;
               if (pre) {
                 const float o = xl[rr * LDX + k] - pt[k];
                 float gg = v;
@@ -1108,10 +1146,38 @@
                 }
                 p1[kb] += (double)gg;
                 p2[kb] += (double)gg * (double)o;
+                if constexpr (FOLD) ggv[kb][r] = gg;
               }
             }
           }
         }
+      }
+      if constexpr (FOLD) {
+        bf16x4 Zh[ZB], Zl[ZB];
+#pragma unroll
+        for (int zb = 0; zb < ZB; ++zb) {
+          const int col = 16 * zb + c;
+          float zv[4];
+#pragma unroll
+          for (int r = 0; r < 4; ++r) {
+            const float raw = zl[(4 * g + r) * LDZ + col];
+            const float in = (col < FK0) ? raw - fsh[col] : ((col == FK0) ? 1.f : 0.f);
+            zv[r] = (4 * g + r < cnt) ? in : 0.f;
+          }
+          split_bf16<4>(zv, Zh[zb], Zl[zb]);
+        }
+#pragma unroll
+        for (int kb = 0; kb < KB; ++kb) {
+          bf16x4 ah, al;
+          split_bf16<4>(ggv[kb], ah, al);
+#pragma unroll
+          for (int zb = 0; zb < ZB; ++zb) FA[kb][zb] = mfma3_16<LO>(ah, al, Zh[zb], Zl[zb], FA[kb][zb]);
+        }
+#pragma unroll
+        for (int za = 0; za < ZB; ++za)
+#pragma unroll
+          for (int zb = 0; zb < ZB; ++zb)
+            FG[za][zb] = mfma3_16<LO>(Zh[za], Zl[za], Zh[zb], Zl[zb], FG[za][zb]);
       }
     }
     FM_PROBE(4)
@@ -1145,6 +1211,47 @@
             for (int r = 0; r < 4; ++r) C3[nb][kb][r] += red[(16 * nb + 4 * g + r) * LDX + 16 * kb + c];
       }
       __syncthreads();
+    }
+  }
+  if constexpr (FOLD) {
+    float* red = &x_lds[0][0];
+    for (int w = 1; w < NW; ++w) {
+      if (wid == w) {
+#pragma unroll
+        for (int zb = 0; zb < ZB; ++zb)
+#pragma unroll
+          for (int r = 0; r < 4; ++r) {
+#pragma unroll
+            for (int kb = 0; kb < KB; ++kb) red[(16 * kb + 4 * g + r) * ZP + 16 * zb + c] = FA[kb][zb][r];
+#pragma unroll
+            for (int za = 0; za < ZB; ++za) red[(KPP + 16 * za + 4 * g + r) * ZP + 16 * zb + c] = FG[za][zb][r];
+          }
+      }
+      __syncthreads();
+      if (wid == 0) {
+#pragma unroll
+        for (int zb = 0; zb < ZB; ++zb)
+#pragma unroll
+          for (int r = 0; r < 4; ++r) {
+#pragma unroll
+            for (int kb = 0; kb < KB; ++kb) FA[kb][zb][r] += red[(16 * kb + 4 * g + r) * ZP + 16 * zb + c];
+#pragma unroll
+            for (int za = 0; za < ZB; ++za) FG[za][zb][r] += red[(KPP + 16 * za + 4 * g + r) * ZP + 16 * zb + c];
+          }
+      }
+      __syncthreads();
+    }
+    if (wid == 0) {
+      float* fp = fold_partial + (size_t)blockIdx.x * FLN;
+#pragma unroll
+      for (int zb = 0; zb < ZB; ++zb)
+#pragma unroll
+        for (int r = 0; r < 4; ++r) {
+#pragma unroll
+          for (int kb = 0; kb < KB; ++kb) fp[(16 * kb + 4 * g + r) * ZP + 16 * zb + c] = FA[kb][zb][r];
+#pragma unroll
+          for (int za = 0; za < ZB; ++za) fp[(KPP + 16 * za + 4 * g + r) * ZP + 16 * zb + c] = FG[za][zb][r];
+        }
     }
   }
   if (!WGR || wid == 0) {
@@ -1226,8 +1333,8 @@
                         total + (size_t)b * len, 0);
 }
 
-template <int NV>
-__device__ __forceinline__ void sliced_col_sums(const double* const (&base)[NV], const int (&ntab)[NV],
+template <int NV, typename T = double, int UNRF = 0>
+__device__ __forceinline__ void sliced_col_sums(const T* const (&base)[NV], const int (&ntab)[NV],
                                                 int len, const int (&col)[NV], double (*sl)[17],
                                                 double (&out)[NV]) {
   const int cl = threadIdx.x & 15, slice = threadIdx.x >> 4;
@@ -1243,30 +1350,30 @@
     const int n = hi[v] - lo[v];
     kmax = n > kmax ? n : kmax;
   }
-  constexpr int UNR = NV <= 3 ? 4 : 1;
+  constexpr int UNR = UNRF > 0 ? UNRF : (NV <= 3 ? 4 : 1);
   int k = 0;
   if constexpr (UNR > 1)
   for (; k + UNR <= kmax; k += UNR) {
-    double t[NV][UNR];
+    T t[NV][UNR];
 #pragma unroll
     for (int j = 0; j < UNR; ++j)
 #pragma unroll
       for (int v = 0; v < NV; ++v)
-        t[v][j] = (lo[v] + k + j < hi[v]) ? base[v][(size_t)(lo[v] + k + j) * len + col[v]] : 0.0;
+        t[v][j] = (lo[v] + k + j < hi[v]) ? base[v][(size_t)(lo[v] + k + j) * len + col[v]] : (T)0;
 #pragma unroll
     for (int j = 0; j < UNR; ++j)
 #pragma unroll
       for (int v = 0; v < NV; ++v)
-        if (lo[v] + k + j < hi[v]) acc[v] += t[v][j];
+        if (lo[v] + k + j < hi[v]) acc[v] += (double)t[v][j];
   }
   for (; k < kmax; ++k) {
-    double t[NV];
+    T t[NV];
 #pragma unroll
     for (int v = 0; v < NV; ++v)
-      t[v] = (lo[v] + k < hi[v]) ? base[v][(size_t)(lo[v] + k) * len + col[v]] : 0.0;
+      t[v] = (lo[v] + k < hi[v]) ? base[v][(size_t)(lo[v] + k) * len + col[v]] : (T)0;
 #pragma unroll
     for (int v = 0; v < NV; ++v)
-      if (lo[v] + k < hi[v]) acc[v] += t[v];
+      if (lo[v] + k < hi[v]) acc[v] += (double)t[v];
   }
 #pragma unroll
   for (int v = 0; v < NV; ++v) {
@@ -1323,14 +1430,111 @@
 }
 
 constexpr int POST_GB = 2;
+struct FmlpFold {
+  const float* tabs;
+  const float* shift;
+  const float* W0;
+  const float* am0;
+  float* gW0;
+  int K0, ZP, first;
+  FmlpGroups grp;
+};
+__device__ __forceinline__ void bwd_post_fold(const double* __restrict__ pst, const FmlpGroups& grp,
+                                              int K, int B, const spt_gn_bwd_tables& pn,
+                                              const FmlpFold& fd, int bx) {
+  __shared__ double sl[64][17];
+  __shared__ double gk[32], sxs[32];
+  const int cl = threadIdx.x & 15, slice = threadIdx.x >> 4;
+  const int K0 = fd.K0, ZP = fd.ZP, cb = bx / K0, k = bx - cb * K0;
+  const int c = cb * 16 + cl, len = 2 * K + 1, flen = (K + ZP) * ZP;
+  const bool cv = c < K;
+  double acc = 0.0;
+  for (int b = 0; b < B; ++b) {
+    double s3[3], f3[3], Af = 0.0;
+    const float* ft = fd.tabs + (size_t)fd.grp.start[b] * flen;
+    const float* const fbase[3] = {ft, ft, ft};
+    const int fnt[3] = {fd.grp.count[b], fd.grp.count[b], fd.grp.count[b]};
+#pragma unroll 1
+    for (int jb = 0; jb < ZP / 16; ++jb) {
+      const int jrow = 16 * jb + cl;
+      const int fcol[3] = {(cv && jb == 0) ? c * ZP + k : -1, (K + jrow) * ZP + k, (K + jrow) * ZP + K0};
+      sliced_col_sums<3, float, 1>(fbase, fnt, flen, fcol, sl, f3);
+      if (slice == 0) {
+        gk[jrow] = f3[1];
+        sxs[jrow] = f3[2];
+      }
+      if (jb == 0) Af = f3[0];
+    }
+    const double* pb = pst + (size_t)grp.start[b] * len;
+    const double* const base[3] = {pb, pb, pb};
+    const int ntab[3] = {grp.count[b], grp.count[b], grp.count[b]};
+    const int col[3] = {cv ? c : -1, cv ? K + c : -1, 2 * K};
+    sliced_col_sums<3, double, 1>(base, ntab, len, col, sl, s3);
+    if (slice == 0 && cv) {
+      const double w = (double)pn.weight[c], a = (double)pn.mean_scale[c];
+      const double A = s3[0], GO = s3[1], cnt = s3[2];
+      double n = cnt;
+      if (n < 1.0) n = 1.0;
+      const double sd = (double)pn.rstd[b * K + c], mu = (double)pn.mean[b * K + c];
+      const double k2 = w * sd * sd * sd * GO / n;
+      const double sumdo = w * sd * A - k2 * n * mu * (1.0 - a);
+      const double q1 = (double)(float)(w * sd), q2 = (double)(float)k2, q3 = (double)(float)(a * sumdo / n);
+      const double s = (double)fd.shift[b * FOLD_SHIFT_LD + k];
+      double d = -(double)fd.am0[b * K + c], wg = 0.0, ws = 0.0;
+      for (int j = 0; j < K0; ++j) {
+        const double wj = (double)fd.W0[(size_t)c * K0 + j];
+        d += wj * (double)fd.shift[b * FOLD_SHIFT_LD + j];
+        wg += wj * gk[j];
+        ws += wj * sxs[j];
+      }
+      const double so = ws + cnt * d;
+      const double Bm = wg + d * sxs[k] + so * s;
+      acc += q1 * (Af + A * s) - q2 * Bm - q3 * (sxs[k] + cnt * s);
+    }
+    __syncthreads();
+  }
+  if (slice == 0 && cv) fd.gW0[(size_t)c * K0 + k] = (float)acc;
+}
+__global__ __launch_bounds__(1024) void fold_shift_kernel(const float* __restrict__ x0, int K0,
+                                                          FmlpRuns rt, float* __restrict__ shift) {
+  __shared__ float sl[32][33];
+  const int b = blockIdx.x, cl = threadIdx.x & 31, slice = threadIdx.x >> 5;
+  int64_t r0 = 0, r1 = 0;
+  for (int r = rt.n - 1; r >= 0; --r)
+    if (rt.g[r] == b && rt.r1[r] > rt.r0[r]) { r0 = rt.r0[r]; r1 = rt.r1[r]; }
+  if (r1 - r0 > 4096) r1 = r0 + 4096;
+  float acc = 0.f;
+  if (cl < K0) {
+    int64_t i = r0 + slice;
+    for (; i + 7 * 32 < r1; i += 8 * 32) {
+      float t[8];
+#pragma unroll
+      for (int u = 0; u < 8; ++u) t[u] = x0[(i + 32 * u) * K0 + cl];
+#pragma unroll
+      for (int u = 0; u < 8; ++u) acc += t[u];
+    }
+    for (; i < r1; i += 32) acc += x0[i * K0 + cl];
+  }
+  sl[slice][cl] = acc;
+  __syncthreads();
+  if (slice == 0) {
+    double t = 0;
+    for (int k = 0; k < 32; ++k) t += (double)sl[k][cl];
+    shift[b * FOLD_SHIFT_LD + cl] = (cl < K0 && r1 > r0) ? (float)(t / (double)(r1 - r0)) : 0.f;
+  }
+}
 __global__ __launch_bounds__(1024, 8) void bwd_post_kernel(const float* __restrict__ gwp, int ntab_w,
                                                         int NK, float* __restrict__ gW, int accumulate,
                                                         int nA, const double* __restrict__ pst,
                                                         FmlpGroups grp, int K, int B,
                                                         double* __restrict__ prev_total,
-                                                        spt_gn_bwd_tables pn) {
+                                                        spt_gn_bwd_tables pn, FmlpFold fd) {
   if ((int)blockIdx.x < nA) {
     reduce_tables_body<float>(gwp, ntab_w, NK, gW, accumulate, (int)blockIdx.x);
+    return;
+  }
+  if (fd.tabs && (int)blockIdx.x >= fd.first) {
+    bwd_post_fold(pst, grp, K, B, pn, fd, (int)blockIdx.x - fd.first);
     return;
   }
   const int bx = (int)blockIdx.x - nA, len = 2 * K + 1;
@@ -1400,14 +1604,22 @@
 
 static void bwd_post_launch(const float* gwp, int ntab_w, int NK, float* gW, int accumulate,
                             const double* pst, const FmlpGroups& grp, int K, int B,
-                            double* prev_total, const spt_gn_bwd_tables* pn, hipStream_t stream) {
+                            double* prev_total, const spt_gn_bwd_tables* pn, hipStream_t stream,
+                            const FmlpFold* fold = nullptr) {
   const int nA = (NK + 15) / 16;
   spt_gn_bwd_tables none = {};
   int nB = 0;
   if (pn && pn->c1) nB = (K + 15) / 16;
   else if (prev_total) nB = ((2 * K + 1 + 15) / 16) * B;
-  bwd_post_kernel<<<nA + nB, 1024, 0, stream>>>(gwp, ntab_w, NK, gW, accumulate, nA, pst, grp, K, B,
-                                                prev_total, (pn && pn->c1) ? *pn : none);
+  FmlpFold fd = {};
+  int nF = 0;
+  if (fold) {
+    fd = *fold;
+    fd.first = nA + nB;
+    nF = ((K + 15) / 16) * fd.K0;
+  }
+  bwd_post_kernel<<<nA + nB + nF, 1024, 0, stream>>>(gwp, ntab_w, NK, gW, accumulate, nA, pst, grp, K, B,
+                                                     prev_total, (pn && pn->c1) ? *pn : none, fd);
 }
 
 static int grid_for_nw(int64_t rows, int per_cu, int nwv) {
@@ -1438,7 +1650,11 @@
                         const float* pbs, float pslope, const float* W, float* gx,
                         float* gw_partial, double* pstat_partial, const int32_t* perm,
                         const int32_t* pos_seg, const float* gout, const int32_t* arg,
-                        hipStream_t stream, bool s16 = false, int* gw_tabs = nullptr);
+                        hipStream_t stream, bool s16 = false, int* gw_tabs = nullptr,
+                        const float* x0 = nullptr, const float* fshift = nullptr,
+                        float* fold_partial = nullptr, int K0 = 0);
+bool fmlp_dma_fold_supported(int K0, int K, int N);
+int fmlp_fold_len(int K, int K0);
 }
 
 using namespace spt;
@@ -1673,9 +1889,17 @@
                          int K, const float* pre_am, const float* pre_scale, const float* pre_bias,
                          float pre_slope, const float* W, float* gx, float* gW, int accumulate,
                          double* prev_total, int mode, void* ws, size_t ws_bytes,
-                         hipStream_t stream, const spt_gn_bwd_tables* prev_norm = nullptr) {
+                         hipStream_t stream, const spt_gn_bwd_tables* prev_norm = nullptr,
+                         const float* fold_x0 = nullptr, int fold_K0 = 0, const float* fold_W0 = nullptr,
+                         float* fold_gW0 = nullptr) {
   const int g_fmlp_mode = fmlp_mode_of(mode);
   const bool g_fmlp_split_bf16 = g_fmlp_mode >= 1;
+  if (fold_x0) {
+    SPT_CHECK_ARG(!pooled && !gx && fold_W0 && fold_gW0 && prev_norm && pre_am,
+                  "fold: dense layer, no gx, norm tables");
+    SPT_CHECK_ARG(spt_fused_linear_bwd_fold_supported(fold_K0, K, N, mode), "fold: shape pair or mode not built");
+    SPT_CHECK_ARG(((size_t)fold_x0 & (fold_K0 % 4 == 0 ? 15 : 3)) == 0, "fold: x0 alignment");
+  }
   const bool want_prev = prev_total || prev_norm;
   SPT_CHECK_ARG(!prev_norm || (prev_norm->weight && prev_norm->mean_scale && prev_norm->mean &&
                                prev_norm->rstd && prev_norm->c1 && prev_norm->c2 && prev_norm->c3 &&
@@ -1692,7 +1916,7 @@
   } else {
     SPT_CHECK_ARG(spt_fused_linear_supported(K, N), "(K, N) not built");
     SPT_CHECK_ARG(gy, "null pointer");
-    SPT_CHECK_ARG(!want_prev || (gx && pre_am), "previous-layer statistics need gx and its tables");
+    SPT_CHECK_ARG(!want_prev || ((gx || fold_x0) && pre_am), "previous-layer statistics need gx and its tables");
   }
   const int k4 = (K + 3) / 4, nbk = N / 16;
   int gx_ = 1, nwv = 1;
@@ -1778,6 +2002,8 @@
           gy, h, 0, 0, am, scale, bias, slope, c1, c2, c3, xprev, K, pre_am, pre_scale,          \
           pre_bias, pre_slope, W, nullptr, gwp, nullptr, rt);                                    \
   }
+  float* fold_tabs = nullptr;
+  float* fold_shift = nullptr;
   int per_run = 0;
   int gw_tabs = 0;
   const bool h16 = mode >= 0 && (mode & SPT_FMLP_H_BF16), x16 = mode >= 0 && (mode & SPT_FMLP_X_BF16);
@@ -1839,6 +2065,32 @@
     }
 #undef XSP
 #undef XSD
+  } else if (fold_x0) {
+    constexpr size_t FOLD_MAX_TABS = 1024;
+    const int flen = fmlp_fold_len(K, fold_K0);
+    SPT_CHECK_ARG((FOLD_MAX_TABS * ((size_t)N * K + flen) + FMLP_MAX_RUNS * FOLD_SHIFT_LD) * 4 <=
+                  (size_t)MAX_BWD_WAVES * N * K * 4, "fold: tables do not fit the workspace");
+    fold_tabs = gwp + FOLD_MAX_TABS * N * K;
+    fold_shift = fold_tabs + FOLD_MAX_TABS * flen;
+    fold_shift_kernel<<<num_graphs, 1024, 0, stream>>>(fold_x0, fold_K0, rt, fold_shift);
+    if (fmlp_dma_of(mode) && fmlp_dma_fold_supported(fold_K0, K, N)) {
+      per_run = fmlp_dma_bwd_launch(false, true, gy, h, rt, max_rows, N, am, scale, bias, slope, c1, c2,
+                                    c3, xprev, K, pre_am, pre_scale, pre_bias, pre_slope, W, nullptr,
+                                    gwp, pstp, nullptr, nullptr, nullptr, nullptr, stream, false,
+                                    &gw_tabs, fold_x0, fold_shift, fold_tabs, fold_K0);
+    } else if (fold_K0 == 18 && k4 == 8 && nbk == 2) {
+      constexpr int NWB = 4;
+      gx_ = cap_grid(grid_for_nw(max_rows, 4, NWB), NWB);
+      nwv = NWB;
+      gw_tabs = gx_;
+      const dim3 grid((unsigned)gx_, (unsigned)nr);
+      bwd_kernel_bf<8, 2, true, NWB, true, false, false, false, false, 18><<<grid, NWB * 64, 0, stream>>>(
+          gy, h, 0, 0, am, scale, bias, slope, c1, c2, c3, xprev, K, pre_am, pre_scale, pre_bias,
+          pre_slope, W, nullptr, gwp, pstp, rt, nullptr, nullptr, nullptr, nullptr, fold_x0, fold_shift,
+          fold_tabs);
+      per_run = gx_ * nwv;
+    }
+    SPT_CHECK_ARG((size_t)gw_tabs * nr <= FOLD_MAX_TABS, "fold: more tables than the workspace layout holds");
   } else if (g_fmlp_split_bf16 && gx && fmlp_dma_of(mode) && fmlp_dma_supported(K, N)) {
     per_run = fmlp_dma_bwd_launch(pooled, g_fmlp_mode != 3, gy, h, rt, max_rows, N, am, scale, bias,
                                   slope, c1, c2, c3, xprev, K, pre_am, pre_scale, pre_bias, pre_slope,
@@ -1853,8 +2105,19 @@
 #undef X
 #undef XP
   SPT_CHECK_ARG(per_run > 0, "no kernel for this shape");
+  FmlpFold fd = {};
+  if (fold_x0) {
+    fd.tabs = fold_tabs;
+    fd.shift = fold_shift;
+    fd.gW0 = fold_gW0;
+    fd.W0 = fold_W0;
+    fd.am0 = pre_am;
+    fd.K0 = fold_K0;
+    fd.ZP = fold_zp(fold_K0);
+    fd.grp = fmlp_groups(rt, num_graphs, gw_tabs);
+  }
   bwd_post_launch(gwp, gw_tabs * nr, N * K, gW, accumulate, pst, fmlp_groups(rt, num_graphs, per_run), K,
-                  num_graphs, prev_total, prev_norm, stream);
+                  num_graphs, prev_total, prev_norm, stream, fold_x0 ? &fd : nullptr);
   SPT_CHECK_LAUNCH();
   return 0;
 }
@@ -1980,6 +2243,31 @@
                        am, scale, bias, slope, c1, c2, c3, xprev, K, pre_am, pre_scale, pre_bias,
                        pre_slope, W, gx, gW, 0, prev_total, mode, ws, ws_bytes, (hipStream_t)stream_,
                        prev_norm);
+}
+
+extern "C" int spt_fused_linear_bwd_fold_supported(int K0, int K, int N, int mode) {
+  const int m = fmlp_mode_of(mode);
+  if (mode >= 0 && (mode & (SPT_FMLP_H_BF16 | SPT_FMLP_X_BF16))) return 0;
+  return m == 1 && g_fmlp_x3 &&
+         ((fmlp_dma_of(mode) && fmlp_dma_fold_supported(K0, K, N)) || (K0 == 18 && K == 32 && N == 32));
+}
+extern "C" int spt_fused_linear_bwd_runs_gn_fold_f32(
+    const float* gy, const float* h, int nruns, const int64_t* run_r0, const int64_t* run_r1,
+    const int32_t* run_graph, int num_graphs, int N, const float* am, const float* scale,
+    const float* bias, float slope, const float* c1, const float* c2, const float* c3,
+    const float* xprev, int K, const float* pre_am, const float* pre_scale, const float* pre_bias,
+    float pre_slope, const float* W, float* gW, int mode, void* ws, size_t ws_bytes,
+    const spt_gn_bwd_tables* prev_norm, const float* x0, int K0, const float* W0, float* gW0,
+    spt_stream_t stream_) {
+  FmlpRuns rt;
+  int64_t max_rows;
+  const char* err = fmlp_make_runs(nruns, run_r0, run_r1, run_graph, num_graphs, &rt, &max_rows);
+  SPT_CHECK_ARG(!err, err ? err : "");
+  SPT_CHECK_ARG(prev_norm && x0 && W0 && gW0, "null pointer");
+  return fmlp_bwd_impl(false, gy, nullptr, nullptr, nullptr, nullptr, h, rt, max_rows, num_graphs, N,
+                       am, scale, bias, slope, c1, c2, c3, xprev, K, pre_am, pre_scale, pre_bias,
+                       pre_slope, W, nullptr, gW, 0, nullptr, mode, ws, ws_bytes, (hipStream_t)stream_,
+                       prev_norm, x0, K0, W0, gW0);
 }
 
 namespace spt {
diff --git a/superpoint_transformer_amd/csrc/fused_mlp_dma.hip b/superpoint_transformer_amd/csrc/fused_mlp_dma.hip
--- a/superpoint_transformer_amd/csrc/fused_mlp_dma.hip
+++ b/superpoint_transformer_amd/csrc/fused_mlp_dma.hip
@@ -83,7 +83,8 @@
   return r;
 }
 
-template <int K, int N, int NW, int OCC, bool LO, bool POOLED, bool S16 = false>
+constexpr int fold_len(int K, int K0) { return (K + (K0 + 16) / 16 * 16) * ((K0 + 16) / 16 * 16); }
+template <int K, int N, int NW, int OCC, bool LO, bool POOLED, bool S16 = false, int FK0 = 0>
 __global__ __launch_bounds__(NW * 64, OCC) void bwd_dma_kernel(
     const float* __restrict__ gy, const float* __restrict__ h, int64_t r0, int64_t r1,
     const float* __restrict__ am, const float* __restrict__ sc, const float* __restrict__ bs,
@@ -93,7 +94,13 @@
     float pslope, const float* __restrict__ W, float* __restrict__ gx,
     float* __restrict__ gw_partial, double* __restrict__ pstat_partial,
     const int32_t* __restrict__ perm, const int32_t* __restrict__ pos_seg,
-    const float* __restrict__ gout, const int32_t* __restrict__ arg, FmlpRuns rt) {
+    const float* __restrict__ gout, const int32_t* __restrict__ arg, FmlpRuns rt,
+    const float* __restrict__ x0 = nullptr, const float* __restrict__ fshift = nullptr,
+    float* __restrict__ fold_partial = nullptr) {
+  constexpr bool FOLD = FK0 > 0;
+  constexpr int FOLD_K0 = FK0;
+  static_assert(!FOLD || (!POOLED && !S16), "the fold reads dense f32 rows");
+  static_assert(!FOLD || (FK0 % 4 == 0 && FK0 < 16 && TR * FK0 * 4 <= 1024), "x0 tile: one DMA block, one k block");
   constexpr int NC = N / 4, KC = K / 4, NBK = N / 16, KB = K / 16, NS = N / 32;
   if (rt.n > 0) {
     const int run_ = blockIdx.y, gph_ = rt.g[run_];
@@ -104,6 +111,10 @@
     if (pam) { pam += (size_t)gph_ * K; psc += (size_t)gph_ * K; }
     gw_partial += (size_t)run_ * gridDim.x * N * K;
     if (pstat_partial) pstat_partial += (size_t)run_ * gridDim.x * NW * (2 * K + 1);
+    if constexpr (FOLD) {
+      fshift += (size_t)gph_ * 32;
+      fold_partial += (size_t)run_ * gridDim.x * fold_len(K, FK0);
+    }
   }
   constexpr int HI = TR * NC / 64, XI = TR * KC / 64;
   constexpr int RH = 64 / NC;
@@ -115,6 +126,8 @@
   __shared__ __attribute__((aligned(16))) __bf16 wt_hi[K * LDT];
   __shared__ __attribute__((aligned(16))) __bf16 wt_lo[LO ? K * LDT : 8];
   __shared__ __attribute__((aligned(16))) float pt[3 * K];
+  __shared__ __attribute__((aligned(16))) float x0b[FOLD ? NW : 1][FOLD ? 256 : 4];
+  __shared__ float fsh[16];
   const int lane = threadIdx.x & 63;
   const int wid = __builtin_amdgcn_readfirstlane(threadIdx.x >> 6);
   const int g = lane >> 4, c = lane & 15;
@@ -130,6 +143,9 @@
     wt_hi[k * LDT + n] = hh;
     if constexpr (LO) wt_lo[k * LDT + n] = (__bf16)(w - (float)hh);
   }
+  if constexpr (FOLD) {
+    if (threadIdx.x < 16) fsh[threadIdx.x] = threadIdx.x < FOLD_K0 ? fshift[threadIdx.x] : 0.f;
+  }
   for (int i = threadIdx.x; i < K; i += NW * 64) {
     pt[i] = pre ? pam[i] : 0.f;
     pt[K + i] = pre ? psc[i] : 1.f;
@@ -145,6 +161,10 @@
   double p1[KB], p2[KB];
 #pragma unroll
   for (int kb = 0; kb < KB; ++kb) p1[kb] = p2[kb] = 0.0;
+  f32x4 FA[FOLD ? KB : 1], FG = (f32x4){0.f, 0.f, 0.f, 0.f};
+#pragma unroll
+  for (int kb = 0; kb < (FOLD ? KB : 1); ++kb) FA[kb] = (f32x4){0.f, 0.f, 0.f, 0.f};
+  float* X0B = x0b[FOLD ? wid : 0];
 
   const int64_t ntiles = (r1 - r0 + TR - 1) / TR;
   const int64_t wave = (int64_t)blockIdx.x * NW + wid;
@@ -234,6 +254,11 @@
   auto issue_x = [&](int64_t t, int rid_l) {
     if (t >= ntiles) return;
     const int64_t row0 = r0 + t * TR;
+    if constexpr (FOLD) {
+      const int cnt = (int)((r1 - row0) < TR ? (r1 - row0) : TR);
+      const int last = cnt * FOLD_K0 - 4;
+      lds_dma16(x0 + row0 * FOLD_K0 + (4 * ln < last ? 4 * ln : last), X0B);
+    }
     if constexpr (S16) {
       const uint16_t* xb = reinterpret_cast<const uint16_t*>(xprev) + (POOLED ? 0 : row0 * K);
       const int x16 = ln / KC16, q16 = ln % KC16;
@@ -383,9 +408,23 @@
     const int rid_cur = rid_l;
     wait_lds();
     issue_h(t + nwaves, rid_n, seg_n);
+    bf16x4 X0h, X0l;
+    if constexpr (FOLD) {
+      float x0v[4];
+#pragma unroll
+      for (int r = 0; r < 4; ++r) {
+        const int rr = 4 * g + r;
+        const float xr = X0B[rr * FOLD_K0 + (c < FOLD_K0 ? c : 0)];
+        const float one = (c == FOLD_K0) ? 1.f : 0.f;
+        x0v[r] = (rr < cnt) ? ((c < FOLD_K0) ? xr - fsh[c] : one) : 0.f;
+      }
+      split_bf16<4>(x0v, X0h, X0l);
+      FG = mfma3_16<LO>(X0h, X0l, X0h, X0l, FG);
+    }
 #pragma unroll
     for (int kb = 0; kb < KB; ++kb) {
       const int k = 16 * kb + c;
+      float ggv[4] = {0.f, 0.f, 0.f, 0.f};
 #pragma unroll
       for (int r = 0; r < 4; ++r) {
         float* xs = XB + (4 * g + r) * K + 4 * ((4 * kb + (c >> 2)) ^ (4 * (g & 1))) + (c & 3);
@@ -399,18 +438,26 @@
           }
           p1[kb] += (double)gg;
           p2[kb] += (double)gg * (double)o;
-        }
-        *xs = v;
-      }
-    }
-    lds_order();
-#pragma unroll
-    for (int i = 0; i < XI; ++i) {
-      const int rr = hx + RX * i;
-      const float4 v = *reinterpret_cast<const float4*>(XB + rr * K + 4 * px);
-      const int64_t orow = POOLED ? (int64_t)pickx(rid_cur, RX * i) : row0 + rr;
-      if (!(SPT_FDMA_SKIP & 16) && rr < cnt)
-        *reinterpret_cast<float4*>(gx + orow * K + 4 * (px ^ (4 * ((rr >> 2) & 1)))) = v;
+          if constexpr (FOLD) ggv[r] = gg;
+        }
+        if constexpr (!FOLD) *xs = v;
+      }
+      if constexpr (FOLD) {
+        bf16x4 ah, al;
+        split_bf16<4>(ggv, ah, al);
+        FA[kb] = mfma3_16<LO>(ah, al, X0h, X0l, FA[kb]);
+      }
+    }
+    if constexpr (!FOLD) {
+      lds_order();
+#pragma unroll
+      for (int i = 0; i < XI; ++i) {
+        const int rr = hx + RX * i;
+        const float4 v = *reinterpret_cast<const float4*>(XB + rr * K + 4 * px);
+        const int64_t orow = POOLED ? (int64_t)pickx(rid_cur, RX * i) : row0 + rr;
+        if (!(SPT_FDMA_SKIP & 16) && rr < cnt)
+          *reinterpret_cast<float4*>(gx + orow * K + 4 * (px ^ (4 * ((rr >> 2) & 1)))) = v;
+      }
     }
     wait_lds();
     issue_x(t + nwaves, rid_n);
@@ -455,6 +502,40 @@
         for (int r = 0; r < 4; ++r)
           gwp[(size_t)(16 * nb + 4 * g + r) * K + 16 * kb + c] = C3[nb][kb][r];
   }
+  if constexpr (FOLD) {
+    constexpr int FLN = fold_len(K, FK0);
+    static_assert(FLN <= NW * (W_H + W_X + 2 * W_G), "the fold table fits the tile buffers");
+    float* red = &lw[0][0];
+    for (int w = 1; w < NW; ++w) {
+      if (wid == w) {
+#pragma unroll
+        for (int r = 0; r < 4; ++r) {
+#pragma unroll
+          for (int kb = 0; kb < KB; ++kb) red[(16 * kb + 4 * g + r) * 16 + c] = FA[kb][r];
+          red[(K + 4 * g + r) * 16 + c] = FG[r];
+        }
+      }
+      __syncthreads();
+      if (wid == 0) {
+#pragma unroll
+        for (int r = 0; r < 4; ++r) {
+#pragma unroll
+          for (int kb = 0; kb < KB; ++kb) FA[kb][r] += red[(16 * kb + 4 * g + r) * 16 + c];
+          FG[r] += red[(K + 4 * g + r) * 16 + c];
+        }
+      }
+      __syncthreads();
+    }
+    if (wid == 0) {
+      float* fp = fold_partial + (size_t)blockIdx.x * FLN;
+#pragma unroll
+      for (int r = 0; r < 4; ++r) {
+#pragma unroll
+        for (int kb = 0; kb < KB; ++kb) fp[(16 * kb + 4 * g + r) * 16 + c] = FA[kb][r];
+        fp[(K + 4 * g + r) * 16 + c] = FG[r];
+      }
+    }
+  }
   if (pstat_partial) {
     double* pp = pstat_partial + (size_t)wave * (2 * K + 1);
 #pragma unroll
@@ -471,10 +552,15 @@
 
 }
 
+bool fmlp_dma_fold_supported(int K0, int K, int N) {
+  return K0 == 12 && K == 32 && N == 64;
+}
+int fmlp_fold_len(int K, int K0) { return fdma::fold_len(K, K0); }
 bool fmlp_dma_supported(int K, int N) {
   return (K == 64 && N == 128) || (K == 32 && N == 64) || (K == 64 && N == 64);
 }
 
+bool fmlp_dma_fold_supported(int K0, int K, int N);
 int fmlp_dma_bwd_launch(bool pooled, bool lo, const float* gy, const float* h, FmlpRuns rt,
                         int64_t max_rows, int N, const float* am, const float* sc, const float* bs,
                         float slope, const float* c1, const float* c2, const float* c3,
@@ -482,10 +568,24 @@
                         const float* pbs, float pslope, const float* W, float* gx,
                         float* gw_partial, double* pstat_partial, const int32_t* perm,
                         const int32_t* pos_seg, const float* gout, const int32_t* arg,
-                        hipStream_t stream, bool s16, int* gw_tabs) {
+                        hipStream_t stream, bool s16, int* gw_tabs, const float* x0,
+                        const float* fshift, float* fold_partial, int K0) {
   using namespace fdma;
   const int64_t tiles = (max_rows + TR - 1) / TR;
   const int nr = rt.n < 1 ? 1 : rt.n;
+  if (x0) {
+    if (!fmlp_dma_fold_supported(K0, K, N) || pooled || s16 || !lo || !fshift || !fold_partial || !pam) return 0;
+    int64_t blocks = (tiles + 8 - 1) / 8;
+    const int64_t cap = (256 * 2) / nr > 1 ? (256 * 2) / nr : 1;
+    if (blocks > cap) blocks = cap;
+    if (blocks < 1) blocks = 1;
+    const dim3 grid((unsigned)blocks, (unsigned)nr);
+    bwd_dma_kernel<32, 64, 8, 4, true, false, false, 12><<<grid, 8 * 64, 0, stream>>>(
+        gy, h, 0, 0, am, sc, bs, slope, c1, c2, c3, xprev, pam, psc, pbs, pslope, W, nullptr,
+        gw_partial, pstat_partial, perm, pos_seg, gout, arg, rt, x0, fshift, fold_partial);
+    if (gw_tabs) *gw_tabs = (int)blocks;
+    return (int)blocks * 8;
+  }
 #define SPT_DMA_CASE(KK, NN, NWV, PER_CU, OCC)                                                        \
   if (K == KK && N == NN) {                                                                        \
     int64_t blocks = (tiles + NWV - 1) / NWV;                                                      \
diff --git a/superpoint_transformer_amd/ops.py b/superpoint_transformer_amd/ops.py
--- a/superpoint_transformer_amd/ops.py
+++ b/superpoint_transformer_amd/ops.py
@@ -1502,6 +1502,17 @@
     return old
 
 
+FOLD_BOTTOM = os.environ.get("SPT_FMLP_FOLD_BOTTOM", "1") != "0"
+
+
+def fold_bottom(on=None):
+    global FOLD_BOTTOM
+    old = FOLD_BOTTOM
+    if on is not None:
+        FOLD_BOTTOM = bool(on)
+    return old
+
+
 def _fmlp_backward(saved, meta, gy, top_total=None, pooled=None, top_tabs=None):
     L, runs, slopes, in_dtype, need_gx0 = meta[:5]
     fmode = meta[5] if len(meta) > 5 else -1
@@ -1552,7 +1563,13 @@
                 _lib.check(st, "spt_graphnorm_bwd_tables_f32")
             xprev = hs[l - 1] if l else x2
             pre = tabs[l - 1] if l else None
-            want_gx = l > 0 or need_gx0
+            lmode = (3 | _ST_H | (_ST_X if l else 0)) if store16 else fmode
+            fold = (l == 1 and FOLD_BOTTOM and FUSE_POST and not need_gx0 and not store16
+                    and not (pooled is not None and l == L - 1)
+                    and x2.dtype == torch.float32 and x2.data_ptr() % 16 == 0
+                    and bool(_lib.lib.spt_fused_linear_bwd_fold_supported(
+                        int(Ws[0].shape[1]), K, N, lmode)))
+            want_gx = (l > 0 or need_gx0) and not fold
             gx = torch.empty((R, K), dtype=torch.float32, device=dev) if want_gx else None
             gW = torch.empty((N, K), dtype=torch.float32, device=dev)
             nxt_tabs, pn = None, None
@@ -1567,7 +1584,21 @@
             pa = ps = pb = None
             if pre is not None:
                 pa, ps, pb = pre[2], pre[3], gnb[l - 1]
-            lmode = (3 | _ST_H | (_ST_X if l else 0)) if store16 else fmode
+            if fold:
+                K0 = int(Ws[0].shape[1])
+                gW0 = torch.empty((K, K0), dtype=torch.float32, device=dev)
+                with _timed(f"fused_linear_bwd_fold:{K0}x{K}x{N}:{R}"):
+                    st = _lib.lib.spt_fused_linear_bwd_runs_gn_fold_f32(
+                        _lib.ptr(g_cur), _lib.ptr(hs[l]), nr, c_r0, c_r1, c_g, B, N,
+                        _lib.ptr(am), _lib.ptr(sc), _lib.ptr(gnb[l]), float(slopes[l]),
+                        _lib.ptr(c1), _lib.ptr(c2), _lib.ptr(c3), _lib.ptr(xprev), K,
+                        _lib.ptr(pa), _lib.ptr(ps), _lib.ptr(pb), float(slopes[0]), _lib.ptr(Ws[l]),
+                        _lib.ptr(gW), lmode, _lib.ptr(ws), ws.numel(), ctypes.addressof(pn),
+                        _lib.ptr(x2), K0, _lib.ptr(Ws[0]), _lib.ptr(gW0), sp)
+                _lib.check(st, "spt_fused_linear_bwd_runs_gn_fold_f32")
+                grads[4], grads[5], grads[6], grads[7] = gW, gw_n, gb_n, ga_n
+                grads[0], grads[1], grads[2], grads[3] = gW0, nxt_tabs[3], nxt_tabs[4], nxt_tabs[5]
+                break
             if pooled is not None and l == L - 1:
                 p_gout, p_arg, p_csr = pooled
                 args = (_lib.ptr(p_gout), _lib.ptr(p_arg), _lib.ptr(p_csr.perm),
```

After: 360.0, median of 6. +3.4%, better.
